# stemangiola/ppcseq

Hardware: AMD Instinct MI355X
Metric: effective samples/sec (whole node) for NB hierarchical fit (higher is better)
Workload: dtype f64; 1 GPU; BASELINE cfg3: synthetic 20000 genes x 200 samples (seed 20253), C=2, K=1000; NUTS (Stan defaults) warm-up 150 + 250 kept draws/chain, 8 chains per GPU (cfg3 names 8 chains; chains are the sharded unit, so N GPUs run 8N chains); mode=chains, chains_total=8, lanes_per_gene=4, loglik_workgroups=939, ess_estimator=rank-normalised split-chain bulk-ESS, min over 6 hyper-parameters and lp__, grad_evals=1471121, divergent_after_warmup=0, round_structure=pipelined: merged log-likelihood / state-machine launch + gene kernel, stream_groups=library default (3 from eight chains on, 2 from four), rounds_last_step_all_groups=115040

## Files before the change

### include/ppcx.h

```cpp
#ifndef PPCX_H
#define PPCX_H
#include <stdint.h>
#ifdef __cplusplus
extern "C" {
#endif

#if defined(__GNUC__)
#define PPCX_API __attribute__((visibility("default")))
#else
#define PPCX_API
#endif

#define PPCX_OK 0
#define PPCX_ERR_ARG (-1)
#define PPCX_ERR_HIP (-2)
#define PPCX_ERR_INIT (-3)
#define PPCX_ERR_STEPSIZE (-4)
#define PPCX_ERR_STALL (-5)
#define PPCX_ERR_LIMIT (-6)
#define PPCX_ERR_CANCELLED (-7)

typedef struct ppcx_model ppcx_model;
typedef struct ppcx_fit ppcx_fit;

#define PPCX_VERSION 400
PPCX_API int ppcx_version(void);
PPCX_API int ppcx_device_count(void);
PPCX_API int ppcx_device_memory(int device, unsigned long long* free_bytes, unsigned long long* total_bytes);
PPCX_API const char* ppcx_last_error(void);

PPCX_API int ppcx_model_create(int device, int G, int S, int C, int K, const int32_t* counts, const double* X,
                      const double* exposure_rate, double lambda_mu_mu, int n_excl, const int32_t* excl,
                      ppcx_model** out);
PPCX_API int ppcx_model_set_exclusions(ppcx_model* m, int n_excl, const int32_t* excl);
PPCX_API int ppcx_model_set_launch(ppcx_model* m, int lanes_per_gene, int workgroups);
PPCX_API int ppcx_model_get_launch(const ppcx_model* m, int* lanes_per_gene, int* nblocks);
PPCX_API int ppcx_model_set_rounds(ppcx_model* m, int pipelined, int stream_groups);
typedef int (*ppcx_progress_fn)(void* user, int first_chain, int chains, int chains_done, long long rounds, double seconds);
PPCX_API int ppcx_model_set_progress(ppcx_model* m, ppcx_progress_fn fn, void* user, double every_seconds);
PPCX_API int ppcx_model_get_rounds(const ppcx_model* m, int nchains, int* pipelined, int* stream_groups);
PPCX_API int ppcx_model_get_plan(ppcx_model* m, int nchains, int* lanes_per_gene, int* workgroups_per_chain, int* bounds, int cap);
PPCX_API int ppcx_model_dim(const ppcx_model* m);
PPCX_API void ppcx_model_destroy(ppcx_model* m);

PPCX_API int ppcx_log_prob_grad(ppcx_model* m, int n_points, const double* u, double* lp, double* grad);

typedef struct {
  int chains, iter, warmup;
  unsigned long long seed;
  double adapt_delta;
  int max_treedepth;
  double init_radius;
  double stepsize0;
  int init_buffer, term_buffer, window;
  int chain_id_offset;
} ppcx_nuts_config;
PPCX_API void ppcx_nuts_config_default(ppcx_nuts_config* cfg);

PPCX_API int ppcx_fit_nuts(ppcx_model* m, const ppcx_nuts_config* cfg, ppcx_fit** out);
PPCX_API int ppcx_fit_info(const ppcx_fit* f, int* chains, int* n_keep, int* D, int* iter);
PPCX_API int ppcx_fit_from_draws(ppcx_model* m, int chains, int n_keep, const double* draws, ppcx_fit** out);
PPCX_API int ppcx_fit_get_draws(ppcx_fit* f, double* out);
PPCX_API int ppcx_fit_get_columns(ppcx_fit* f, int n_cols, const int32_t* cols, double* out);
#define PPCX_SUMMARY_FIELDS 8
PPCX_API int ppcx_fit_summary(ppcx_fit* f, int n_cols, const int32_t* cols, double* out);
PPCX_API int ppcx_fit_get_approximation(ppcx_fit* f, double* mu, double* omega);
PPCX_API int ppcx_fit_get_log_ratios(ppcx_fit* f, double* log_p, double* log_g);
PPCX_API int ppcx_fit_psis(ppcx_fit* f, int n_cols, const int32_t* cols, double* khat);
#define PPCX_LOO_FIELDS 4
PPCX_API int ppcx_fit_get_log_lik(ppcx_fit* f, int n_genes, const int32_t* genes, double* out);
PPCX_API int ppcx_fit_loo(ppcx_fit* f, int n_genes, const int32_t* genes, const double* r_eff, double* out);
#define PPCX_LOO_MCSE_FIELDS 6
PPCX_API int ppcx_fit_loo_mcse(ppcx_fit* f, int n_genes, const int32_t* genes, const double* r_eff, double* out);
PPCX_API int ppcx_fit_relative_eff(ppcx_fit* f, int n_genes, const int32_t* genes, double* out);
#define PPCX_LOO_PREDICT_FIELDS 6
PPCX_API int ppcx_fit_loo_predict(ppcx_fit* f, int n_genes, const int32_t* genes, const double* r_eff, double truncation_compensation,
                                  double p_lo, double p_hi, unsigned long long seed, double* out);
PPCX_API int ppcx_fit_loo_approx(ppcx_fit* f, int n_genes, const int32_t* genes, double* out);
PPCX_API int ppcx_fit_loo_predict_approx(ppcx_fit* f, int n_genes, const int32_t* genes, double truncation_compensation, double p_lo,
                                         double p_hi, unsigned long long seed, double* out);
#define PPCX_PPC_EXACT_FIELDS 9
PPCX_API int ppcx_fit_ppc_exact(ppcx_fit* f, int n_genes, const int32_t* genes, double truncation_compensation, double p_lo,
                                double p_hi, double* out);
PPCX_API int ppcx_fit_get_diagnostics(ppcx_fit* f, double* lp, double* stepsize, int32_t* treedepth,
                             int32_t* n_leapfrog, int32_t* divergent, double* accept);
PPCX_API int ppcx_fit_get_inv_metric(ppcx_fit* f, double* inv_metric);
PPCX_API int ppcx_fit_get_timing(ppcx_fit* f, double* seconds, long long* grad_evals, double* gene_kernel_ms_mean,
                        long long* gene_kernel_samples, double* gene_kernel_chain_launches_mean);

PPCX_API int ppcx_fit_get_kernel_times(ppcx_fit* f, double* loglik_ms, double* close_ms, double* update_ms,
                              long long* launch_triples);

PPCX_API int ppcx_fit_ppc(ppcx_fit* f, double truncation_compensation, double p_lo, double p_hi,
                 unsigned long long seed, int n_gen, int resample, double* ci, int32_t* counts_rng);
PPCX_API int ppcx_fit_get_ppc_timing(ppcx_fit* f, double* kernel_ms, long long* nb_draws);
PPCX_API void ppcx_fit_free(ppcx_fit* f);

PPCX_API void ppcx_do_inference_C(const int* dims, const int* counts, const double* X, const double* exposure_rate,
                         const int* excl, const double* reals, double* ci, double* slope, int* counts_rng,
                         int* status, char** errbuf, const int* errlen);

typedef struct {
  int output_samples, iter; double tol_rel_obj; int grad_samples, elbo_samples, eval_elbo, adapt_iter;
  unsigned long long seed; double init_radius;
} ppcx_advi_config;
PPCX_API void ppcx_advi_config_default(ppcx_advi_config* cfg);
PPCX_API int ppcx_fit_advi(ppcx_model* m, const ppcx_advi_config* cfg, ppcx_fit** out);
PPCX_API int ppcx_fit_advi_iterative(ppcx_model* m, const ppcx_advi_config* cfg, int max_attempts, ppcx_fit** out);
PPCX_API int ppcx_fit_advi_info(const ppcx_fit* f, int* iterations, int* converged, double* elbo, double* eta);

typedef struct ppcx_comm ppcx_comm;
PPCX_API int ppcx_model_create_shard(int device, int G_total, int S, int C, int K_total, int g0, int g1,
                            const int32_t* counts_shard, const double* X, const double* exposure_rate,
                            double lambda_mu_mu, int n_excl, const int32_t* excl_local, ppcx_model** out);
PPCX_API int ppcx_model_create_shard_strided(int device, int G_total, int S, int C, int K_total, int g0, int gene_stride, int n_genes,
                            const int32_t* counts_shard, const double* X, const double* exposure_rate,
                            double lambda_mu_mu, int n_excl, const int32_t* excl_local, ppcx_model** out);
PPCX_API int ppcx_fit_nuts_shards(ppcx_model** shards, int n_shards, const ppcx_nuts_config* cfg, ppcx_fit** fits);
PPCX_API int ppcx_comm_unique_id(char* out128);
PPCX_API int ppcx_comm_create(int device, int nranks, int rank, const char* id128, ppcx_comm** out);
PPCX_API void ppcx_comm_destroy(ppcx_comm* c);
PPCX_API int ppcx_fit_nuts_comm(ppcx_model* shard, const ppcx_nuts_config* cfg, ppcx_comm* comm, ppcx_fit** out);

typedef struct ppcx_xchg ppcx_xchg;
PPCX_API int ppcx_xchg_create(int device, int nranks, int rank, int max_chains, ppcx_xchg** out);
PPCX_API int ppcx_xchg_handle(ppcx_xchg* x, char* out64);
PPCX_API int ppcx_xchg_connect(ppcx_xchg* x, const char* handles );
PPCX_API int ppcx_xchg_connect_local(ppcx_xchg** group, int n);
PPCX_API int ppcx_xchg_set_timeout(ppcx_xchg* x, double seconds);
PPCX_API void ppcx_xchg_destroy(ppcx_xchg* x);
PPCX_API int ppcx_fit_nuts_xchg(ppcx_model* shard, const ppcx_nuts_config* cfg, ppcx_xchg* x, ppcx_fit** out);
PPCX_API int ppcx_fit_get_xchg_timing(ppcx_fit* f, double* wait_us_per_exchange, long long* exchanges);

PPCX_API int ppcx_guard_decision(const double* reduced5, int local_status);

#ifdef __cplusplus
}
#endif
#endif
```

### ppcseq_amd/_lib.py

```python
from __future__ import annotations

import ctypes as C
import os
from dataclasses import dataclass

import numpy as np

_HERE = os.path.dirname(os.path.abspath(__file__))
LIB_PATH = os.environ.get("PPCX_LIB", os.path.join(_HERE, "libppcx.so"))

EXPORTS = [
    "ppcx_version", "ppcx_device_count", "ppcx_last_error", "ppcx_model_create", "ppcx_model_set_exclusions",
    "ppcx_model_set_launch", "ppcx_model_get_launch", "ppcx_model_get_plan", "ppcx_model_dim", "ppcx_model_destroy", "ppcx_log_prob_grad",
    "ppcx_nuts_config_default", "ppcx_fit_nuts", "ppcx_fit_info", "ppcx_fit_from_draws", "ppcx_fit_get_draws", "ppcx_fit_get_columns",
    "ppcx_fit_get_diagnostics", "ppcx_fit_get_timing", "ppcx_fit_get_kernel_times", "ppcx_fit_ppc", "ppcx_fit_free", "ppcx_do_inference_C", "ppcx_model_set_rounds", "ppcx_model_get_rounds", "ppcx_model_set_progress",
    "ppcx_model_create_shard", "ppcx_model_create_shard_strided", "ppcx_fit_nuts_shards", "ppcx_comm_unique_id", "ppcx_comm_create", "ppcx_comm_destroy",
    "ppcx_fit_nuts_comm", "ppcx_advi_config_default", "ppcx_fit_advi", "ppcx_fit_advi_info", "ppcx_fit_advi_iterative",
    "ppcx_guard_decision", "ppcx_device_memory", "ppcx_fit_get_ppc_timing",
    "ppcx_xchg_create", "ppcx_xchg_handle", "ppcx_xchg_connect", "ppcx_xchg_connect_local", "ppcx_xchg_set_timeout", "ppcx_xchg_destroy",
    "ppcx_fit_nuts_xchg", "ppcx_fit_get_xchg_timing", "ppcx_fit_get_inv_metric", "ppcx_fit_summary",
    "ppcx_fit_get_approximation", "ppcx_fit_get_log_ratios", "ppcx_fit_psis", "ppcx_fit_get_log_lik", "ppcx_fit_loo",
    "ppcx_fit_loo_predict", "ppcx_fit_relative_eff", "ppcx_fit_loo_mcse", "ppcx_fit_loo_approx", "ppcx_fit_loo_predict_approx",
    "ppcx_fit_ppc_exact",
]
ABI_VERSION = 400
SUMMARY_FIELDS = ("mean", "sd", "q05", "q50", "q95", "rhat", "ess_bulk", "ess_tail")
LOO_FIELDS = ("elpd_loo", "p_loo", "looic", "khat")
LOO_MCSE_FIELDS = LOO_FIELDS + ("mcse_elpd_loo", "n_eff")
LOO_PREDICT_FIELDS = ("mean", "lower", "upper", "pit_lt", "pit_le", "khat")
PPC_EXACT_FIELDS = ("mean", "sd", "p_le", "p_ge", "lower", "upper", "y", "excluded", "outside")


class PpcxError(RuntimeError):
    pass


class NutsConfig(C.Structure):
    _fields_ = [("chains", C.c_int), ("iter", C.c_int), ("warmup", C.c_int), ("seed", C.c_ulonglong),
                ("adapt_delta", C.c_double), ("max_treedepth", C.c_int), ("init_radius", C.c_double),
                ("stepsize0", C.c_double), ("init_buffer", C.c_int), ("term_buffer", C.c_int), ("window", C.c_int),
                ("chain_id_offset", C.c_int)]


class AdviConfig(C.Structure):
    _fields_ = [("output_samples", C.c_int), ("iter", C.c_int), ("tol_rel_obj", C.c_double), ("grad_samples", C.c_int),
                ("elbo_samples", C.c_int), ("eval_elbo", C.c_int), ("adapt_iter", C.c_int), ("seed", C.c_ulonglong),
                ("init_radius", C.c_double)]


PROGRESS_FN = C.CFUNCTYPE(C.c_int, C.c_void_p, C.c_int, C.c_int, C.c_int, C.c_longlong, C.c_double)
_lib = None


def use_library(path=None):
    global _lib, LIB_PATH
    _lib = None
    LIB_PATH = path if path else os.environ.get("PPCX_LIB", os.path.join(_HERE, "libppcx.so"))


def load() -> C.CDLL:
    global _lib
    if _lib is not None:
        return _lib
    if not os.path.exists(LIB_PATH):
        raise PpcxError(f"{LIB_PATH} not found: run `python -m ppcseq_amd.build` (hipcc, gfx950) first; "
                        "there is no CPU fallback")
    lib = C.CDLL(LIB_PATH)
    lib.ppcx_version.restype = C.c_int
    if lib.ppcx_version() != ABI_VERSION:
        raise PpcxError(f"{LIB_PATH} has ABI version {lib.ppcx_version()}, this binding needs {ABI_VERSION}: rebuild it "
                        "(`python -m ppcseq_amd.build --force`)")
    dp, ip = C.POINTER(C.c_double), C.POINTER(C.c_int32)
    lib.ppcx_guard_decision.argtypes = [dp, C.c_int]
    lib.ppcx_device_memory.argtypes = [C.c_int, C.POINTER(C.c_ulonglong), C.POINTER(C.c_ulonglong)]
    lib.ppcx_fit_get_ppc_timing.argtypes = [C.c_void_p, dp, C.POINTER(C.c_longlong)]
    lib.ppcx_last_error.restype = C.c_char_p
    lib.ppcx_model_create.argtypes = [C.c_int] * 5 + [ip, dp, dp, C.c_double, C.c_int, ip, C.POINTER(C.c_void_p)]
    lib.ppcx_model_set_exclusions.argtypes = [C.c_void_p, C.c_int, ip]
    lib.ppcx_model_set_launch.argtypes = [C.c_void_p, C.c_int, C.c_int]
    lib.ppcx_model_get_launch.argtypes = [C.c_void_p, C.POINTER(C.c_int), C.POINTER(C.c_int)]
    lib.ppcx_model_get_plan.argtypes = [C.c_void_p, C.c_int, C.POINTER(C.c_int), C.POINTER(C.c_int), C.POINTER(C.c_int32), C.c_int]
    lib.ppcx_model_dim.argtypes = [C.c_void_p]
    lib.ppcx_model_destroy.argtypes = [C.c_void_p]
    lib.ppcx_model_destroy.restype = None
    lib.ppcx_log_prob_grad.argtypes = [C.c_void_p, C.c_int, dp, dp, dp]
    lib.ppcx_nuts_config_default.argtypes = [C.POINTER(NutsConfig)]
    lib.ppcx_nuts_config_default.restype = None
    lib.ppcx_fit_nuts.argtypes = [C.c_void_p, C.POINTER(NutsConfig), C.POINTER(C.c_void_p)]
    lib.ppcx_fit_info.argtypes = [C.c_void_p] + [C.POINTER(C.c_int)] * 4
    lib.ppcx_fit_from_draws.argtypes = [C.c_void_p, C.c_int, C.c_int, dp, C.POINTER(C.c_void_p)]
    lib.ppcx_fit_get_draws.argtypes = [C.c_void_p, dp]
    lib.ppcx_fit_get_columns.argtypes = [C.c_void_p, C.c_int, ip, dp]
    lib.ppcx_fit_summary.argtypes = [C.c_void_p, C.c_int, ip, dp]
    lib.ppcx_fit_get_approximation.argtypes = [C.c_void_p, dp, dp]
    lib.ppcx_fit_get_log_ratios.argtypes = [C.c_void_p, dp, dp]
    lib.ppcx_fit_psis.argtypes = [C.c_void_p, C.c_int, ip, dp]
    lib.ppcx_fit_get_log_lik.argtypes = [C.c_void_p, C.c_int, ip, dp]
    lib.ppcx_fit_loo.argtypes = [C.c_void_p, C.c_int, ip, dp, dp]
    lib.ppcx_fit_loo_mcse.argtypes = [C.c_void_p, C.c_int, ip, dp, dp]
    lib.ppcx_fit_loo_predict.argtypes = [C.c_void_p, C.c_int, ip, dp, C.c_double, C.c_double, C.c_double, C.c_ulonglong, dp]
    lib.ppcx_fit_relative_eff.argtypes = [C.c_void_p, C.c_int, ip, dp]
    lib.ppcx_fit_loo_approx.argtypes = [C.c_void_p, C.c_int, ip, dp]
    lib.ppcx_fit_loo_predict_approx.argtypes = [C.c_void_p, C.c_int, ip, C.c_double, C.c_double, C.c_double, C.c_ulonglong, dp]
    lib.ppcx_fit_ppc_exact.argtypes = [C.c_void_p, C.c_int, ip, C.c_double, C.c_double, C.c_double, dp]
    lib.ppcx_fit_get_diagnostics.argtypes = [C.c_void_p, dp, dp, ip, ip, ip, dp]
    lib.ppcx_fit_get_timing.argtypes = [C.c_void_p, dp, C.POINTER(C.c_longlong), dp, C.POINTER(C.c_longlong), dp]
    lib.ppcx_fit_get_kernel_times.argtypes = [C.c_void_p, dp, dp, dp, C.POINTER(C.c_longlong)]
    lib.ppcx_fit_get_inv_metric.argtypes = [C.c_void_p, dp]
    lib.ppcx_fit_ppc.argtypes = [C.c_void_p, C.c_double, C.c_double, C.c_double, C.c_ulonglong, C.c_int, C.c_int, dp, ip]
    lib.ppcx_fit_free.argtypes = [C.c_void_p]
    lib.ppcx_model_set_rounds.argtypes = [C.c_void_p, C.c_int, C.c_int]
    lib.ppcx_xchg_create.argtypes = [C.c_int, C.c_int, C.c_int, C.c_int, C.POINTER(C.c_void_p)]
    lib.ppcx_xchg_handle.argtypes = [C.c_void_p, C.c_char_p]
    lib.ppcx_xchg_connect.argtypes = [C.c_void_p, C.c_char_p]
    lib.ppcx_xchg_connect_local.argtypes = [C.POINTER(C.c_void_p), C.c_int]
    lib.ppcx_xchg_set_timeout.argtypes = [C.c_void_p, C.c_double]
    lib.ppcx_xchg_destroy.argtypes = [C.c_void_p]
    lib.ppcx_xchg_destroy.restype = None
    lib.ppcx_fit_nuts_xchg.argtypes = [C.c_void_p, C.POINTER(NutsConfig), C.c_void_p, C.POINTER(C.c_void_p)]
    lib.ppcx_fit_get_xchg_timing.argtypes = [C.c_void_p, dp, C.POINTER(C.c_longlong)]
    lib.ppcx_model_get_rounds.argtypes = [C.c_void_p, C.c_int, C.POINTER(C.c_int), C.POINTER(C.c_int)]
    lib.ppcx_model_set_progress.argtypes = [C.c_void_p, PROGRESS_FN, C.c_void_p, C.c_double]
    if hasattr(lib, "ppcx_testing_set"):
        lib.ppcx_testing_set.argtypes = [C.c_char_p, C.c_longlong]
        lib.ppcx_testing_set_nccl_provider.argtypes = [C.c_char_p]
        lib.ppcx_testing_bench_kernel.argtypes = [C.c_void_p, C.c_int, C.c_int, C.c_int, C.c_int, C.c_int, dp, C.POINTER(C.c_int)]
    if hasattr(lib, "ppcx_testing_eval_math"):
        lib.ppcx_testing_eval_math.argtypes = [C.c_int, C.c_int, dp, dp, ip, dp, dp]
    if hasattr(lib, "ppcx_testing_get_disp_table"):
        lib.ppcx_testing_get_disp_table.argtypes = [C.c_void_p, dp]
    if hasattr(lib, "ppcx_testing_psis"):
        lib.ppcx_testing_psis.argtypes = [C.c_int, C.c_int, dp, dp, dp]
    if hasattr(lib, "ppcx_testing_loo"):
        lib.ppcx_testing_loo.argtypes = [C.c_int, C.c_int, dp, ip, dp, dp]
    if hasattr(lib, "ppcx_testing_loo_mcse"):
        lib.ppcx_testing_loo_mcse.argtypes = [C.c_int, C.c_int, dp, ip, dp, dp]
    if hasattr(lib, "ppcx_testing_loo_predict"):
        lib.ppcx_testing_loo_predict.argtypes = [dp, ip, C.c_int, C.c_int, ip, ip, dp, C.c_double, C.c_double, dp]
    if hasattr(lib, "ppcx_testing_loo_approx"):
        lib.ppcx_testing_loo_approx.argtypes = [C.c_int, C.c_int, dp, dp, ip, dp]
        lib.ppcx_testing_loo_predict_approx.argtypes = [dp, dp, ip, C.c_int, C.c_int, ip, ip, C.c_double, C.c_double, dp]
    if hasattr(lib, "ppcx_testing_relative_eff"):
        lib.ppcx_testing_relative_eff.argtypes = [C.c_int, C.c_int, C.c_int, dp, dp]
    if hasattr(lib, "ppcx_testing_ppc_exact"):
        lib.ppcx_testing_ppc_exact.argtypes = [C.c_int, C.c_int, dp, dp, ip, ip, C.c_double, C.c_double, C.c_double, dp]
    lib.ppcx_fit_free.restype = None
    lib.ppcx_advi_config_default.argtypes = [C.POINTER(AdviConfig)]
    lib.ppcx_advi_config_default.restype = None
    lib.ppcx_fit_advi.argtypes = [C.c_void_p, C.POINTER(AdviConfig), C.POINTER(C.c_void_p)]
    lib.ppcx_fit_advi_iterative.argtypes = [C.c_void_p, C.POINTER(AdviConfig), C.c_int, C.POINTER(C.c_void_p)]
    lib.ppcx_fit_advi_info.argtypes = [C.c_void_p, C.POINTER(C.c_int), C.POINTER(C.c_int), C.POINTER(C.c_double), C.POINTER(C.c_double)]
    lib.ppcx_model_create_shard.argtypes = [C.c_int] * 7 + [ip, dp, dp, C.c_double, C.c_int, ip, C.POINTER(C.c_void_p)]
    lib.ppcx_model_create_shard_strided.argtypes = [C.c_int] * 8 + [ip, dp, dp, C.c_double, C.c_int, ip, C.POINTER(C.c_void_p)]
    lib.ppcx_fit_nuts_shards.argtypes = [C.POINTER(C.c_void_p), C.c_int, C.POINTER(NutsConfig), C.POINTER(C.c_void_p)]
    lib.ppcx_comm_unique_id.argtypes = [C.c_char_p]
    lib.ppcx_comm_create.argtypes = [C.c_int, C.c_int, C.c_int, C.c_char_p, C.POINTER(C.c_void_p)]
    lib.ppcx_comm_destroy.argtypes = [C.c_void_p]
    lib.ppcx_comm_destroy.restype = None
    lib.ppcx_fit_nuts_comm.argtypes = [C.c_void_p, C.POINTER(NutsConfig), C.c_void_p, C.POINTER(C.c_void_p)]
    _lib = lib
    return lib


def _check(rc: int):
    if rc != 0:
        raise PpcxError(f"ppcx error {rc}: {load().ppcx_last_error().decode()}")


def _p(a, t):
    return a.ctypes.data_as(C.POINTER(t)) if a is not None else None


def testing_set(key: str, value: int):
    lib = load()
    if not hasattr(lib, "ppcx_testing_set"):
        raise PpcxError(f"{LIB_PATH} is not the testing build")
    _check(lib.ppcx_testing_set(key.encode(), int(value)))


def testing_set_nccl_provider(path: str):
    lib = load()
    if not hasattr(lib, "ppcx_testing_set_nccl_provider"):
        raise PpcxError(f"{LIB_PATH} is not the testing build")
    _check(lib.ppcx_testing_set_nccl_provider(path.encode() if path else None))


TESTING_MATH = ("fast_rcp", "fast_log", "fast_exp", "table_log", "window_log", "stirling_tails", "stirling_excess",
                "log_erfc_ratio", "cell", "cell_win", "cell_y", "cell_win_y", "sincos_2pi", "lgamma_int1", "rng_exp", "rng_div")
TESTING_MATH_MORE = ("nb2_tails",)


def testing_eval_math(fn: str, a, b=None, y=None):
    lib = load()
    if not hasattr(lib, "ppcx_testing_eval_math"):
        raise PpcxError(f"{LIB_PATH} is not the testing build, or one built before ppcx_testing_math.hip existed: rebuild it "
                        "(`python -m ppcseq_amd.build --testing --force`)")
    a = np.ascontiguousarray(a, dtype=np.float64).ravel()
    n = a.size
    b = np.ascontiguousarray(np.zeros(n) if b is None else np.broadcast_to(b, (n,)), dtype=np.float64)
    y = np.ascontiguousarray(np.zeros(n) if y is None else np.broadcast_to(y, (n,)), dtype=np.int32)
    o0, o1 = np.zeros(n), np.zeros(n)
    rc = lib.ppcx_testing_eval_math((TESTING_MATH + TESTING_MATH_MORE).index(fn), n, _p(a, C.c_double), _p(b, C.c_double), _p(y, C.c_int32),
                                    _p(o0, C.c_double), _p(o1, C.c_double))
    if rc != 0:
        raise PpcxError(f"ppcx_testing_eval_math({fn}) failed with code {rc}")
    return o0, o1


def testing_psis(lr, cols=None):
    lib = load()
    if not hasattr(lib, "ppcx_testing_psis"):
        raise PpcxError(f"{LIB_PATH} is not the testing build, or one built before ppcx_testing_psis existed: rebuild it "
                        "(`python -m ppcseq_amd.build --testing --force`)")
    lr = np.ascontiguousarray(lr, dtype=np.float64).ravel()
    n = lr.size
    cols = np.zeros((n, 0)) if cols is None else np.ascontiguousarray(cols, dtype=np.float64).reshape(n, -1)
    out = np.zeros(cols.shape[1] + 1)
    _check(lib.ppcx_testing_psis(n, int(cols.shape[1]), _p(lr, C.c_double), _p(cols, C.c_double) if cols.size else None,
                                 _p(out, C.c_double)))
    return out


def testing_loo(ll, excluded=None, r_eff=None):
    return _testing_loo("ppcx_testing_loo", LOO_FIELDS, ll, excluded, r_eff)


def testing_loo_mcse(ll, excluded=None, r_eff=None):
    return _testing_loo("ppcx_testing_loo_mcse", LOO_MCSE_FIELDS, ll, excluded, r_eff)


def _testing_loo(entry, fields, ll, excluded, r_eff):
    lib = load()
    if not hasattr(lib, entry):
        raise PpcxError(f"{LIB_PATH} is not the testing build, or one built before {entry} existed: rebuild it "
                        "(`python -m ppcseq_amd.build --testing --force`)")
    ll = np.asarray(ll, dtype=np.float64)
    ll = ll.reshape(ll.shape[0], -1)
    n, nc = ll.shape
    cols = np.ascontiguousarray(ll.T)
    ex = None if excluded is None else np.ascontiguousarray(excluded, dtype=np.int32).ravel()
    re = None if r_eff is None else np.ascontiguousarray(r_eff, dtype=np.float64).ravel()
    out = np.zeros((nc, len(fields)))
    _check(getattr(lib, entry)(n, nc, _p(cols, C.c_double), _p(ex, C.c_int32) if ex is not None else None,
                               _p(re, C.c_double) if re is not None else None, _p(out, C.c_double)))
    return out


def testing_loo_predict(ll, x, y, excluded=None, r_eff=None, p_lo=0.025, p_hi=0.975):
    lib = load()
    if not hasattr(lib, "ppcx_testing_loo_predict"):
        raise PpcxError(f"{LIB_PATH} is not the testing build, or one built before ppcx_testing_loo_predict existed: rebuild it "
                        "(`python -m ppcseq_amd.build --testing --force`)")
    ll = np.asarray(ll, dtype=np.float64)
    ll = ll.reshape(ll.shape[0], -1)
    n, nc = ll.shape
    cols = np.ascontiguousarray(ll.T)
    xs = np.ascontiguousarray(np.asarray(x).reshape(n, nc).T, dtype=np.int32)
    ys = np.ascontiguousarray(np.broadcast_to(np.asarray(y), (nc,)), dtype=np.int32)
    ex = None if excluded is None else np.ascontiguousarray(excluded, dtype=np.int32).ravel()
    re = None if r_eff is None else np.ascontiguousarray(r_eff, dtype=np.float64).ravel()
    out = np.zeros((nc, len(LOO_PREDICT_FIELDS)))
    _check(lib.ppcx_testing_loo_predict(_p(cols, C.c_double), _p(xs, C.c_int32), n, nc, _p(ys, C.c_int32),
                                        _p(ex, C.c_int32) if ex is not None else None,
                                        _p(re, C.c_double) if re is not None else None, float(p_lo), float(p_hi),
                                        _p(out, C.c_double)))
    return out


def _testing_approx_columns(entry, ll, log_ratio, excluded):
    lib = load()
    if not hasattr(lib, entry):
        raise PpcxError(f"{LIB_PATH} is not the testing build, or one built before {entry} existed: rebuild it "
                        "(`python -m ppcseq_amd.build --testing --force`)")
    ll = np.asarray(ll, dtype=np.float64)
    ll = ll.reshape(ll.shape[0], -1)
    lr = np.ascontiguousarray(log_ratio, dtype=np.float64).ravel()
    if lr.size != ll.shape[0]:
        raise ValueError("log_ratio must hold one value per draw")
    ex = None if excluded is None else np.ascontiguousarray(excluded, dtype=np.int32).ravel()
    return lib, np.ascontiguousarray(ll.T), lr, ex


def testing_loo_approx(ll, log_ratio, excluded=None):
# ... 11 lines not shown
    xs = np.ascontiguousarray(np.asarray(x).reshape(n, nc).T, dtype=np.int32)
    ys = np.ascontiguousarray(np.broadcast_to(np.asarray(y), (nc,)), dtype=np.int32)
    out = np.zeros((nc, len(LOO_PREDICT_FIELDS)))
    _check(lib.ppcx_testing_loo_predict_approx(_p(cols, C.c_double), _p(lr, C.c_double), _p(xs, C.c_int32), n, nc, _p(ys, C.c_int32),
                                               _p(ex, C.c_int32) if ex is not None else None, float(p_lo), float(p_hi),
                                               _p(out, C.c_double)))
    return out


def testing_relative_eff(ll, chains):
    lib = load()
    if not hasattr(lib, "ppcx_testing_relative_eff"):
        raise PpcxError(f"{LIB_PATH} is not the testing build, or one built before ppcx_testing_relative_eff existed: rebuild it "
                        "(`python -m ppcseq_amd.build --testing --force`)")
    ll = np.asarray(ll, dtype=np.float64)
    ll = ll.reshape(ll.shape[0], -1)
    rows, nc = ll.shape
    chains = int(chains)
    if chains < 1 or rows % chains:
        raise ValueError("ll must hold chains * n rows")
    cols = np.ascontiguousarray(ll.T)
    out = np.zeros(nc)
    _check(lib.ppcx_testing_relative_eff(chains, rows // chains, nc, _p(cols, C.c_double), _p(out, C.c_double)))
    return out


def _ppc_exact_dict(out):
    res = {k: out[..., i].copy() for i, k in enumerate(PPC_EXACT_FIELDS)}
    nan = np.isnan(res["lower"]) | np.isnan(res["upper"])
    for k in ("lower", "upper"):
        res[k] = np.where(nan, -1, res[k]).astype(np.int64)
    res["y"] = res["y"].astype(np.int64)
    res["excluded"] = res["excluded"] != 0
    res["outside"] = np.where(nan, 0, res["outside"]) != 0
    return res


def testing_ppc_exact(eta, sigma_raw, y, excluded=None, truncation_compensation=1.0, p_lo=0.025, p_hi=0.975, raw=False):
    lib = load()
    if not hasattr(lib, "ppcx_testing_ppc_exact"):
        raise PpcxError(f"{LIB_PATH} is not the testing build, or one built before ppcx_testing_ppc_exact existed: rebuild it "
                        "(`python -m ppcseq_amd.build --testing --force`)")
    eta = np.asarray(eta, dtype=np.float64)
    eta = eta.reshape(eta.shape[0], -1)
    n, nc = eta.shape
    ec = np.ascontiguousarray(eta.T)
    sc = np.ascontiguousarray(np.asarray(sigma_raw, dtype=np.float64).reshape(n, nc).T)
    ys = np.ascontiguousarray(np.broadcast_to(np.asarray(y), (nc,)), dtype=np.int32)
    ex = None if excluded is None else np.ascontiguousarray(excluded, dtype=np.int32).ravel()
    out = np.zeros((nc, len(PPC_EXACT_FIELDS)))
    _check(lib.ppcx_testing_ppc_exact(n, nc, _p(ec, C.c_double), _p(sc, C.c_double), _p(ys, C.c_int32),
                                      _p(ex, C.c_int32) if ex is not None else None, float(truncation_compensation), float(p_lo),
                                      float(p_hi), _p(out, C.c_double)))
    return out if raw else _ppc_exact_dict(out)


def loo_estimates(pointwise, excluded):
    keep = ~np.asarray(excluded, bool)
    out = {}
    for name in LOO_FIELDS[:3]:
        v = np.asarray(pointwise[name], dtype=np.float64)[keep]
        se = float(np.sqrt(v.size * np.var(v, ddof=1))) if v.size > 1 else float("nan")
        out[name] = (float(np.sum(v)), se)
    return out


def device_count() -> int:
    return int(load().ppcx_device_count())


def device_memory(device=0):
    f, t = C.c_ulonglong(), C.c_ulonglong()
    _check(load().ppcx_device_memory(int(device), C.byref(f), C.byref(t)))
    return int(f.value), int(t.value)


def shard_genes(G_total, g0, stride):
    return list(range(int(g0), int(G_total), int(stride)))


class Model:

    def __init__(self, counts, X, exposure_rate, K, lambda_mu_mu=5.612671, excl=None, device=0, shard=None):
        lib = load()
        counts = np.ascontiguousarray(counts, dtype=np.int32)
        if counts.ndim != 2:
            raise ValueError("counts must be G x S")
        self.G, self.S = counts.shape
        X = np.asfortranarray(np.asarray(X, dtype=np.float64).reshape(self.S, -1))
        self.C = X.shape[1]
        self.K = int(K)
        exposure_rate = np.ascontiguousarray(exposure_rate, dtype=np.float64)
        if exposure_rate.shape != (self.S,):
            raise ValueError("exposure_rate must have length S")
        excl = np.ascontiguousarray(excl if excl is not None else np.zeros(0), dtype=np.int32)
        self.X, self.exposure_rate = X, exposure_rate
        self.excl = excl.copy()
        self.counts = counts
        h = C.c_void_p()
        self.shard = shard
        if shard is None:
            _check(lib.ppcx_model_create(int(device), self.G, self.S, self.C, self.K, _p(counts, C.c_int32),
                                         _p(X, C.c_double), _p(exposure_rate, C.c_double), float(lambda_mu_mu),
                                         int(excl.size), _p(excl, C.c_int32), C.byref(h)))
        else:
            if len(shard) == 5:
                Gt, Kt, g0, stride = int(shard[0]), int(shard[1]), int(shard[2]), int(shard[4])
                if len(shard_genes(Gt, g0, stride)) != self.G:
                    raise ValueError("counts must hold exactly the genes of the shard")
                self.K = len([g for g in shard_genes(Gt, g0, stride) if g < Kt])
                _check(lib.ppcx_model_create_shard_strided(int(device), Gt, self.S, self.C, Kt, g0, stride, self.G, _p(counts, C.c_int32),
                                                           _p(X, C.c_double), _p(exposure_rate, C.c_double), float(lambda_mu_mu),
                                                           int(excl.size), _p(excl, C.c_int32), C.byref(h)))
            else:
                Gt, Kt, g0, g1 = (int(v) for v in shard)
                if g1 - g0 != self.G:
                    raise ValueError("counts must hold exactly the genes of the shard")
                self.K = max(0, min(g1, Kt) - min(g0, Kt))
                _check(lib.ppcx_model_create_shard(int(device), Gt, self.S, self.C, Kt, g0, g1, _p(counts, C.c_int32),
                                                   _p(X, C.c_double), _p(exposure_rate, C.c_double), float(lambda_mu_mu),
                                                   int(excl.size), _p(excl, C.c_int32), C.byref(h)))
        self._h = h
        self.D = int(lib.ppcx_model_dim(h))

    def set_exclusions(self, excl):
        excl = np.ascontiguousarray(excl if excl is not None else np.zeros(0), dtype=np.int32)
        _check(load().ppcx_model_set_exclusions(self._h, int(excl.size), _p(excl, C.c_int32)))
        self.excl = excl.copy()

    def set_launch(self, lanes_per_gene=0, workgroups=0):
        _check(load().ppcx_model_set_launch(self._h, int(lanes_per_gene), int(workgroups)))

    def get_plan(self, nchains):
        lanes, nb = C.c_int(), C.c_int()
        _check(load().ppcx_model_get_plan(self._h, int(nchains), C.byref(lanes), C.byref(nb), None, 0))
        b = np.zeros(4 * nb.value + 1, np.int32)
        _check(load().ppcx_model_get_plan(self._h, int(nchains), C.byref(lanes), C.byref(nb), _p(b, C.c_int32), int(b.size)))
        return lanes.value, nb.value, b

    def get_launch(self):
        a, b = C.c_int(), C.c_int()
        _check(load().ppcx_model_get_launch(self._h, C.byref(a), C.byref(b)))
        return a.value, b.value

    def testing_disp_table(self):
        lib = load()
        if not hasattr(lib, "ppcx_testing_get_disp_table"):
            raise PpcxError(f"{LIB_PATH} is not the testing build, or one built before ppcx_testing_get_disp_table existed: "
                            "rebuild it (`python -m ppcseq_amd.build --testing --force`)")
        out = np.zeros((self.G, 32, 2, 12))
        _check(lib.ppcx_testing_get_disp_table(self._h, _p(out, C.c_double)))
        return out

    def log_prob_grad(self, u):
        u = np.ascontiguousarray(u, dtype=np.float64)
        one = u.ndim == 1
        u2 = u.reshape(-1, self.D)
        lp = np.zeros(u2.shape[0])
        g = np.zeros_like(u2)
        _check(load().ppcx_log_prob_grad(self._h, u2.shape[0], _p(u2, C.c_double), _p(lp, C.c_double), _p(g, C.c_double)))
        return (float(lp[0]), g[0]) if one else (lp, g)

    def fit_nuts(self, chains=3, iter=300, warmup=150, seed=1, adapt_delta=0.8, max_treedepth=10, init_radius=2.0,
                 stepsize0=1.0, init_buffer=75, term_buffer=50, window=25, chain_id_offset=0) -> "Fit":
        cfg = NutsConfig(chains, iter, warmup, seed, adapt_delta, max_treedepth, init_radius, stepsize0,
                         init_buffer, term_buffer, window, chain_id_offset)
        h = C.c_void_p()
        _check(load().ppcx_fit_nuts(self._h, C.byref(cfg), C.byref(h)))
        return Fit(self, h)

    def fit_advi(self, output_samples=1000, iter=50000, tol_rel_obj=0.005, elbo_samples=100, eval_elbo=100, adapt_iter=50,
                 seed=1, init_radius=2.0, max_attempts=1) -> "Fit":
        cfg = AdviConfig(output_samples, iter, tol_rel_obj, 1, elbo_samples, eval_elbo, adapt_iter, seed, init_radius)
        h = C.c_void_p()
        if max_attempts > 1:
            _check(load().ppcx_fit_advi_iterative(self._h, C.byref(cfg), int(max_attempts), C.byref(h)))
        else:
            _check(load().ppcx_fit_advi(self._h, C.byref(cfg), C.byref(h)))
        return Fit(self, h)

    def fit_from_draws(self, draws) -> "Fit":
        draws = np.ascontiguousarray(draws, dtype=np.float64)
        if draws.ndim != 3 or draws.shape[2] != self.D:
            raise ValueError("draws must be [chains, n_keep, D]")
        h = C.c_void_p()
        _check(load().ppcx_fit_from_draws(self._h, draws.shape[0], draws.shape[1], _p(draws, C.c_double), C.byref(h)))
        return Fit(self, h)

    def fit_nuts_comm(self, comm: "Comm", **kw) -> "Fit":
        cfg = _make_cfg(**kw)
        h = C.c_void_p()
        _check(load().ppcx_fit_nuts_comm(self._h, C.byref(cfg), comm._h, C.byref(h)))
        return Fit(self, h)

    def fit_nuts_xchg(self, xchg: "Xchg", **kw) -> "Fit":
        cfg = _make_cfg(**kw)
        h = C.c_void_p()
        _check(load().ppcx_fit_nuts_xchg(self._h, C.byref(cfg), xchg._h, C.byref(h)))
        return Fit(self, h)

    def set_rounds(self, pipelined=-2, stream_groups=-1):
        _check(load().ppcx_model_set_rounds(self._h, int(pipelined), int(stream_groups)))

    def set_progress(self, fn=None, every_seconds=1.0):
        self._progress_cb = PROGRESS_FN((lambda user, c0, n, done, rounds, sec: 1 if fn(c0, n, done, rounds, sec) else 0) if fn else 0)
        _check(load().ppcx_model_set_progress(self._h, self._progress_cb, None, float(every_seconds)))

    def get_rounds(self, nchains=1):
        a, b = C.c_int(), C.c_int()
        _check(load().ppcx_model_get_rounds(self._h, int(nchains), C.byref(a), C.byref(b)))
        return bool(a.value), b.value

    def bench_kernel(self, which=0, nchains=1, warm_rounds=40, reps=50, n_merge=1):
        lib = load()
        if not hasattr(lib, "ppcx_testing_bench_kernel"):
            raise PpcxError(f"{LIB_PATH} is not the testing build")
        ms, t = C.c_double(), C.c_int()
        _check(lib.ppcx_testing_bench_kernel(self._h, int(which), nchains, warm_rounds, reps, n_merge, C.byref(ms), C.byref(t)))
        return ms.value, t.value

    def close(self):
        if getattr(self, "_h", None):
            load().ppcx_model_destroy(self._h)
            self._h = None

    def __del__(self):
        try:
            self.close()
        except Exception:
            pass


def _make_cfg(chains=3, iter=300, warmup=150, seed=1, adapt_delta=0.8, max_treedepth=10, init_radius=2.0,
              stepsize0=1.0, init_buffer=75, term_buffer=50, window=25, chain_id_offset=0):
    return NutsConfig(chains, iter, warmup, seed, adapt_delta, max_treedepth, init_radius, stepsize0,
                      init_buffer, term_buffer, window, chain_id_offset)


def fit_nuts_shards(models, **kw):
    cfg = _make_cfg(**kw)
    n = len(models)
    hm = (C.c_void_p * n)(*[m._h for m in models])
    hf = (C.c_void_p * n)()
    _check(load().ppcx_fit_nuts_shards(hm, n, C.byref(cfg), hf))
    return [Fit(m, C.c_void_p(h)) for m, h in zip(models, hf)]


class Comm:

    @staticmethod
    def unique_id() -> bytes:
        buf = C.create_string_buffer(128)
        _check(load().ppcx_comm_unique_id(buf))
        return buf.raw

    def __init__(self, nranks, rank, unique_id: bytes, device=0):
        h = C.c_void_p()
        _check(load().ppcx_comm_create(int(device), int(nranks), int(rank), unique_id, C.byref(h)))
        self._h = h

    def close(self):
        if getattr(self, "_h", None):
            load().ppcx_comm_destroy(self._h)
            self._h = None


class Xchg:

    def __init__(self, nranks, rank, max_chains, device=0):
        h = C.c_void_p()
        _check(load().ppcx_xchg_create(int(device), int(nranks), int(rank), int(max_chains), C.byref(h)))
        self._h, self.nranks, self.rank = h, int(nranks), int(rank)

    def handle(self) -> bytes:
        buf = C.create_string_buffer(64)
        _check(load().ppcx_xchg_handle(self._h, buf))
        return buf.raw

    def connect(self, handles):
        blob = b"".join(handles)
        if len(blob) != 64 * self.nranks:
            raise ValueError("need one 64-byte handle per rank")
        _check(load().ppcx_xchg_connect(self._h, blob))

    @staticmethod
    def local_group(n, max_chains, devices=None):
        xs = [Xchg(n, k, max_chains, device=(devices[k] if devices else 0)) for k in range(n)]
        arr = (C.c_void_p * n)(*[x._h for x in xs])
        _check(load().ppcx_xchg_connect_local(arr, n))
        return xs

    def set_timeout(self, seconds):
        _check(load().ppcx_xchg_set_timeout(self._h, float(seconds)))

    def close(self):
        if getattr(self, "_h", None):
            load().ppcx_xchg_destroy(self._h)
            self._h = None


@dataclass
class Timing:
    seconds: float
    grad_evals: int
    gene_kernel_ms_mean: float
    gene_kernel_samples: int
# ... 212 lines not shown
```

### ppcseq_amd/build.py

```python
from __future__ import annotations

import os
import subprocess
import sys
import threading

HERE = os.path.dirname(os.path.abspath(__file__))
CSRC = os.path.join(HERE, "csrc")
LIB = os.path.join(HERE, "libppcx.so")
TESTING_LIB = os.path.join(os.path.dirname(HERE), "tests", "libppcx_testing.so")
SOURCES = ["ppcx_kernels.hip", "ppcx_summary.hip", "ppcx_psis.hip", "ppcx_loo.hip", "ppcx_loo_predict.hip", "ppcx_reff.hip", "ppcx_ppc_exact.hip", "ppcx_ppc.hip",
           "ppcx_capi.hip", "ppcx_run.hip", "ppcx_fit_nuts.hip", "ppcx_fit_advi.hip", "ppcx_fit_api.hip"]
TESTING_SOURCES = ["ppcx_testing_math.hip"]
HEADERS = ["ppcx_math.h", "ppcx_disp.h", "ppcx_model.h", "ppcx_nuts.h", "ppcx_gene.h", "ppcx_kernels.h", "ppcx_summary.h", "ppcx_summary_dev.h", "ppcx_psis.h", "ppcx_psis_dev.h", "ppcx_loo.h", "ppcx_loo_ap.h", "ppcx_loo_dev.h", "ppcx_loo_predict.h", "ppcx_reff.h", "ppcx_nbcdf.h", "ppcx_ppc_exact.h", "ppcx_ppc.h", "ppcx_table.h", "ppcx_block.h", "ppcx_columns.h", "ppcx_host.h", "ppcx_testing.h",
           os.path.join("..", "..", "include", "ppcx.h")]


CODEGEN_FLAGS = ["-fno-slp-vectorize"]


def _sources(extra):
    return SOURCES + (TESTING_SOURCES if "-DPPCX_TESTING" in extra else [])


def _stale(lib: str, extra=()) -> bool:
    if not os.path.exists(lib):
        return True
    t = os.path.getmtime(lib)
    return any(os.path.getmtime(os.path.join(CSRC, f)) > t for f in _sources(extra) + HEADERS)


_COMPILERS = threading.BoundedSemaphore(16)


def _start_compiler(cmd):
    _COMPILERS.acquire()
    p = subprocess.Popen(cmd)
    threading.Thread(target=lambda: (p.wait(), _COMPILERS.release()), daemon=True).start()
    return p


def _compile(lib: str, extra, verbose: bool) -> None:
    hipcc = os.environ.get("HIPCC", "/opt/rocm/bin/hipcc")
    objs = []
    procs = []
    for s in _sources(extra):
        o = lib + "." + s + ".o"
        objs.append(o)
        cmd = [hipcc, "-O3", "-std=c++17", "--offload-arch=gfx950", "-fPIC", "-fvisibility=hidden", "-Wno-unused-result"] + CODEGEN_FLAGS + extra + \
              ["-c", "-o", o, os.path.join(CSRC, s)]
        if verbose:
            print(" ".join(cmd), file=sys.stderr)
        procs.append(_start_compiler(cmd))
    for p in procs:
        if p.wait() != 0:
            raise subprocess.CalledProcessError(p.returncode, p.args)
    subprocess.check_call([hipcc, "--offload-arch=gfx950", "-shared", "-fPIC", "-o", lib] + objs)
    for o in objs:
        os.remove(o)


def build(force: bool = False, verbose: bool = False) -> str:
    if force or _stale(LIB):
        _compile(LIB, [], verbose)
    return LIB


def build_testing(force: bool = False, verbose: bool = False) -> str:
    if force or _stale(TESTING_LIB, ["-DPPCX_TESTING"]):
        _compile(TESTING_LIB, ["-DPPCX_TESTING"], verbose)
    return TESTING_LIB


def build_all(force: bool = False, verbose: bool = False):
    jobs = []
    if force or _stale(LIB):
        jobs.append((LIB, []))
    if force or _stale(TESTING_LIB, ["-DPPCX_TESTING"]):
        jobs.append((TESTING_LIB, ["-DPPCX_TESTING"]))
    errs = []

    def run(lib, extra):
        try:
            _compile(lib, extra, verbose)
        except Exception as e:
            errs.append(e)
    th = [threading.Thread(target=run, args=j) for j in jobs]
    for t in th:
        t.start()
    for t in th:
        t.join()
    if errs:
        raise errs[0]
    return LIB, TESTING_LIB


if __name__ == "__main__":
    if "--testing" in sys.argv:
        print(*build_all(force="--force" in sys.argv, verbose=True))
    else:
        print(build(force="--force" in sys.argv, verbose=True))
```

### ppcseq_amd/csrc/ppcx_capi.hip

```cpp
#include <math.h>
#include <stdlib.h>
#include <algorithm>
#include <memory>
#include "ppcx_host.h"

thread_local std::string g_err;
int fail(int code, const std::string& msg) { g_err = msg; return code; }
int hip_fail(hipError_t e, const char* what) { return fail(PPCX_ERR_HIP, std::string(what) + ": " + hipGetErrorString(e)); }
int hip_done(const char* who, hipError_t e) {
  return e == hipSuccess ? PPCX_OK : who ? hip_fail(e, who) : fail(PPCX_ERR_HIP, hipGetErrorString(e));
}
#ifdef PPCX_TESTING
TestHooks g_test;
#endif

extern "C" int ppcx_version(void) { return PPCX_VERSION; }
extern "C" int ppcx_device_count(void) { int n = 0; if (hipGetDeviceCount(&n) != hipSuccess) return 0; return n; }
extern "C" const char* ppcx_last_error(void) { return g_err.c_str(); }
extern "C" int ppcx_device_memory(int device, unsigned long long* free_bytes, unsigned long long* total_bytes) {
  int ndev = 0;
  HIPCHK(hipGetDeviceCount(&ndev));
  if (device < 0 || device >= ndev) return fail(PPCX_ERR_ARG, "no such HIP device");
  HIPCHK(hipSetDevice(device));
  size_t f = 0, t = 0;
  HIPCHK(hipMemGetInfo(&f, &t));
  if (free_bytes) *free_bytes = (unsigned long long)f;
  if (total_bytes) *total_bytes = (unsigned long long)t;
  return PPCX_OK;
}

static double pass_cost(const ppcx_model* m, int L, int p, int n) {
  const int S = m->d.S;
  bool slope = false;
  for (int i = p; i < p + n; ++i) slope = slope || m->pos_slope[i];
  double slope_w = m->d.C > 2 ? 1.0 : 1.15;
#ifdef PPCX_TESTING
  if (g_test.slope_cost_permille > 0) slope_w = 1e-3 * g_test.slope_cost_permille;
#endif
  double lin_w = 2.5;
#ifdef PPCX_TESTING
  if (g_test.slope_cost_permille > 0) lin_w = 1e-3 * g_test.slope_cost_permille;
#endif
  const double sweep = (double)((S + L - 1) / L) * (!m->d.x0_is_one ? 2.5 : (slope && !m->d.x1_binary ? lin_w : (slope ? slope_w : 1.0)));
  return 5.8 + sweep;
}
static int resident_workgroups(const ppcx_model* m, int reserve) {
  int n = m->wgs_override > 0 ? m->wgs_override : m->n_cu * (reserve > 0 ? m->ls_wgs_per_cu : m->wgs_per_cu);
  n -= reserve;
  return n < 1 ? 1 : n;
}
constexpr double kTrimSlack = 0.0;
static int workgroups_per_chain(const ppcx_model* m, int L, int nch, int n_res, bool whole_runs = true, bool trim = false) {
  int nbpc = n_res / (nch < 1 ? 1 : nch);
  if (nbpc >= 8 && whole_runs) nbpc = nbpc / 8 * 8;
  if (nbpc < 1) nbpc = 1;
  const int gpw = 64 / L, npass = (m->d.G + gpw - 1) / gpw;
  if (nbpc > (npass + 3) / 4) nbpc = (npass + 3) / 4;
  if (trim) {
    double slack = kTrimSlack;
#ifdef PPCX_TESTING
    if (g_test.trim_slack_permille >= 0) slack = 1e-3 * g_test.trim_slack_permille;
#endif
    int maxp = (npass + 4 * nbpc - 1) / (4 * nbpc);
#ifdef PPCX_TESTING
    maxp += g_test.trim_extra_passes;
#endif
    int nb2 = (int)ceil((double)npass * (1.0 + slack) / (4.0 * maxp));
    if (nb2 >= 8 && whole_runs) nb2 = (nb2 + 7) / 8 * 8;
    if (nb2 < nbpc) nbpc = nb2;
  }
  return nbpc;
}
static int default_stream_groups(int nch) { return nch >= 8 ? 3 : (nch >= 4 ? 2 : 1); }
int fit_stream_groups(const ppcx_model* m, int nch) {
  if (m->opt_stream_groups >= 1) return m->opt_stream_groups < nch ? m->opt_stream_groups : nch;
  return default_stream_groups(nch);
}
int fit_launch_chains(const ppcx_model* m, int nch) {
  const int g = fit_stream_groups(m, nch);
  return (nch + g - 1) / g;
}
static void drop_plans(ppcx_model* m) {
  std::lock_guard<std::mutex> lk(m->plan_mutex);
  m->plans.clear();
}
void choose_launch(ppcx_model* m, int nchains) {
  const int G = m->d.G, S = m->d.S;
  int bestL = 64; double best = 1e300;
  for (int L = 64; L >= 1; L >>= 1) {
    const int gpw = 64 / L;
    const double npass = ceil((double)G / gpw), c_pass = (8.0 + (double)((S + L - 1) / L)) * (L <= 2 ? 1.2 : 1.0);
    const int wpc = 4 * workgroups_per_chain(m, L, nchains, resident_workgroups(m, 0));
    const double t = ceil(npass / wpc) * c_pass;
    if (t < best) { best = t; bestL = L; }
  }
  const int L = m->L_override > 0 ? m->L_override : bestL;
  if (L != m->L) {
    drop_plans(m);
    m->L = L;
  }
  m->nblocks_chosen = workgroups_per_chain(m, m->L, nchains, resident_workgroups(m, 0)) * nchains;
}
int plan_launch(ppcx_model* m, int nch, int reserve, bool trim, int* nbpc_out, const int** d_bounds_out) {
  std::lock_guard<std::mutex> lk(m->plan_mutex);
  const int n_res = resident_workgroups(m, reserve);
  const auto key = std::make_pair(nch, trim ? -n_res : n_res);
  auto it = m->plans.find(key);
  if (it != m->plans.end()) { *nbpc_out = it->second.nbpc; *d_bounds_out = it->second.d_bounds.p; return PPCX_OK; }
  const int G = m->d.G, L = m->L, gpw = 64 / L;
  const int nbpc = workgroups_per_chain(m, L, nch, n_res, reserve == 0, trim), wpc = 4 * nbpc, npass = (G + gpw - 1) / gpw;
  std::vector<double> cost(npass);
  double total = 0;
  for (int k = 0; k < npass; ++k) {
    const int p = k * gpw;
    cost[k] = pass_cost(m, L, p, G - p < gpw ? G - p : gpw);
    total += cost[k];
  }
  std::vector<int> bounds(wpc + 1, G);
  bounds[0] = 0;
  {
    int k = 0; double cum = 0.0;
    for (int j = 1; j < wpc; ++j) {
      const double target = total * (double)j / (double)wpc;
      while (k < npass && cum + 0.5 * cost[k] < target) cum += cost[k++];
      bounds[j] = k * gpw < G ? k * gpw : G;
    }
  }
  {
    const long pmax = ((long)(npass + wpc - 1) / wpc) * gpw;
    for (int j = 0; j < wpc; ++j) if (bounds[j + 1] - bounds[j] > pmax) bounds[j + 1] = (int)(bounds[j] + pmax);
    bounds[wpc] = G;
    for (int j = wpc - 1; j >= 0; --j) if (bounds[j + 1] - bounds[j] > pmax) bounds[j] = (int)(bounds[j + 1] - pmax);
  }
  DeviceBuffer<int> d_bounds;
  HIPCHK(d_bounds.alloc((size_t)(wpc + 1)));
  HIPCHK(hipMemcpy(d_bounds.p, bounds.data(), sizeof(int) * (size_t)(wpc + 1), hipMemcpyHostToDevice));
  ppcx_model::Plan& pl = m->plans[key];
  pl.nbpc = nbpc; std::swap(pl.d_bounds.p, d_bounds.p);
  *nbpc_out = pl.nbpc; *d_bounds_out = pl.d_bounds.p;
  return PPCX_OK;
}

static int upload_counts(ppcx_model* m, int n_excl, const int32_t* excl) {
  const int G = m->d.G, S = m->d.S, C = m->d.C;
  std::vector<int32_t> cnt(m->counts_host);
  for (int e = 0; e < n_excl; ++e) {
    if (excl[e] < 0 || excl[e] >= G * S) return fail(PPCX_ERR_ARG, "excluded cell id out of range");
    cnt[excl[e]] = -1;
  }
  std::vector<double> Sy(G, 0.0), SyE(G, 0.0), SyX((size_t)C * G, 0.0), SX((size_t)C * G, 0.0), ncell(G, 0.0), Lg1(G, 0.0);
  std::vector<unsigned char> gflags(G, 0);
  for (int g = 0; g < G; ++g) {
    double sy = 0, sye = 0, nc = 0, lg1 = 0;
    for (int s = 0; s < S; ++s) {
      const int y = cnt[(size_t)g * S + s];
      if (y < 0) { gflags[g] |= 1; continue; }
      sy += y; sye += (double)y * m->expo_host[s]; nc += 1.0; lg1 += lgamma((double)y + 1.0);
      for (int c = 0; c < C; ++c) { SyX[(size_t)c * G + g] += (double)y * m->X_host[(size_t)c * S + s]; SX[(size_t)c * G + g] += m->X_host[(size_t)c * S + s]; }
    }
    Sy[g] = sy; SyE[g] = sye; ncell[g] = nc; Lg1[g] = lg1;
  }
  HIPCHK(hipMemcpy(m->d_gflags.p, gflags.data(), (size_t)G, hipMemcpyHostToDevice));
  {
    std::vector<int> ord(G);
    for (int g = 0; g < G; ++g) ord[g] = g;
    const int K = m->d.K;
    std::stable_sort(ord.begin(), ord.end(), [&](int a, int b) {
      const bool sa = a < K && C >= 2, sb = b < K && C >= 2;
      if (sa != sb) return sa;
      return gflags[a] > gflags[b];
    });
    {
      int ns = 0;
      while (ns < G && ord[ns] < K && C >= 2) ++ns;
      constexpr int kOrderBlock = 16;
      const int nbs = (ns + kOrderBlock - 1) / kOrderBlock, nb = (G + kOrderBlock - 1) / kOrderBlock;
      const bool dear_slopes = m->d.x0_is_one && !m->d.x1_binary;
      if (ns > 0 && ns < G && nbs < nb && dear_slopes) {
        std::vector<int> mixed; mixed.reserve(G);
        int is = 0, ip = ns, sb = 0;
        for (int b = 0; b < nb; ++b) {
          const bool slope_block = sb < nbs && b == (int)((long long)sb * nb / nbs);
          if (slope_block && is < ns) { for (int k = 0; k < kOrderBlock && is < ns; ++k) mixed.push_back(ord[is++]); ++sb; }
          else { for (int k = 0; k < kOrderBlock && ip < G; ++k) mixed.push_back(ord[ip++]); }
        }
        while (is < ns) mixed.push_back(ord[is++]);
        while (ip < G) mixed.push_back(ord[ip++]);
        ord.swap(mixed);
      }
    }
    HIPCHK(hipMemcpy(m->d_order.p, ord.data(), sizeof(int) * (size_t)G, hipMemcpyHostToDevice));
    m->pos_slope.resize(G);
    for (int p = 0; p < G; ++p) m->pos_slope[p] = ord[p] < K && C >= 2;
    drop_plans(m);
  }
  HIPCHK(hipMemcpy(m->d_counts.p, cnt.data(), sizeof(int32_t) * cnt.size(), hipMemcpyHostToDevice));
  m->excluded_host.assign(cnt.size(), 0);
  for (size_t i = 0; i < cnt.size(); ++i) m->excluded_host[i] = cnt[i] < 0;
  {
    const hipError_t e = launch_disp_build_kernel(m->d_counts.p, G, S, nullptr, G, m->fit, m->d_disp.p, m->stream.s);
    if (e != hipSuccess) return fail(PPCX_ERR_HIP, std::string("dispersion-table kernel: ") + hipGetErrorString(e));
  }
  HIPCHK(hipMemcpy(m->d_Sy.p, Sy.data(), sizeof(double) * G, hipMemcpyHostToDevice));
  HIPCHK(hipMemcpy(m->d_SyE.p, SyE.data(), sizeof(double) * G, hipMemcpyHostToDevice));
  HIPCHK(hipMemcpy(m->d_SyX.p, SyX.data(), sizeof(double) * SyX.size(), hipMemcpyHostToDevice));
  HIPCHK(hipMemcpy(m->d_SX.p, SX.data(), sizeof(double) * SX.size(), hipMemcpyHostToDevice));
  HIPCHK(hipMemcpy(m->d_ncell.p, ncell.data(), sizeof(double) * G, hipMemcpyHostToDevice));
  HIPCHK(hipMemcpy(m->d_Lg1.p, Lg1.data(), sizeof(double) * G, hipMemcpyHostToDevice));
  HIPCHK(hipStreamSynchronize(m->stream.s));
  return PPCX_OK;
}

extern "C" int ppcx_model_create(int device, int G, int S, int C, int K, const int32_t* counts, const double* X,
                                 const double* exposure, double lambda_mu_mu, int n_excl, const int32_t* excl,
                                 ppcx_model** out) {
  if (!out) return fail(PPCX_ERR_ARG, "out is NULL");
  *out = nullptr;
  if (G < 1 || S < 1 || C < 1 || K < 0 || K > G) return fail(PPCX_ERR_ARG, "need G>=1, S>=1, C>=1, 0<=K<=G");
  if (C > kMaxC) return fail(PPCX_ERR_LIMIT, "C exceeds the 16 design columns this build supports");
  if ((long long)G * S > 2000000000LL) return fail(PPCX_ERR_LIMIT, "G*S exceeds int32 cell ids");
  if (!counts || !X || !exposure || (n_excl > 0 && !excl)) return fail(PPCX_ERR_ARG, "NULL input buffer");
  for (long long i = 0; i < (long long)G * S; ++i) if (counts[i] < 0) return fail(PPCX_ERR_ARG, "negative count");
  int ndev = 0;
  HIPCHK(hipGetDeviceCount(&ndev));
  if (device < 0 || device >= ndev) return fail(PPCX_ERR_ARG, "no such HIP device");
  HIPCHK(hipSetDevice(device));
  std::unique_ptr<ppcx_model> owner(new ppcx_model());
  ppcx_model* m = owner.get();
  m->device = device;
  m->d = make_dims(G, S, C, K, lambda_mu_mu);
  m->CM = C <= 2 ? 2 : (C <= 4 ? 4 : (C <= 8 ? 8 : 16));
  {
    hipDeviceProp_t prop;
    HIPCHK(hipGetDeviceProperties(&prop, device));
    m->n_cu = prop.multiProcessorCount > 0 ? prop.multiProcessorCount : 256;
  }
  m->counts_host.assign(counts, counts + (size_t)G * S);
  m->X_host.assign(X, X + (size_t)S * C);
  m->expo_host.assign(exposure, exposure + S);
  int x0 = 1;
  for (int s = 0; s < S; ++s) if (X[s] != 1.0) x0 = 0;
  m->d.x0_is_one = x0;
  int x1b = (C >= 2);
  for (size_t i = (size_t)S; i < (size_t)S * C && x1b; ++i) if (X[i] != 0.0 && X[i] != 1.0) x1b = 0;
#ifdef PPCX_TESTING
  if (g_test.force_generic) x1b = 0;
#endif
  m->d.x1_binary = x1b;
  m->d.raw_consts = (!x0 || (C >= 2 && K > 0 && !x1b)) ? 1 : 0;
  if (C > 8 && (!x0 || (K > 0 && !x1b)))
    return fail(PPCX_ERR_LIMIT, "more than 8 design columns are supported for designs of a column of ones and 0 / 1 indicator columns only");
  if (const char* e = getenv("PPCX_PIPELINE")) if (atoi(e) == 0) m->opt_pipelined = 0;
  if (const char* e = getenv("PPCX_STREAM_GROUPS")) { const int v = atoi(e); if (v >= 1) m->opt_stream_groups = v; }
  if (loglik_lds_bytes(m->d) > 160u * 1024u)
    return fail(PPCX_ERR_LIMIT, "the per-sample constants (S * C doubles; S * (2 + C) for a design without a column of ones) do not fit the 160 KB of LDS of a compute unit beside the 20 KB of tables");
  m->wgs_per_cu = loglik_resident_workgroups_per_cu(m->CM, m->d);
  if (m->wgs_per_cu < 1) return fail(PPCX_ERR_LIMIT, "the log-likelihood kernel cannot be resident with S * (2 + C) doubles of per-sample constants in LDS");
  m->ls_wgs_per_cu = ls_resident_workgroups_per_cu(m->CM, m->d);
  std::vector<double> E(S);
  for (int s = 0; s < S; ++s) E[s] = exp(exposure[s]);
  HIPCHK(m->stream.create());
  HIPCHK(m->d_counts.alloc(((size_t)G * S + 512)));
  HIPCHK(hipMemset(m->d_counts.p, 0, sizeof(int32_t) * ((size_t)G * S + 512)));
  HIPCHK(m->d_E.alloc(S));
  HIPCHK(m->d_expo.alloc(S));
  HIPCHK(m->d_X.alloc((size_t)S * C));
  HIPCHK(m->d_Sy.alloc(G));
  HIPCHK(m->d_SyE.alloc(G));
  HIPCHK(m->d_SyX.alloc((size_t)C * G));
  HIPCHK(m->d_SX.alloc((size_t)C * G));
  HIPCHK(m->d_ncell.alloc(G));
  HIPCHK(m->d_disp.alloc((size_t)G * kDispGeneDoubles));
  HIPCHK(m->d_gflags.alloc((size_t)G));
  disp_fit_init(m->fit);
  HIPCHK(m->d_Lg1.alloc(G));
  HIPCHK(m->d_logtab.alloc(2 * kLogTabSize));
  { double tab[2 * kLogTabSize]; fill_log_table(tab); HIPCHK(hipMemcpy(m->d_logtab.p, tab, sizeof(tab), hipMemcpyHostToDevice)); }
  HIPCHK(m->d_wintab.alloc(2 * kWinTabSize));
  { std::vector<double> wt(2 * kWinTabSize); fill_window_log_table(wt.data()); HIPCHK(hipMemcpy(m->d_wintab.p, wt.data(), sizeof(double) * wt.size(), hipMemcpyHostToDevice)); }
  m->e_min = m->e_max = E[0];
  for (int s = 1; s < S; ++s) { if (E[s] < m->e_min) m->e_min = E[s]; if (E[s] > m->e_max) m->e_max = E[s]; }
  HIPCHK(m->d_order.alloc((size_t)G));
  HIPCHK(hipMemcpy(m->d_E.p, E.data(), sizeof(double) * S, hipMemcpyHostToDevice));
  HIPCHK(hipMemcpy(m->d_expo.p, exposure, sizeof(double) * S, hipMemcpyHostToDevice));
  HIPCHK(hipMemcpy(m->d_X.p, X, sizeof(double) * (size_t)S * C, hipMemcpyHostToDevice));
  const int rc = upload_counts(m, n_excl, excl);
  if (rc != PPCX_OK) return rc;
  choose_launch(m, 1);
  *out = owner.release();
  return PPCX_OK;
}
extern "C" int ppcx_model_create_shard_strided(int device, int G_total, int S, int C, int K_total, int g0, int gene_stride, int n_genes,
                                               const int32_t* counts_shard, const double* X, const double* exposure,
                                               double lambda_mu_mu, int n_excl, const int32_t* excl_local, ppcx_model** out) {
  if (g0 < 0 || gene_stride < 1 || n_genes < 1 || K_total < 0 || K_total > G_total ||
      (long long)g0 + (long long)gene_stride * (n_genes - 1) >= G_total) return fail(PPCX_ERR_ARG, "bad gene shard");
  int kl = 0;
  if (g0 < K_total) kl = (K_total - g0 + gene_stride - 1) / gene_stride;
  if (kl > n_genes) kl = n_genes;
  int rc = ppcx_model_create(device, n_genes, S, C, kl, counts_shard, X, exposure, lambda_mu_mu, n_excl, excl_local, out);
  if (rc != PPCX_OK) return rc;
  (*out)->d.Gt = G_total; (*out)->d.Kt = K_total; (*out)->d.g0 = g0; (*out)->d.k0 = g0 < K_total ? g0 : K_total; (*out)->d.gstride = gene_stride;
  return PPCX_OK;
}
extern "C" int ppcx_model_create_shard(int device, int G_total, int S, int C, int K_total, int g0, int g1,
                                       const int32_t* counts_shard, const double* X, const double* exposure,
                                       double lambda_mu_mu, int n_excl, const int32_t* excl_local, ppcx_model** out) {
  if (g0 < 0 || g1 <= g0 || g1 > G_total) return fail(PPCX_ERR_ARG, "bad gene range");
  return ppcx_model_create_shard_strided(device, G_total, S, C, K_total, g0, 1, g1 - g0, counts_shard, X, exposure, lambda_mu_mu, n_excl, excl_local, out);
}

extern "C" int ppcx_model_set_exclusions(ppcx_model* m, int n_excl, const int32_t* excl) {
  if (!m || (n_excl > 0 && !excl) || n_excl < 0) return fail(PPCX_ERR_ARG, "bad arguments");
  HIPCHK(hipSetDevice(m->device));
  return upload_counts(m, n_excl, excl);
}
extern "C" int ppcx_model_set_launch(ppcx_model* m, int lanes_per_gene, int workgroups) {
  if (!m) return fail(PPCX_ERR_ARG, "model is NULL");
  if (lanes_per_gene != 0 && (lanes_per_gene < 1 || lanes_per_gene > 64 || (lanes_per_gene & (lanes_per_gene - 1))))
    return fail(PPCX_ERR_ARG, "lanes_per_gene must be 0 or a power of two <= 64");
  if (workgroups < 0 || workgroups > (1 << 20)) return fail(PPCX_ERR_ARG, "workgroups must be 0 (automatic) or a positive count");
  HIPCHK(hipSetDevice(m->device));
  m->L_override = lanes_per_gene; m->wgs_override = workgroups;
  drop_plans(m);
  choose_launch(m, 1);
  return PPCX_OK;
}
extern "C" int ppcx_model_set_rounds(ppcx_model* m, int pipelined, int stream_groups) {
  if (!m) return fail(PPCX_ERR_ARG, "model is NULL");
  if (pipelined < -2 || pipelined > 1 || stream_groups < -1 || stream_groups > 64) return fail(PPCX_ERR_ARG, "pipelined must be -2 .. 1 and stream_groups -1 .. 64");
  if (pipelined != -2) m->opt_pipelined = pipelined;
  if (stream_groups != -1) m->opt_stream_groups = stream_groups;
  return PPCX_OK;
}
bool model_pipelines(const ppcx_model* m) {
  return m->opt_pipelined != 0 && m->ls_wgs_per_cu >= 1;
}
extern "C" int ppcx_model_set_progress(ppcx_model* m, ppcx_progress_fn fn, void* user, double every_seconds) {
  if (!m || !(every_seconds >= 0)) return fail(PPCX_ERR_ARG, "bad arguments");
  m->progress = fn; m->progress_user = user; m->progress_every = every_seconds;
  return PPCX_OK;
}
extern "C" int ppcx_model_get_rounds(const ppcx_model* m, int nchains, int* pipelined, int* stream_groups) {
  if (!m || nchains < 1) return fail(PPCX_ERR_ARG, "bad arguments");
  if (pipelined) *pipelined = model_pipelines(m) ? 1 : 0;
  if (stream_groups) *stream_groups = fit_stream_groups(m, nchains);
  return PPCX_OK;
}
extern "C" int ppcx_model_get_launch(const ppcx_model* m, int* lanes_per_gene, int* nblocks) {
  if (!m) return fail(PPCX_ERR_ARG, "model is NULL");
  if (lanes_per_gene) *lanes_per_gene = m->L;
  if (nblocks) *nblocks = m->nblocks_chosen;
  return PPCX_OK;
}
extern "C" int ppcx_model_get_plan(ppcx_model* m, int nchains, int* lanes_per_gene, int* workgroups_per_chain, int* bounds, int cap) {
  if (!m || nchains == 0) return fail(PPCX_ERR_ARG, "bad arguments");
  HIPCHK(hipSetDevice(m->device));
  const bool trim = nchains < 0;
  if (trim) nchains = -nchains; else choose_launch(m, nchains);
  int nbpc = 0; const int* d_bounds = nullptr;
  const int rc = plan_launch(m, nchains, 0, trim, &nbpc, &d_bounds);
  if (rc != PPCX_OK) return rc;
  if (lanes_per_gene) *lanes_per_gene = m->L;
  if (workgroups_per_chain) *workgroups_per_chain = nbpc;
  if (bounds) {
    const int n = 4 * nbpc + 1;
    if (cap < n) return fail(PPCX_ERR_ARG, "bounds buffer too small");
    HIPCHK(hipMemcpy(bounds, d_bounds, sizeof(int) * (size_t)n, hipMemcpyDeviceToHost));
  }
  return PPCX_OK;
}
extern "C" int ppcx_model_dim(const ppcx_model* m) { return m ? m->d.D : PPCX_ERR_ARG; }
extern "C" void ppcx_model_destroy(ppcx_model* m) {
  if (!m) return;
  if (m->live_fits > 0) { m->destroy_requested = true; return; }
  (void)hipSetDevice(m->device);
  delete m;
}

#ifdef PPCX_TESTING
extern "C" int ppcx_testing_set(const char* key, long long value) {
  if (!key) return fail(PPCX_ERR_ARG, "key is NULL");
  const std::string k(key);
  if (k == "fail_at_round") g_test.fail_at_round = value;
  else if (k == "fail_rank") g_test.fail_rank = (int)value;
  else if (k == "force_generic") g_test.force_generic = (int)value;
  else if (k == "slope_cost_permille") g_test.slope_cost_permille = (int)value;
  else if (k == "trim_slack_permille") g_test.trim_slack_permille = (int)value;
  else if (k == "trim_extra_passes") g_test.trim_extra_passes = (int)value;
  else if (k == "psis_slots") g_test.psis_slots = (int)value;
  else if (k == "psis_scratch_bytes") g_test.psis_scratch_bytes = value;
  else if (k == "loo_scratch_bytes") g_test.loo_scratch_bytes = value;
  else return fail(PPCX_ERR_ARG, "unknown test hook " + k);
  return PPCX_OK;
}
extern "C" int ppcx_testing_get_disp_table(ppcx_model* m, double* out) {
  if (!m || !out) return fail(PPCX_ERR_ARG, "bad arguments");
  HIPCHK(hipSetDevice(m->device));
  HIPCHK(hipStreamSynchronize(m->stream.s));
  HIPCHK(hipMemcpy(out, m->d_disp.p, sizeof(double) * (size_t)m->d.G * kDispGeneDoubles, hipMemcpyDeviceToHost));
  return PPCX_OK;
}
#endif
```

### ppcseq_amd/csrc/ppcx_gene.h

```cpp
#pragma once
#include "ppcx_nuts.h"


namespace ppcx {

template <int CM>
struct GeneCtx {
  static constexpr int NCM = CM + 1;
  int gg, ncoord;
  bool active, has_slopes, fast, two;
  int idx[NCM];
  double q[NCM];
  GeneParams<CM> gp;
};

PPCX_HD void coord_consts(const Dims& d, const VecRef& v, int i, double q) {
  if (i >= d.off_sigma_raw && i < d.off_tail) {
    v.at(V_C0, i) = fast_exp(-q); v.at(V_C2, i) = q;
  } else if (i >= d.off_intercept && i < d.off_sigma_raw) {
    v.at(V_C0, i) = fast_exp(q);
    if (d.raw_consts) v.at(V_C2, i) = q;
  }
}

template <int CM>
PPCX_HD void gene_index(const Dims& d, int g, GeneCtx<CM>& x) {
  constexpr int NCM = CM + 1;
  x.active = g < d.G;
  x.gg = x.active ? g : 0;
  const int C = d.C;
  const int nslope = x.gg < d.K ? (C - 1 > 1 ? C - 1 : 1) : 0;
  x.ncoord = x.active ? 2 + nslope : 0;
#pragma unroll
  for (int j = 0; j < NCM; ++j)
    x.idx[j] = j == 0 ? d.off_intercept + x.gg : (j == 1 ? d.off_sigma_raw + x.gg : coef_index(d, j - 1, x.gg));
  x.has_slopes = x.active && x.gg < d.K && C >= 2;
  x.two = x.has_slopes && d.x0_is_one && d.x1_binary;
  x.fast = d.x0_is_one && (!x.has_slopes || x.two);
}
template <int CM>
PPCX_HD void gene_params(const Dims& d, const VecRef& v, GeneCtx<CM>& x) {
  x.gp.coef[0] = x.q[0];
#pragma unroll
  for (int cc = 1; cc < CM; ++cc) x.gp.coef[cc] = (x.has_slopes && cc < d.C) ? x.q[cc + 1] : 0.0;
  x.gp.sigma_raw = x.q[1];
  x.gp.phi = x.active ? v.at(V_C0, x.idx[1]) : 1.0;
  x.gp.invphi = 0.0;
}
template <int CM>
PPCX_HD void gene_load(const Dims& d, const Cmd& c, const VecRef& v, int g, GeneCtx<CM>& x) {
  constexpr int NCM = CM + 1;
  gene_index<CM>(d, g, x);
#pragma unroll
  for (int j = 0; j < NCM; ++j) x.q[j] = j < x.ncoord ? v.at(V_Q0 + 3 * c.dir, x.idx[j]) : 0.0;
  gene_params<CM>(d, v, x);
}

struct CellData {
  const int* counts;
  const double* disp;
  const unsigned char* gflags;
  const double* Sy;
  const double* ncell;
  double e_min, e_max;
};

struct GenePre { double phi, sigma, a0, Sy, n; int flags; };
PPCX_HD GenePre gene_pre_load(const Dims& d, const VecRef& v, const CellData& m, int g) {
  GenePre r;
  r.phi = v.at(V_C0, d.off_sigma_raw + g);
  r.sigma = v.at(V_C2, d.off_sigma_raw + g);
  r.a0 = v.at(V_C0, d.off_intercept + g);
  r.Sy = m.Sy[g]; r.n = m.ncell[g]; r.flags = m.gflags[g];
  return r;
}
template <int L> struct DispDeal {
  static constexpr int NL = L >= 8 ? 4 : (L >= 4 ? 2 : 1);
  static constexpr int CH = kDispStride / NL;
};

template <int CM, int L, int MODE, bool MASKED, bool WIN>
PPCX_HD void sweep_cells(int S, const int* row, const double* sE, const double* sX1, int sub, double A, double A1, double one,
                         const GeneParams<CM>& gp, const double* tab, CellAcc<CM>& acc, const double* ec = nullptr, int C = 2) {
  const int nmin = S / L;
  const int nlane = nmin + (sub < S - nmin * L ? 1 : 0);
  const int* p = row + sub;
  const double* q = sE + sub;
  const double* qx = sX1 + sub;
  int y0 = p[0], y1 = p[L], y2 = p[2 * L], y3 = p[3 * L];
  int k = 0;
#define PPCX_SWEEP_CELL(Y, E, XB, OFF, COND)                                                    \
  if ((COND) && (!MASKED || (Y) >= 0)) {                                                        \
    if (MODE == 1) { const double a1_ = (XB) != 0.0 ? A1 : A;                                   \
                     const double rho_ = WIN ? cell_eval_win<CM, true>(Y, E, a1_, one, gp, tab, acc) : cell_eval<CM, true>(Y, E, a1_, gp, tab, acc); \
                     acc.Tx[1] = fma(XB, rho_, acc.Tx[1]); }                                    \
    else if (MODE == 2) {                                                                       \
      double a_ = (XB) != 0.0 ? A1 : A; double xk_[CM];                                         \
      _Pragma("unroll") for (int cc = 2; cc < CM; ++cc) { xk_[cc] = cc < C ? qx[(cc - 1) * S + (OFF)] : 0.0; a_ = xk_[cc] != 0.0 ? a_ * ec[cc] : a_; } \
      const double rho_ = WIN ? cell_eval_win<CM, true>(Y, E, a_, one, gp, tab, acc) : cell_eval<CM, true>(Y, E, a_, gp, tab, acc); \
      acc.Tx[1] = fma(XB, rho_, acc.Tx[1]);                                                     \
      _Pragma("unroll") for (int cc = 2; cc < CM; ++cc) acc.Tx[cc] = fma(xk_[cc], rho_, acc.Tx[cc]); \
    }                                                                                           \
    else if (MODE == 3) {                                                                       \
      double t_ = (XB) * ec[1]; double xk_[CM];                                                 \
      _Pragma("unroll") for (int cc = 2; cc < CM; ++cc) { xk_[cc] = cc < C ? qx[(cc - 1) * S + (OFF)] : 0.0; t_ = fma(xk_[cc], ec[cc], t_); } \
      const double rho_ = cell_eval<CM, true>(Y, E, A * fast_exp(t_), gp, tab, acc);           \
      acc.Tx[1] = fma(XB, rho_, acc.Tx[1]);                                                     \
      _Pragma("unroll") for (int cc = 2; cc < CM; ++cc) acc.Tx[cc] = fma(xk_[cc], rho_, acc.Tx[cc]); \
    }                                                                                           \
    else if (WIN) (void)cell_eval_win<CM, false>(Y, E, A, one, gp, tab, acc);                   \
    else (void)cell_eval<CM, false>(Y, E, A, gp, tab, acc);                                     \
  }
  for (; k + 4 <= nmin; k += 4) {
    const double e0 = q[0], e1 = q[L], e2 = q[2 * L], e3 = q[3 * L];
    double x0 = 0.0, x1 = 0.0, x2 = 0.0, x3 = 0.0;
    if (MODE != 0) { x0 = qx[0]; x1 = qx[L]; x2 = qx[2 * L]; x3 = qx[3 * L]; }
    p += 4 * L; q += 4 * L; qx += 4 * L;
    const int n0 = p[0], n1 = p[L], n2 = p[2 * L], n3 = p[3 * L];
    if (MODE == 0 && !MASKED && WIN) {
      CellMidWin c0, c1, c2, c3;
      (void)cell_front_win<CM, false>(y0, e0, A, one, gp, tab, acc, c0);
      (void)cell_front_win<CM, false>(y1, e1, A, one, gp, tab, acc, c1);
      (void)cell_front_win<CM, false>(y2, e2, A, one, gp, tab, acc, c2);
      (void)cell_front_win<CM, false>(y3, e3, A, one, gp, tab, acc, c3);
#if defined(__HIP_DEVICE_COMPILE__)
      __builtin_amdgcn_sched_barrier(0);
#endif
      cell_back_win<CM>(c0, acc); cell_back_win<CM>(c1, acc); cell_back_win<CM>(c2, acc); cell_back_win<CM>(c3, acc);
    } else if (MODE == 0 && !MASKED) {
      CellMid c0, c1, c2, c3;
      (void)cell_front<CM, false>(y0, e0, A, gp, tab, acc, c0);
      (void)cell_front<CM, false>(y1, e1, A, gp, tab, acc, c1);
      (void)cell_front<CM, false>(y2, e2, A, gp, tab, acc, c2);
      (void)cell_front<CM, false>(y3, e3, A, gp, tab, acc, c3);
#if defined(__HIP_DEVICE_COMPILE__)
      __builtin_amdgcn_sched_barrier(0);
#endif
      cell_back<CM>(c0, acc); cell_back<CM>(c1, acc); cell_back<CM>(c2, acc); cell_back<CM>(c3, acc);
    } else {
      PPCX_SWEEP_CELL(y0, e0, x0, -4 * L, true)
      PPCX_SWEEP_CELL(y1, e1, x1, -3 * L, true)
      PPCX_SWEEP_CELL(y2, e2, x2, -2 * L, true)
      PPCX_SWEEP_CELL(y3, e3, x3, -L, true)
    }
    y0 = n0; y1 = n1; y2 = n2; y3 = n3;
  }
  if (k < nlane) {
    const double e0 = q[0], e1 = q[L], e2 = q[2 * L], e3 = q[3 * L];
    double x0 = 0.0, x1 = 0.0, x2 = 0.0, x3 = 0.0;
    if (MODE != 0) { x0 = qx[0]; x1 = qx[L]; x2 = qx[2 * L]; x3 = qx[3 * L]; }
    PPCX_SWEEP_CELL(y0, e0, x0, 0, true)
    PPCX_SWEEP_CELL(y1, e1, x1, L, k + 1 < nlane)
    PPCX_SWEEP_CELL(y2, e2, x2, 2 * L, k + 2 < nlane)
    PPCX_SWEEP_CELL(y3, e3, x3, 3 * L, k + 3 < nlane)
  }
#undef PPCX_SWEEP_CELL
}

template <int CM, int L>
PPCX_HD void generic_cells(const Dims& d, const Cmd& c, const VecRef& v, int g, bool has_slopes, const int* row,
                           const double* sExpo, const double* sX, int sub, GeneParams<CM>& gp, const double* tab,
                           CellAcc<CM>& acc) {
  const int S = d.S, C = d.C;
  gp.coef[0] = v.at(V_C2, d.off_intercept + g);
#pragma unroll
  for (int cc = 1; cc < CM; ++cc) gp.coef[cc] = (has_slopes && cc < C) ? v.at(V_C2, coef_index(d, cc, g)) : 0.0;
  (void)c;
  for (int s = sub; s < S; s += L) {
    const int y = row[s];
    if (y >= 0) {
      double t = sExpo[s] + gp.sigma_raw;
#pragma unroll
      for (int cc = 0; cc < CM; ++cc) if (cc < C) t += sX[cc * S + s] * gp.coef[cc];
      const double u = fast_exp(t);
      const double rho = cell_eval<CM, true>(y, u, 1.0, gp, tab, acc);
#pragma unroll
      for (int cc = 0; cc < CM; ++cc) if (cc < C) acc.Tx[cc] = fma(sX[cc * S + s], rho, acc.Tx[cc]);
    }
  }
}

template <int CM, int L, int GEN = 3>
PPCX_HD void lane_gene_sums(const Dims& d, const Cmd& c, const VecRef& v, const CellData& m, int g, const GenePre& pre, int sub,
                            const double* sE, const double* sExpo, const double* sX, const double* tab, const double* wtab,
                            GeneSumsV<CM>& o
#ifdef PPCX_TRACE
                            , unsigned long long* trace_stamps = nullptr
#endif
                            ) {
#if defined(PPCX_TRACE) && defined(__HIP_DEVICE_COMPILE__)
#define PPCX_GSTAMP(k) do { if (trace_stamps) trace_stamps[k] = __builtin_readcyclecounter(); } while (0)
#else
#define PPCX_GSTAMP(k) ((void)0)
#endif
  const int S = d.S;
  const bool has_slopes = g < d.K && d.C >= 2;
  const bool two = has_slopes && d.x0_is_one && d.x1_binary;
  const bool lin = (GEN & 1) && d.x0_is_one && has_slopes && !two;
  const bool generic = (GEN & 2) && !d.x0_is_one;
  GeneParams<CM> gp;
  gp.phi = pre.phi;
  const double sigma = pre.sigma;
  gp.sigma_raw = sigma;
  gp.invphi = fast_rcp(gp.phi);
  const double A = pre.a0 * gp.invphi;
  const bool masked = (pre.flags & 1) != 0;
  const int* row = m.counts + (long)g * S;
  constexpr int NL = DispDeal<L>::NL, CH = DispDeal<L>::CH;
  const DispRef dr = disp_ref(sigma);
  const int fn = L == 1 ? 0 : sub / NL, jch = L == 1 ? 0 : sub - fn * NL;
  const bool tab_lane = dr.in && (L == 1 || fn < 2);
  const double* pc = m.disp + (((long)g * kDispPanels + dr.panel) * 2 + (fn & 1)) * kDispStride + jch * CH;
  double cf[CH], cf2[L == 1 ? CH : 1];
#pragma unroll
  for (int k = 0; k < CH; ++k) cf[k] = 0.0;
  cf2[0] = 0.0;
  if (tab_lane) {
#pragma unroll
    for (int k = 0; k < CH; ++k) cf[k] = pc[k];
    if (L == 1) {
#pragma unroll
      for (int k = 0; k < CH; ++k) cf2[k] = pc[kDispStride + k];
    }
  }
  CellAcc<CM> acc; acc.zero();
  PPCX_GSTAMP(5);
  if (GEN & 2) {
    if (PPCX_WAVE_ANY(generic)) {
      if (generic) generic_cells<CM, L>(d, c, v, g, has_slopes, row, sExpo, sX, sub, gp, tab, acc);
    }
  }
  GeneWindow gw; gw.k = 0; gw.ok = false; gw.scale = 1.0;
  bool win = false;
  if (!(GEN & 2) || PPCX_WAVE_ANY(!generic)) {
    if (!generic) {
      const bool any_masked = PPCX_WAVE_ANY(masked);
#define PPCX_SWEEP(MODE, A_LO, A_HI, A_, A1_, X1_, ...)                                                                  \
      gw = gene_window(fma(m.e_min, A_LO, 1.0), fma(m.e_max, A_HI, 1.0));                                                 \
      win = !any_masked && PPCX_WAVE_ALL(gw.ok);                                                                          \
      if (any_masked) sweep_cells<CM, L, MODE, true, false>(S, row, sE, X1_, sub, A_, A1_, 1.0, gp, tab, acc, ##__VA_ARGS__);   \
      else if (win) sweep_cells<CM, L, MODE, false, true>(S, row, sE, X1_, sub, (A_) * gw.scale, (A1_) * gw.scale, gw.scale, gp, wtab, acc, ##__VA_ARGS__); \
      else sweep_cells<CM, L, MODE, false, false>(S, row, sE, X1_, sub, A_, A1_, 1.0, gp, tab, acc, ##__VA_ARGS__);
      if ((GEN & 1) && PPCX_WAVE_ANY(lin)) {
        double be[CM];
        be[0] = 0.0;
#pragma unroll
        for (int cc = 1; cc < CM; ++cc) be[cc] = (lin && cc < d.C) ? v.at(V_C2, coef_index(d, cc, g)) : 0.0;
        if (any_masked) sweep_cells<CM, L, 3, true, false>(S, row, sE, sX + S, sub, A, A, 1.0, gp, tab, acc, be, d.C);
        else sweep_cells<CM, L, 3, false, false>(S, row, sE, sX + S, sub, A, A, 1.0, gp, tab, acc, be, d.C);
      } else if (CM > 2 && d.C > 2 && PPCX_WAVE_ANY(two)) {
        double ec[CM];
        ec[0] = 1.0;
        double a_lo = A, a_hi = A;
#pragma unroll
        for (int cc = 1; cc < CM; ++cc) {
          ec[cc] = (two && cc < d.C) ? v.at(V_C0, coef_index(d, cc, g)) : 1.0;
          a_lo = ec[cc] < 1.0 ? a_lo * ec[cc] : a_lo; a_hi = ec[cc] > 1.0 ? a_hi * ec[cc] : a_hi;
        }
        const double A1 = A * ec[1];
        PPCX_SWEEP(2, a_lo, a_hi, A, A1, sX + S, ec, d.C)
      } else if (PPCX_WAVE_ANY(two)) {
        const double A1 = two ? A * v.at(V_C0, coef_index(d, 1, g)) : A;
        PPCX_SWEEP(1, (A1 < A ? A1 : A), (A1 > A ? A1 : A), A, A1, sX + S)
      } else {
        PPCX_SWEEP(0, A, A, A, A, sX)
      }
#undef PPCX_SWEEP
    }
  }
  PPCX_GSTAMP(6);
  if (!win) gw.scale = 1.0;
  cell_acc_close<CM>(gp, acc, gw.scale, &o);
  if ((GEN & 1) && lin) o.Tx[0] = o.Sr;
  if (win && sub == 0 && gw.k != 0) {
    const double kd = (double)gw.k;
    const double klog2 = fma(kd, 6.93147180369123816490e-01, kd * 1.90821492927058770002e-10);
    o.lik -= klog2 * fma(gp.phi, pre.n, pre.Sy);
    o.dph -= klog2 * pre.n;
  }
  if (tab_lane) {
    double hv = cf[CH - 1];
#pragma unroll
    for (int k = CH - 2; k >= 0; --k) hv = fma(hv, dr.x, cf[k]);
    if (NL > 1) {
      const double x3 = dr.x * dr.x * dr.x, xc = CH == 3 ? x3 : x3 * x3;
      double xp = (jch & 1) ? xc : 1.0;
      if (NL > 2) xp = (jch & 2) ? xp * (xc * xc) : xp;
      hv *= xp;
    }
    if (L == 1) {
      double h2 = cf2[CH - 1];
#pragma unroll
      for (int k = CH - 2; k >= 0; --k) h2 = fma(h2, dr.x, cf2[k]);
      o.lik += hv; o.dph += h2;
    } else if (fn == 0) o.lik += hv;
    else o.dph += hv;
  }
  if (PPCX_WAVE_ANY(!dr.in)) {
    PPCX_KEEP_BRANCH();
    if (!dr.in) {
      double F, D;
      disp_row_at(row, S, sub, L, sigma, &F, &D);
      o.lik += F; o.dph += D;
    }
  }
}

struct GeneData { double Sy, SyE, ncell, Lg1, SyX[kMaxC], SX[kMaxC]; };
template <int CM>
PPCX_HD void gene_data_load(const Dims& d, int gg, const double* Sy, const double* SyE, const double* SyXg, const double* SXg,
                            const double* ncell, const double* Lg1, GeneData& o) {
  o.Sy = Sy[gg]; o.SyE = SyE[gg]; o.ncell = ncell[gg]; o.Lg1 = Lg1[gg];
#pragma unroll
  for (int cc = 0; cc < CM; ++cc) {
    if (cc == 0 && d.x0_is_one) { o.SyX[0] = o.Sy; o.SX[0] = o.ncell; continue; }
    o.SyX[cc] = (cc < d.C) ? SyXg[(long)cc * d.G + gg] : 0.0;
    o.SX[cc] = (cc < d.C) ? SXg[(long)cc * d.G + gg] : 0.0;
  }
}
template <int CM>
PPCX_HD void gene_finish_vals(const Dims& d, const Cmd& c, const VecRef& v, const GeneCtx<CM>& x, GeneSumsV<CM>& acc,
                              const GeneData& gd, const double* p_in, const double* minv, double* part, double* pn,
                              double* gn = nullptr) {
  constexpr int NCM = CM + 1;
  if (x.fast) acc.Tx[0] = acc.Sr;
  GeneOut<CM> go;
  gene_close<CM>(d, c.hy, x.gg, x.has_slopes, x.gp, acc, gd.Sy, gd.SyE, gd.SyX, gd.SX, gd.ncell, gd.Lg1, &go);
#pragma unroll
  for (int k = 0; k < 10; ++k) part[k] = 0.0;
  bool bad = false;
#pragma unroll
  for (int j = 0; j < NCM; ++j) {
    const double gnew = j == 0 ? go.g_coef[0] : (j == 1 ? go.g_sigma_raw : go.g_coef[j >= 2 ? j - 1 : 0]);
    pn[j] = 0.0;
    if (gn) gn[j] = gnew;
    if (j < x.ncoord) {
      pn[j] = p_in[j] + 0.5 * c.eps * gnew;
      v.at(V_P0 + 3 * c.dir, x.idx[j]) = pn[j];
      v.at(V_G0 + 3 * c.dir, x.idx[j]) = gnew;
      part[PT_T1] += pn[j] * pn[j] * minv[j];
      bad = bad || !isfinite(gnew);
    }
  }
  if (x.active) {
    part[PT_LP] = go.lp;
#pragma unroll
    for (int k = 0; k < 6; ++k) part[PT_H0 + k] = go.h[k];
    part[PT_NONFINITE] = bad ? 1.0 : 0.0;
  }
}
template <int CM>
PPCX_HD void gene_finish(const Dims& d, const Cmd& c, const VecRef& v, const GeneCtx<CM>& x, GeneSumsV<CM>& acc,
                         const double* Sy, const double* SyE, const double* SyXg, const double* SXg, const double* ncell,
                         const double* Lg1, double* part, double* pn, double* minv, double* gn = nullptr) {
  constexpr int NCM = CM + 1;
  GeneData gd;
  gene_data_load<CM>(d, x.gg, Sy, SyE, SyXg, SXg, ncell, Lg1, gd);
  double p_in[NCM];
#pragma unroll
  for (int j = 0; j < NCM; ++j) {
    minv[j] = 1.0; p_in[j] = 0.0;
    if (j < x.ncoord) { minv[j] = v.at(V_MINV, x.idx[j]); p_in[j] = v.at(V_P0 + 3 * c.dir, x.idx[j]); }
  }
  gene_finish_vals<CM>(d, c, v, x, acc, gd, p_in, minv, part, pn, gn);
}

PPCX_HD void coord_update(const Dims& d, const Cmd& nc, const VecRef& v, int i, double* draws, double* T0,
                          const CoordCache* cc = nullptr) {
  const CoordVals cv = coord_pre(nc, v, i, i, global_flat(d, i), true, draws, d.D, nc.k0, nc.k1, T0, cc);
  if (nc.type == CMD_FLUSH) return;
  double qn = cv.q;
  if (nc.eps != 0.0) {
    double ph;
    kick_drift(cv.q, cv.p, cv.g, nc.eps, cv.minv, &ph, &qn);
    v.at(V_P0 + 3 * nc.dir, i) = ph;
    v.at(V_Q0 + 3 * nc.dir, i) = qn;
  }
  coord_consts(d, v, i, qn);
}

template <int CM>
PPCX_HD int gene_rare_pre(const Dims& d, const Cmd& c, const VecRef& v, const GeneCtx<CM>& x, double* draws, double* T0) {
  if ((c.pre_flags & ~kPreCommon) == 0) return ~0;
  constexpr int NCM = CM + 1;
#pragma unroll
  for (int j = 0; j < NCM; ++j) {
    if (j < x.ncoord) { const int i = x.idx[j]; (void)coord_pre<~0>(c, v, i, i, global_flat(d, i), true, draws, d.D, c.k0, c.k1, T0); }
  }
  return 0;
}
template <int CM, bool CACHED = false>
PPCX_HD void gene_coord_update(const Dims& d, const Cmd& c, const VecRef& v, GeneCtx<CM>& x, double* draws, double* T0,
                               bool consts, const CoordCache* cache = nullptr, double* p_out = nullptr,
                               double* minv_out = nullptr, bool store_p = true, int fmask = -1) {
  constexpr int NCM = CM + 1;
  if (!CACHED && fmask == -1) fmask = gene_rare_pre<CM>(d, c, v, x, draws, T0);
#pragma unroll
  for (int j = 0; j < NCM; ++j) {
    x.q[j] = 0.0;
    if (p_out) { p_out[j] = 0.0; minv_out[j] = 1.0; }
    if (j < x.ncoord) {
      const int i = x.idx[j];
      CoordVals cv;
      if (CACHED) { const CoordCache cj = cache[j]; cv = coord_pre<kPreCommon>(c, v, i, i, global_flat(d, i), true, draws, d.D, c.k0, c.k1, T0, &cj, fmask); }
      else cv = coord_pre<kPreCommon>(c, v, i, i, global_flat(d, i), true, draws, d.D, c.k0, c.k1, T0, nullptr, fmask);
      double qn = cv.q, ph = cv.p;
      if (c.type != CMD_FLUSH) {
        if (c.eps != 0.0) {
          kick_drift(cv.q, cv.p, cv.g, c.eps, cv.minv, &ph, &qn);
          if (store_p) v.at(V_P0 + 3 * c.dir, i) = ph;
          v.at(V_Q0 + 3 * c.dir, i) = qn;
        }
        if (consts) coord_consts(d, v, i, qn);
      }
      x.q[j] = qn;
      if (p_out) { p_out[j] = ph; minv_out[j] = cv.minv; }
    }
  }
}
template <int CM>
PPCX_HD void gene_spec_consts(const Dims& d, const Cmd& c, const VecRef& v, const GeneCtx<CM>& x, const double* pn,
                              const double* gn, const double* minv) {
  constexpr int NCM = CM + 1;
  const bool turn = c.next_dir != c.dir;
  const int o = 1 - c.dir;
#pragma unroll
  for (int j = 0; j < NCM; ++j) {
    if (j < x.ncoord) {
      double ph, qn;
      if (turn) kick_drift(v.at(V_Q0 + 3 * o, x.idx[j]), v.at(V_P0 + 3 * o, x.idx[j]), v.at(V_G0 + 3 * o, x.idx[j]), -c.eps, minv[j], &ph, &qn);
      else kick_drift(x.q[j], pn[j], gn[j], c.eps, minv[j], &ph, &qn);
// ... 109 lines not shown
```

### ppcseq_amd/csrc/ppcx_host.h

```cpp
#pragma once
#include <hip/hip_runtime.h>
#include <atomic>
#include <map>
#include <mutex>
#include <string>
#include <vector>
#include "../../include/ppcx.h"
#include "ppcx_kernels.h"
#include "ppcx_columns.h"

using namespace ppcx;

extern thread_local std::string g_err;
int fail(int code, const std::string& msg);
int hip_fail(hipError_t e, const char* what);
int hip_done(const char* who, hipError_t e);
#define HIPCHK(expr)                                                                       \
  do {                                                                                     \
    hipError_t e_ = (expr);                                                                \
    if (e_ != hipSuccess) return hip_fail(e_, #expr);                                      \
  } while (0)

#ifdef PPCX_TESTING
#include "ppcx_testing.h"
struct TestHooks {
  long long fail_at_round = 0; int fail_rank = -1;
  int force_generic = 0;
  int slope_cost_permille = 0;
  int trim_slack_permille = -1;
  int trim_extra_passes = 0;
  int psis_slots = 0;
  long long psis_scratch_bytes = 0;
  long long loo_scratch_bytes = 0;
  std::string rccl_lib;
};
extern TestHooks g_test;
#endif

struct ppcx_model {
  int device;
  DeviceStream stream;
  Dims d;
  int CM, L = 64;
  int L_override = 0, wgs_override = 0;
  int n_cu = 256, wgs_per_cu = 4;
  int ls_wgs_per_cu = 0;
  int nblocks_chosen = 0;
  int opt_pipelined = -1, opt_stream_groups = 0;
  ppcx_progress_fn progress = nullptr; void* progress_user = nullptr; double progress_every = 1.0;
  std::vector<char> pos_slope;
  struct Plan { int nbpc = 0; DeviceBuffer<int> d_bounds; };
  std::map<std::pair<int, int>, Plan> plans;
  std::mutex plan_mutex;
  std::vector<int32_t> counts_host;
  std::vector<char> excluded_host;
  std::vector<double> X_host, expo_host;
  DeviceBuffer<int> d_counts;
  DeviceBuffer<double> d_E, d_expo, d_X, d_Sy, d_SyE, d_SyX, d_SX, d_ncell, d_Lg1;
  DeviceBuffer<double> d_disp;
  DeviceBuffer<unsigned char> d_gflags;
  DispFit fit;
  DeviceBuffer<double> d_logtab, d_wintab;
  double e_min = 1.0, e_max = 1.0;
  DeviceBuffer<int> d_order;
  int live_fits = 0;
  bool destroy_requested = false;
};

struct ppcx_fit {
  ppcx_model* m;
  NutsConfig cfg;
  int chains, n_keep, iter;
  DeviceBuffer<double> d_draws;
  DeviceBuffer<double> d_lp, d_stepsize, d_accept;
  DeviceBuffer<int> d_treedepth, d_nleap, d_div;
  double seconds = 0; long long grad_evals = 0;
  double kA_ms_mean = 0; long long kA_samples = 0; double kA_chain_launches_mean = 0;
  double kC_ms_mean = 0, kU_ms_mean = 0; long long launch_triples = 0;
  double advi_elbo = 0, advi_eta = 0; int advi_converged = 0;
  double ppc_ms = 0; long long ppc_draws = 0;
  long long xchg_ticks = 0, xchg_count = 0;
  std::vector<double> inv_metric;
  bool advi = false;
  DeviceBuffer<double> d_mu, d_omega;
  DeviceBuffer<double> d_log_p, d_log_g, d_r;
};
inline void fit_attach(ppcx_fit* f, ppcx_model* m) { f->m = m; m->live_fits++; }

struct Work {
  DeviceStream own;
  hipStream_t stream = nullptr;
  DeviceBuffer<double> vecs, hyper_vecs[2], partials, t0[2], sums, red;
  DeviceBuffer<Cmd> cmds[2]; DeviceBuffer<ChainState> states[2]; DeviceBuffer<int> done;
  PinnedBuffer<int> done_host;
  long Dpad = 0; int nb_update = 1, nb_close = 1; long launches = 0;
  bool pipelined = false;
  bool shared_chip = false;
  std::atomic<int>* stop = nullptr;
  DeviceBuffer<int> active; PinnedBuffer<int> active_host; int n_active = 0;
  const XchgArgs* xchg = nullptr; int xchg_chain0 = 0;
};
struct RunIO {
  double* draws = nullptr; long draws_stride = 0; int n_keep = 0, iter = 0;
  double *lp = nullptr, *stepsize = nullptr, *accept = nullptr; int *treedepth = nullptr, *nleap = nullptr, *div = nullptr;
};
inline ChainState* current_states(Work& w) { return w.states[w.launches & 1].p; }
inline double* current_hyper(Work& w) { return w.hyper_vecs[w.launches & 1].p; }

struct PumpStats { double kA_ms_sum = 0, kC_ms_sum = 0, kU_ms_sum = 0; long long kA_samples = 0; double chain_launches = 0; long long pairs = 0; };
struct Shard { ppcx_model* m; Work* w; RunIO io; };

void choose_launch(ppcx_model* m, int nchains);
int fit_stream_groups(const ppcx_model* m, int nch);
int fit_launch_chains(const ppcx_model* m, int nch);
int plan_launch(ppcx_model* m, int nch, int reserve, bool trim, int* nbpc, const int** d_bounds);
bool model_pipelines(const ppcx_model* m);

int work_alloc(Work& w, ppcx_model* m, int nchains);
int launch_step(ppcx_model* m, Work& w, int nchains, const RunIO& io, int phases, bool with_update = false);
int launch_update(ppcx_model* m, Work& w, int nchains, const RunIO& io);
int launch_loglik(ppcx_model* m, Work& w, int nchains);
int launch_close(ppcx_model* m, Work& w, int nchains);
int pump(std::vector<Shard>& sh, int nchains, ppcx_comm* comm, long long max_pairs, bool time_kernels, PumpStats* stats);
int pump(ppcx_model* m, Work& w, int nchains, const RunIO& io, long long max_pairs, bool time_kernels, PumpStats* stats,
         ppcx_comm* comm = nullptr);

int psis_ratios(ppcx_fit* f);
```

### ppcseq_amd/csrc/ppcx_kernels.h

```cpp
#pragma once
#include <hip/hip_runtime.h>
#include "ppcx_gene.h"

namespace ppcx {

constexpr int kLdsPad = 256;
struct LoglikArgs {
  Dims d;
  CellData cd;
  const double* sampleE;
  const double* exposure;
  const double* X;
  double* vecs;
  long Dpad;
  const Cmd* cmds;
  double* sums;
  const double* logtab;
  const double* wintab;
  const int* order;
  int lgL;
  int nchains;
  const int* active;
  int nbpc;
  const int* bounds;
#ifdef PPCX_TRACE
  unsigned long long* trace;
#endif
};
#ifdef PPCX_TRACE
constexpr int kTraceBlocks = 64, kTracePasses = 8, kTraceStamps = 8;
#endif

struct CloseArgs {
  Dims d;
  const double* Sy;
  const double* SyE;
  const double* SyX;
  const double* SX;
  const double* ncell;
  const double* Lg1;
  const double* sums;
  double* vecs; long Dpad;
  const Cmd* cmds;
  double* partials;
};

struct GeneArgs {
  CloseArgs c;
  double* draws; long draws_chain_stride;
  int spec;
};

constexpr int kMaxRanks = 16;
struct XchgArgs {
  int nranks = 1, rank = 0, max_chains = 0;
  int chain0 = 0;
  unsigned epoch = 0;
  long long timeout_ticks = 0;
  double* recv[kMaxRanks];
  unsigned long long* flags[kMaxRanks];
};
PPCX_HD long xchg_recv_index(const XchgArgs& x, int slot, int src, int chain) { return (((long)slot * x.nranks + src) * x.max_chains + x.chain0 + chain) * PT_COUNT; }
PPCX_HD long xchg_flag_index(const XchgArgs& x, int slot, int src, int chain) { return ((long)slot * x.nranks + src) * x.max_chains + x.chain0 + chain; }
PPCX_HD long xchg_abort_index(const XchgArgs& x, int src) { return 2L * x.nranks * x.max_chains + src; }
PPCX_HD size_t xchg_recv_doubles(int nranks, int max_chains) { return (size_t)2 * nranks * max_chains * PT_COUNT; }
PPCX_HD size_t xchg_flag_words(int nranks, int max_chains) { return (size_t)2 * nranks * max_chains + nranks; }

enum StepPhase : int { STEP_REDUCE = 1, STEP_ADVANCE = 2 };
struct StepArgs {
  Dims d;
  int phases;
  const ChainState* states_in; ChainState* states_out;
  const Cmd* cmds_in; Cmd* cmds_out;
  const double* hyper_in; double* hyper_out;
  const double* partials; int nblocks_close;
  int slab_stride;
  const double* t0; int nblocks_update;
  double* red;
  double* draws; long draws_chain_stride;
  int n_keep, iter;
  double* out_lp; double* out_stepsize; int* out_treedepth; int* out_n_leapfrog; int* out_divergent; double* out_accept;
  int* done;
  double* upd_vecs; long upd_Dpad; double* upd_t0_out;
  XchgArgs x;
};

constexpr int kMaxShards = 16;
struct ShardSumArgs { double* bufs[kMaxShards]; int n_shards; int n; };

struct UpdateArgs {
  Dims d;
  const Cmd* cmds;
  double* vecs; long Dpad;
  double* draws; long draws_chain_stride;
  double* t0_out;
};

enum AdviOp : int { ADVI_DRAW = 0, ADVI_RESET = 1, ADVI_STEP = 2 };
struct AdviArgs {
  Dims d;
  double* vecs; long Dpad;
  double* hyper;
  Cmd* cmds;
  const double* red;
  int op, n_slots, first_iter;
  double eta_scaled;
  uint32_t k0, prev_draw, draw_base;
  double* out_draws; int out_row0;
  double* omega_part;
};
struct AdviElboArgs { Dims d; const Cmd* cmds; const double* red; int n_slots; double* acc; const double* omega_part; int n_omega_parts; };

struct PpcArgs {
  Dims d;
  const double* draws;
  long n_draws;
  const double* exposure; const double* X;
  double truncation_compensation, p_lo, p_hi;
  uint32_t k0;
  int n_gen, resample, n_cells;
  double* ci;
  int* counts_rng;
  int* scratch;
};

hipError_t launch_loglik_kernel(int CM, const LoglikArgs& a, hipStream_t st);
int loglik_resident_workgroups_per_cu(int CM, const Dims& d);
size_t loglik_lds_bytes(const Dims& d);
hipError_t launch_close_kernel(int CM, const CloseArgs& a, int nblocks, int nchains, hipStream_t st);
hipError_t launch_ls_kernel(int CM, const LoglikArgs& a, const StepArgs& sa, int n_srun, int n_chains_total, int spec, hipStream_t st,
                            hipEvent_t ev_start = nullptr, hipEvent_t ev_stop = nullptr);
int ls_resident_workgroups_per_cu(int CM, const Dims& d);
hipError_t launch_gene_kernel(int CM, const GeneArgs& a, int nblocks, int nchains, hipStream_t st);
hipError_t launch_step_kernel(const StepArgs& a, int nblocks, int nchains, hipStream_t st);
hipError_t launch_sum_shards_kernel(const ShardSumArgs& a, hipStream_t st);
hipError_t launch_update_kernel(const UpdateArgs& a, int nblocks, int nchains, hipStream_t st);
hipError_t launch_advi_kernel(const AdviArgs& a, int nblocks, hipStream_t st);
hipError_t launch_advi_elbo_kernel(const AdviElboArgs& a, hipStream_t st);
hipError_t launch_disp_build_kernel(const int* counts, int G, int S, const int* genes, int n_genes, const DispFit& fit, double* table, hipStream_t st);
hipError_t launch_gather_kernel(const double* draws, long n_rows, int D, const int* cols, int n_cols, double* out, hipStream_t st);
hipError_t launch_fill_kernel(double* p, long n, double val, hipStream_t st);

constexpr int kSummaryLdsDraws = 8192;
constexpr int kSummaryMaxChains = 128;
struct SummaryArgs {
  const double* x;
  int n_cols, M, n;
  int npad;
  double* out;
  double* scratch; long slice;
};
int summary_npad(int M, int n);
long summary_slice_doubles(int M, int n);
size_t summary_lds_bytes(int M, int n);
hipError_t launch_summary_gather_kernel(const double* draws, const double* lp, long rows, int D, const int* cols, int n_cols, double* out, hipStream_t st);
hipError_t launch_summary_kernel(const SummaryArgs& a, int nblocks, hipStream_t st);
constexpr size_t kSummaryScratchBytes = (size_t)256 << 20;
hipError_t summary_columns(const double* draws, const double* lp, int M, int n, int D, int n_cols, const int* cols, double* out,
                           size_t scratch_bytes, hipStream_t st);

constexpr int kPsisLdsDraws = 4096;
constexpr int kPsisMaxSel = 4096;
constexpr size_t kPsisScratchBytes = (size_t)256 << 20;
struct PsisArgs {
  double* x;
  const double* r;
  const int* cols;
  int n_cols; long n;
  int sel_pad;
  double* out;
};
int psis_sel_pad(long n);
hipError_t launch_psis_approx_kernel(const Dims& d, const double* sq, const double* sg, const double* hyper, double* mu, double* omega,
                                     hipStream_t st);
hipError_t launch_psis_stage_kernel(const Dims& d, const double* draws, long row0, int n_slots, double* vecs, long Dpad, Cmd* cmds,
                                    hipStream_t st);
hipError_t launch_psis_record_kernel(const Dims& d, const Cmd* cmds, const double* red, int n_slots, double* log_p, hipStream_t st);
hipError_t launch_psis_log_g_kernel(const double* draws, long rows, int D, const double* mu, const double* omega, const double* log_p,
                                    double* log_g, double* r, hipStream_t st);
hipError_t launch_psis_kernel(const PsisArgs& a, hipStream_t st);
hipError_t psis_columns(const double* draws, const double* r, long n, int D, int n_cols, const int* cols, double* khat,
                        size_t scratch_bytes, hipStream_t st);
struct LooArgs {
  const double* T = nullptr;
  const int* y = nullptr;
  const double* expo = nullptr;
  const double* X = nullptr;
  int S = 1, C = 1;
  const double* cols = nullptr;
  const int* excl = nullptr;
  const double* r_eff = nullptr;
  const double* lr = nullptr;
  long n = 0;
  int cell0 = 0, n_cells = 0;
  double* scratch = nullptr;
  int sel_pad = 0;
  double* out = nullptr;
};
int loo_sel_pad(long n, double r_eff_min);
hipError_t launch_loo_table_kernel(const double* draws, long n_draws, const Dims& d, const int* genes, int n_genes, double* T,
                                   hipStream_t st);
struct FitCells {
  const double* draws = nullptr;
  long n = 0;
  int chains = 0, n_keep = 0;
  Dims d{};
  const double* expo = nullptr;
  const double* X = nullptr;
  int n_genes = 0;
  const int* genes = nullptr;
  const int* yenc = nullptr;
  const double* r_eff = nullptr;
  double r_eff_min = 1.0;
  const double* log_ratio = nullptr;
};
hipError_t ppc_fit(PpcArgs a, double* ci, int32_t* counts_rng, float* kernel_ms, hipStream_t st);
struct GivenCells {
  const double* cols = nullptr; long n = 0; int n_cols = 0;
  int chains = 0, n_keep = 0;
  const int* excl = nullptr;
  const double* r_eff = nullptr; double r_eff_min = 1.0;
  const double* log_ratio = nullptr;
};
hipError_t loo_fit_cells(const FitCells& fc, int fields, double* out, size_t scratch_bytes, hipStream_t st);
hipError_t loo_columns(const GivenCells& gc, int fields, double* out, size_t scratch_bytes, hipStream_t st);
hipError_t loo_fit_log_lik(const FitCells& fc, double* out, size_t scratch_bytes, hipStream_t st);
hipError_t loo_predict_fit_cells(const FitCells& fc, double tc, double p_lo, double p_hi, uint32_t k0, double* out,
                                 size_t scratch_bytes, hipStream_t st);
hipError_t loo_predict_columns(const GivenCells& gc, const int* x, const int* y, double p_lo, double p_hi, double* out,
                               size_t scratch_bytes, hipStream_t st);
hipError_t ppc_exact_fit_cells(const FitCells& fc, double tc, double p_lo, double p_hi, double* out, size_t scratch_bytes,
                               hipStream_t st);
hipError_t ppc_exact_columns(const GivenCells& gc, const double* sigma_raw, const int* y, double tc, double p_lo, double p_hi,
                             double* out, size_t scratch_bytes, hipStream_t st);
struct ReffArgs { LooArgs l; int chains = 0, n_keep = 0; };
hipError_t reff_fit_cells(const FitCells& fc, double* out, size_t scratch_bytes, hipStream_t st);
hipError_t reff_columns(const GivenCells& gc, double* out, size_t scratch_bytes, hipStream_t st);
hipError_t launch_xchg_abort_kernel(const XchgArgs& x, hipStream_t st);

}
```

### ppcseq_amd/csrc/ppcx_kernels.hip

```cpp
#include <hip/hip_runtime.h>
#include <hip/hip_ext.h>
#include "ppcx_gene.h"
#include "ppcx_kernels.h"

namespace ppcx {

typedef int __attribute__((may_alias)) word_t;
typedef double2 __attribute__((may_alias)) dpair_t;

#ifndef PPCX_LOGLIK_OCC
#define PPCX_LOGLIK_OCC 2
#endif
#ifndef PPCX_LOGLIK_OCC_FAST
#define PPCX_LOGLIK_OCC_FAST 4
#endif
__device__ __forceinline__ double wave_xor_add_rt(double v, int lane_xor_mask) {
  const int src = (int)((threadIdx.x ^ (unsigned)lane_xor_mask) & 63u) << 2;
  const int lo = __builtin_amdgcn_ds_bpermute(src, __double2loint(v));
  const int hi = __builtin_amdgcn_ds_bpermute(src, __double2hiint(v));
  return v + __hiloint2double(hi, lo);
}
template <int CTRL, int ROW_MASK>
__device__ __forceinline__ double dpp_take(double v) {
  const int lo = __builtin_amdgcn_update_dpp(0, __double2loint(v), CTRL, ROW_MASK, 0xf, true);
  const int hi = __builtin_amdgcn_update_dpp(0, __double2hiint(v), CTRL, ROW_MASK, 0xf, true);
  return __hiloint2double(hi, lo);
}
template <int L>
__device__ __forceinline__ double group_sum(double v) {
  if (L >= 2) v += dpp_take<0xB1, 0xf>(v);
  if (L >= 4) v += dpp_take<0x4E, 0xf>(v);
  if (L >= 8) v += dpp_take<0x141, 0xf>(v);
  if (L >= 16) v += dpp_take<0x140, 0xf>(v);
  if (L >= 32) v = wave_xor_add_rt(v, 16);
  if (L >= 64) v = wave_xor_add_rt(v, 32);
  return v;
}
template <int CM, int LG, int GEN>
__device__ __forceinline__ void loglik_passes(const LoglikArgs& a, const Cmd& c, const VecRef& v, double* sums, int p0, int p1,
                                              const double* stab, const double* swin, const double* sE, const double* sExpo, const double* sX,
                                              int lane, bool any_generic) {
  constexpr int L = 1 << LG, GPW = 64 >> LG;
  const Dims& d = a.d;
  const int sub = lane & (L - 1), gl = lane >> LG;
  int g_cur = a.order[p0 + gl < p1 ? p0 + gl : p1 - 1];
  int g_next = a.order[p0 + GPW + gl < p1 ? p0 + GPW + gl : p1 - 1];
  GenePre pre_cur = gene_pre_load(d, v, a.cd, g_cur);
#ifdef PPCX_TRACE
  unsigned long long* tr = nullptr;
  if (a.trace && lane == 0 && (blockIdx.x % 16) == 0 && blockIdx.x / 16 < kTraceBlocks)
    tr = a.trace + (((long)(blockIdx.x / 16) * 4 + (threadIdx.x >> 6)) * kTracePasses) * kTraceStamps;
  int tpass = 0;
#define PPCX_STAMP(k) do { if (tr && tpass < kTracePasses) tr[tpass * kTraceStamps + (k)] = __builtin_readcyclecounter(); } while (0)
#else
#define PPCX_STAMP(k) ((void)0)
#endif
  for (int p = p0; p < p1; p += GPW) {
    PPCX_STAMP(0);
#ifdef PPCX_TRACE
    if (tr && tpass < kTracePasses) tr[tpass * kTraceStamps + 7] = __builtin_amdgcn_s_memrealtime();
#endif
#ifdef PPCX_PRIO_BALANCE
    {
      const int rem = (p1 - p + GPW - 1) / GPW;
      if (rem >= 4) __builtin_amdgcn_s_setprio(3); else if (rem == 3) __builtin_amdgcn_s_setprio(2); else if (rem == 2) __builtin_amdgcn_s_setprio(1); else __builtin_amdgcn_s_setprio(0);
    }
#endif
    const bool act = p + gl < p1;
    const int g = g_cur;
    const GenePre pre = pre_cur;
    if (p + GPW < p1) {
      g_cur = g_next;
      pre_cur = gene_pre_load(d, v, a.cd, g_next);
      const int pn = p + 2 * GPW + gl;
      g_next = a.order[pn < p1 ? pn : p1 - 1];
    }
    if (CM > 2 && d.x0_is_one && !PPCX_WAVE_ANY(g < d.K)) {
      GeneSumsV<2> o2;
      lane_gene_sums<2, L, 0>(d, c, v, a.cd, g, pre, sub, sE, sExpo, sX, stab, swin, o2);
      o2.lik = group_sum<L>(o2.lik); o2.dph = group_sum<L>(o2.dph); o2.Sr = group_sum<L>(o2.Sr);
      if (act && sub == 0) { const long G = d.G; sums[0 * G + g] = o2.lik; sums[1 * G + g] = o2.dph; sums[2 * G + g] = o2.Sr; }
      continue;
    }
    GeneSumsV<CM> o;
    PPCX_STAMP(1);
#ifdef PPCX_TRACE
    lane_gene_sums<CM, L, GEN>(d, c, v, a.cd, g, pre, sub, sE, sExpo, sX, stab, swin, o, (tr && tpass < kTracePasses) ? tr + tpass * kTraceStamps : nullptr);
#else
    lane_gene_sums<CM, L, GEN>(d, c, v, a.cd, g, pre, sub, sE, sExpo, sX, stab, swin, o);
#endif
    PPCX_STAMP(2);
    const bool with_tx = any_generic && (!d.x0_is_one || PPCX_WAVE_ANY(g < d.K));
    o.lik = group_sum<L>(o.lik); o.dph = group_sum<L>(o.dph); o.Sr = group_sum<L>(o.Sr);
    PPCX_STAMP(3);
    if (with_tx) {
#pragma unroll
      for (int cc = 0; cc < CM; ++cc) if (cc < d.C) o.Tx[cc] = group_sum<L>(o.Tx[cc]);
    }
    if (act && sub == 0) {
      const long G = d.G;
      sums[0 * G + g] = o.lik; sums[1 * G + g] = o.dph; sums[2 * G + g] = o.Sr;
      if (with_tx) {
#pragma unroll
        for (int cc = 0; cc < CM; ++cc) if (cc < d.C) sums[(3 + cc) * G + g] = o.Tx[cc];
      }
    }
    PPCX_STAMP(4);
#ifdef PPCX_TRACE
    ++tpass;
#endif
  }
#undef PPCX_STAMP
}

template <int CM, int GEN, bool PIPE>
__device__ __forceinline__ void loglik_role(const LoglikArgs& a, int jb, int col, double* lds) {
  if (jb >= a.nbpc) return;
  constexpr int NS = GeneSums<CM>::N;
  const Dims& d = a.d;
  const int S = d.S, C = d.C;
  const int tid = threadIdx.x;
  const int wave = tid >> 6, lane = tid & 63;
  static_assert(2 * kLogTabSize == 2 * 256, "one 16-byte request per thread fills the table");
  const bool any_generic = !d.x0_is_one || (C >= 2 && d.K > 0);
  const bool evenS = (S & 1) == 0;
  const int p0 = a.bounds[jb * 4 + wave], p1 = a.bounds[jb * 4 + wave + 1];
  const double2 f_tab = reinterpret_cast<const dpair_t*>(a.logtab)[tid];
  static_assert(2 * kWinTabSize == 4 * 2 * 256, "four 16-byte requests per thread fill the window table");
  double2 f_win[4];
#pragma unroll
  for (int k = 0; k < 4; ++k) f_win[k] = reinterpret_cast<const dpair_t*>(a.wintab)[tid + 256 * k];
  double2 f_e = {0.0, 0.0};
  if (evenS) { if (tid < S / 2) f_e = reinterpret_cast<const dpair_t*>(a.sampleE)[tid]; }
  else if (tid < S) f_e.x = a.sampleE[tid];
  double f_x = 0.0;
  if (GEN != 2 && any_generic && tid < S) f_x = a.X[S + tid];
  const int chain = a.active ? a.active[col] : col;
  const Cmd& c = a.cmds[chain];
  if (c.type == CMD_DONE || c.type == CMD_FLUSH) return;
  if (PIPE) {
    if (c.evaluated && c.type != CMD_LEAF) return;
  }
  double* stab = lds;
  double* swin = lds + 2 * kLogTabSize;
  double* sE = swin + 2 * kWinTabSize;
  double* sExpo = GEN == 2 ? sE + S + kLdsPad : nullptr;
  double* sX = GEN == 2 ? sExpo + S : sE + kLdsPad;
  const VecRef v{a.vecs + (long)chain * V_COUNT * a.Dpad, a.Dpad};
  double* sums = a.sums + (long)chain * NS * d.G;
  reinterpret_cast<dpair_t*>(stab)[tid] = f_tab;
#pragma unroll
  for (int k = 0; k < 4; ++k) reinterpret_cast<dpair_t*>(swin)[tid + 256 * k] = f_win[k];
  if (evenS) {
    if (tid < S / 2) reinterpret_cast<dpair_t*>(sE)[tid] = f_e;
    for (int i = tid + 256; i < S / 2; i += 256) reinterpret_cast<dpair_t*>(sE)[i] = reinterpret_cast<const dpair_t*>(a.sampleE)[i];
  } else {
    if (tid < S) sE[tid] = f_e.x;
    for (int i = tid + 256; i < S; i += 256) sE[i] = a.sampleE[i];
  }
  if (any_generic) {
    if (GEN == 2) {
      for (int i = tid; i < S; i += 256) sExpo[i] = a.exposure[i];
      for (int i = tid; i < S * C; i += 256) sX[i] = a.X[i];
    } else {
      if (tid < S) sX[S + tid] = f_x;
      for (int i = tid + 256; i < S; i += 256) sX[S + i] = a.X[S + i];
      for (int i = 2 * S + tid; i < S * C; i += 256) sX[i] = a.X[i];
    }
  }
  __syncthreads();
  if (p0 >= p1) return;
  switch (a.lgL) {
    case 0: loglik_passes<CM, 0, GEN>(a, c, v, sums, p0, p1, stab, swin, sE, sExpo, sX, lane, any_generic); break;
    case 1: loglik_passes<CM, 1, GEN>(a, c, v, sums, p0, p1, stab, swin, sE, sExpo, sX, lane, any_generic); break;
    case 2: loglik_passes<CM, 2, GEN>(a, c, v, sums, p0, p1, stab, swin, sE, sExpo, sX, lane, any_generic); break;
    case 3: loglik_passes<CM, 3, GEN>(a, c, v, sums, p0, p1, stab, swin, sE, sExpo, sX, lane, any_generic); break;
    case 4: loglik_passes<CM, 4, GEN>(a, c, v, sums, p0, p1, stab, swin, sE, sExpo, sX, lane, any_generic); break;
    case 5: loglik_passes<CM, 5, GEN>(a, c, v, sums, p0, p1, stab, swin, sE, sExpo, sX, lane, any_generic); break;
    default: loglik_passes<CM, 6, GEN>(a, c, v, sums, p0, p1, stab, swin, sE, sExpo, sX, lane, any_generic); break;
  }
}

template <int CM, int GEN>
__global__ __launch_bounds__(256, GEN ? PPCX_LOGLIK_OCC : PPCX_LOGLIK_OCC_FAST) void ppcx_loglik_kernel(LoglikArgs a) {
  extern __shared__ double lds[];
  const int nch = a.nchains;
  const int lin = blockIdx.x, run = lin / (8 * nch), r = lin - run * (8 * nch);
  loglik_role<CM, GEN, false>(a, run * 8 + (r & 7), r >> 3, lds);
}

__device__ __forceinline__ double wave_sum_to_lane63(double v) {
  v += dpp_take<0x111, 0xf>(v);
  v += dpp_take<0x112, 0xf>(v);
  v += dpp_take<0x114, 0xf>(v);
  v += dpp_take<0x118, 0xf>(v);
  v += dpp_take<0x142, 0xa>(v);
  v += dpp_take<0x143, 0xc>(v);
  return v;
}
template <int N>
__device__ __forceinline__ void block_accumulate(double* vals, double* wacc, int wave, int lane) {
#pragma unroll
  for (int k = 0; k < N; ++k) vals[k] = wave_sum_to_lane63(vals[k]);
  if (lane == 63) {
#pragma unroll
    for (int k = 0; k < N; ++k) wacc[wave * PT_COUNT + k] = vals[k];
  }
}

constexpr int kRowStride = 65, kPartStride = 16, kRowsPerWave = 16;
template <int N>
__device__ __forceinline__ void wave_sums_lds(const double* vals, double* rows, double* out , int lane) {
  static_assert(N >= 1 && N <= kRowsPerWave, "one batch");
#pragma unroll
  for (int k = 0; k < N; ++k) rows[k * kRowStride + lane + (kPartStride - 16) * (lane >> 4)] = vals[k];
  __builtin_amdgcn_fence(__ATOMIC_RELEASE, "wavefront");
  __builtin_amdgcn_wave_barrier();
  const int k = lane >> 2, part = lane & 3;
  double t = 0.0;
  if (k < N) {
    const double* r = rows + k * kRowStride + kPartStride * part;
    double b[8];
#pragma unroll
// ... 555 lines not shown
  __syncthreads();
  gene_block_finish(c, do_update, do_close, wacc, a.partials + ((long)chain * gridDim.x + blockIdx.x) * PT_COUNT, tid);
}

__global__ void ppcx_sum_shards_kernel(ShardSumArgs a) {
  const int i = blockIdx.x * blockDim.x + threadIdx.x;
  if (i >= a.n) return;
  double s = 0.0;
  for (int k = 0; k < a.n_shards; ++k) s += a.bufs[k][i];
  for (int k = 0; k < a.n_shards; ++k) a.bufs[k][i] = s;
}

__global__ __launch_bounds__(256) void ppcx_update_kernel(UpdateArgs a) {
  __shared__ double sT0[256];
  const int chain = blockIdx.y, tid = threadIdx.x;
  const Cmd& nc = a.cmds[chain];
  const Dims& d = a.d;
  double T0 = 0.0;
  if (nc.type != CMD_DONE) {
    const VecRef v{a.vecs + (long)chain * V_COUNT * a.Dpad, a.Dpad};
    double* draws = a.draws ? a.draws + (long)chain * a.draws_chain_stride : nullptr;
    for (int i = 3 + blockIdx.x * 256 + tid; i < d.off_tail; i += gridDim.x * 256) coord_update(d, nc, v, i, draws, &T0);
  }
  if ((nc.pre_flags & (PRE_NEW_TRANSITION | PRE_EPS_TRY)) == 0) return;
  sT0[tid] = T0;
  __syncthreads();
  for (int stp = 128; stp > 0; stp >>= 1) { if (tid < stp) sT0[tid] += sT0[tid + stp]; __syncthreads(); }
  if (tid == 0) a.t0_out[(long)chain * gridDim.x + blockIdx.x] = sT0[0];
}

__device__ __forceinline__ double advi_eta(uint32_t rid, uint32_t draw, uint32_t k0) {
  return coord_normal(rid, draw, 6u, 0u, k0, 0x41445649u);
}
__device__ __forceinline__ void advi_coord(const AdviArgs& a, double* mu, double* om, double* hm, double* ho,
                                            double mu0, double g, uint32_t rid) {
  if (a.op == ADVI_RESET) { *mu = mu0; *om = 0.0; *hm = 0.0; *ho = 0.0; }
  if (a.op == ADVI_STEP) {
    const double eta = advi_eta(rid, a.prev_draw, a.k0);
    const double gm = g, go = g * eta * exp(*om) + 1.0;
    if (isfinite(gm) && isfinite(go)) {
      *hm = a.first_iter ? gm * gm : 0.1 * gm * gm + 0.9 * *hm;
      *ho = a.first_iter ? go * go : 0.1 * go * go + 0.9 * *ho;
      *mu += a.eta_scaled * gm / (1.0 + sqrt(*hm));
      *om += a.eta_scaled * go / (1.0 + sqrt(*ho));
    }
  }
}
__global__ __launch_bounds__(256) void ppcx_advi_kernel(AdviArgs a) {
  __shared__ double s_g6[6];
  __shared__ double s_om[256];
  const Dims& d = a.d;
  const int tid = threadIdx.x;
  const VecRef v0{a.vecs, a.Dpad};
  if (a.op == ADVI_STEP && tid == 0 && blockIdx.x == 0) {
    const Cmd& c = a.cmds[0];
    const double* r = a.red;
    double g6[6];
    (void)hyper_close(d, c.hy, c.hyp_q, r[PT_LP], r + PT_H0, g6);
    for (int k = 0; k < 6; ++k) s_g6[k] = g6[k];
  }
  __syncthreads();
  double om_sum = 0.0;
  for (int i = 3 + blockIdx.x * 256 + tid; i < d.off_tail; i += gridDim.x * 256) {
    double mu = v0.at(V_SQ, i), om = v0.at(V_SG, i), hm = v0.at(V_WM, i), ho = v0.at(V_WM2, i);
    const uint32_t rid = (uint32_t)global_flat(d, i);
    const double g = a.op == ADVI_STEP ? v0.at(V_G1, i) : 0.0;
    advi_coord(a, &mu, &om, &hm, &ho, v0.at(V_Q0, i), g, rid);
    if (a.op != ADVI_DRAW) { v0.at(V_SQ, i) = mu; v0.at(V_SG, i) = om; v0.at(V_WM, i) = hm; v0.at(V_WM2, i) = ho; }
    om_sum += om;
    const double sd = exp(om);
    for (int c = 0; c < a.n_slots; ++c) {
      const double z = mu + sd * advi_eta(rid, a.draw_base + c, a.k0);
      if (a.out_draws) a.out_draws[(long)(a.out_row0 + c) * d.D + i] = z;
      else {
        a.vecs[((long)c * V_COUNT + V_Q1) * a.Dpad + i] = z;
        coord_consts(d, VecRef{a.vecs + (long)c * V_COUNT * a.Dpad, a.Dpad}, i, z);
      }
    }
  }
  if (blockIdx.x == 0 && tid < 6) {
    const int k = tid, col = hyper_index(d, k);
    double* h = a.hyper;
    double mu = h[V_SQ * 8 + k], om = h[V_SG * 8 + k], hm = h[V_WM * 8 + k], ho = h[V_WM2 * 8 + k];
    const uint32_t rid = (uint32_t)global_flat(d, col);
    advi_coord(a, &mu, &om, &hm, &ho, h[V_Q0 * 8 + k], a.op == ADVI_STEP ? s_g6[k] : 0.0, rid);
    if (a.op != ADVI_DRAW) { h[V_SQ * 8 + k] = mu; h[V_SG * 8 + k] = om; h[V_WM * 8 + k] = hm; h[V_WM2 * 8 + k] = ho; }
    om_sum += om;
    const double sd = exp(om);
    for (int c = 0; c < a.n_slots; ++c) {
      const double z = mu + sd * advi_eta(rid, a.draw_base + c, a.k0);
      if (a.out_draws) a.out_draws[(long)(a.out_row0 + c) * d.D + col] = z;
      else a.cmds[c].hyp_q[k] = z;
    }
  }
  __syncthreads();
  if (blockIdx.x == 0 && tid == 0 && !a.out_draws) {
    for (int c = 0; c < a.n_slots; ++c) {
      Cmd& cm = a.cmds[c];
      cm.type = CMD_EVAL; cm.dir = 1; cm.eps = 0.0; cm.pre_flags = 0; cm.n_merge = 0; cm.subtree_complete = 0; cm.leaf_n = 0;
      cm.hy = make_hyper(cm.hyp_q, d.lambda_mu_mu);
    }
  }
  s_om[tid] = om_sum;
  __syncthreads();
  for (int stp = 128; stp > 0; stp >>= 1) { if (tid < stp) s_om[tid] += s_om[tid + stp]; __syncthreads(); }
  if (tid == 0) a.omega_part[blockIdx.x] = s_om[0];
}

__global__ void ppcx_advi_elbo_kernel(AdviElboArgs a) {
  if (threadIdx.x != 0 || blockIdx.x != 0) return;
  for (int c = 0; c < a.n_slots; ++c) {
    const Cmd& cm = a.cmds[c];
    const double* r = a.red + (long)c * PT_COUNT;
    double g6[6];
    const double lp = hyper_close(a.d, cm.hy, cm.hyp_q, r[PT_LP], r + PT_H0, g6);
    if (isfinite(lp)) { a.acc[0] += lp; a.acc[1] += 1.0; } else a.acc[2] += 1.0;
  }
  double s = 0.0;
  for (int b = 0; b < a.n_omega_parts; ++b) s += a.omega_part[b];
  a.acc[3] = s;
}

constexpr int kDispThreads = 384;
__global__ __launch_bounds__(kDispThreads) void ppcx_disp_build_kernel(const int* counts, int G, int S, const int* genes, int n_genes,
                                                                        DispFit fit, double* table) {
  extern __shared__ int s_row[];
  const int gi = blockIdx.x;
  if (gi >= n_genes) return;
  const int g = genes ? genes[gi] : gi;
  const int tid = threadIdx.x;
  double* s_val = reinterpret_cast<double*>(s_row + ((S + 1) & ~1));
  for (int s = tid; s < S; s += kDispThreads) s_row[s] = counts[(long)g * S + s];
  __syncthreads();
  constexpr int NN = kDispPanels * kDispN;
  for (int t = tid; t < NN; t += kDispThreads) {
    const int p = t / kDispN, k = t - p * kDispN;
    double lo;
    const double sg = disp_node_sigma(fit, p, k, &lo);
    const DispPoint pt = disp_point(sg, lo);
    double F, D;
    disp_row(s_row, S, 0, 1, pt, &F, &D);
    s_val[(p * 2 + 0) * kDispN + k] = F; s_val[(p * 2 + 1) * kDispN + k] = D;
  }
  __syncthreads();
  for (int t = tid; t < 2 * kDispPanels; t += kDispThreads) {
    double out[kDispStride];
    disp_fit_panel(fit, s_val + t * kDispN, out);
    double* dst = table + (long)g * kDispGeneDoubles + (long)t * kDispStride;
#pragma unroll
    for (int m = 0; m < kDispStride; ++m) dst[m] = out[m];
  }
}

__global__ void ppcx_gather_kernel(const double* draws, long n_rows, int D, const int* cols, int n_cols, double* out) {
  const long i = (long)blockIdx.x * blockDim.x + threadIdx.x;
  if (i >= n_rows * n_cols) return;
  const long r = i / n_cols; const int cidx = (int)(i % n_cols);
  out[i] = draws[r * D + cols[cidx]];
}

__global__ void ppcx_xchg_abort_kernel(XchgArgs x) {
  const int k = threadIdx.x;
  if (k < x.nranks) sys_store(x.flags[k] + xchg_abort_index(x, x.rank), (unsigned long long)x.epoch);
  __threadfence_system();
}

__global__ void ppcx_fill_kernel(double* p, long n, double val) {
  const long i = (long)blockIdx.x * blockDim.x + threadIdx.x;
  if (i < n) p[i] = val;
}

static int loglik_generic_possible(const Dims& d) { return !d.x0_is_one ? 2 : ((d.C >= 2 && d.K > 0 && !d.x1_binary) ? 1 : 0); }
size_t loglik_lds_bytes(const Dims& d) {
  const size_t per_sample = loglik_generic_possible(d) == 2 ? (size_t)(2 + d.C) : (size_t)(d.C < 1 ? 1 : d.C);
  return sizeof(double) * (2 * kLogTabSize + 2 * kWinTabSize + (size_t)d.S * per_sample + 2 * kLdsPad);
}
#define PPCX_BY_CM_GEN(KERNEL, CM, GEN, EXPR)                                                                     \
  do {                                                                                                            \
    if ((CM) <= 2) { if ((GEN) == 0) { auto k_ = KERNEL<2, 0>; EXPR; } else if ((GEN) == 1) { auto k_ = KERNEL<2, 1>; EXPR; } else { auto k_ = KERNEL<2, 2>; EXPR; } } \
    else if ((CM) <= 4) { if ((GEN) == 0) { auto k_ = KERNEL<4, 0>; EXPR; } else if ((GEN) == 1) { auto k_ = KERNEL<4, 1>; EXPR; } else { auto k_ = KERNEL<4, 2>; EXPR; } } \
    else if ((CM) <= 8) { if ((GEN) == 0) { auto k_ = KERNEL<8, 0>; EXPR; } else if ((GEN) == 1) { auto k_ = KERNEL<8, 1>; EXPR; } else { auto k_ = KERNEL<8, 2>; EXPR; } } \
    else { auto k_ = KERNEL<16, 0>; EXPR; }    \
  } while (0)
static const void* loglik_kernel_ptr(int CM, int gen) {
  const void* f = nullptr;
  PPCX_BY_CM_GEN(ppcx_loglik_kernel, CM, gen, f = (const void*)k_);
  return f;
}
int loglik_resident_workgroups_per_cu(int CM, const Dims& d) {
  int n = 0;
  const size_t lds_bytes = loglik_lds_bytes(d);
  const int gen = loglik_generic_possible(d);
  const void* f = loglik_kernel_ptr(CM, gen);
  if (lds_bytes > 64u * 1024u) {
    if (hipFuncSetAttribute(f, hipFuncAttributeMaxDynamicSharedMemorySize, (int)lds_bytes) != hipSuccess) { (void)hipGetLastError(); return 0; }
  }
  hipError_t e = hipSuccess;
  PPCX_BY_CM_GEN(ppcx_loglik_kernel, CM, gen, e = hipOccupancyMaxActiveBlocksPerMultiprocessor(&n, k_, 256, lds_bytes));
  if (e != hipSuccess) { (void)hipGetLastError(); return 0; }
  return n;
}
hipError_t launch_loglik_kernel(int CM, const LoglikArgs& a, hipStream_t st) {
  const size_t lds_bytes = loglik_lds_bytes(a.d);
  const dim3 grid((unsigned)((a.nbpc + 7) / 8 * 8) * (unsigned)a.nchains);
  LoglikArgs args = a;
  void* params[] = {&args};
  return hipLaunchKernel(loglik_kernel_ptr(CM, loglik_generic_possible(a.d)), grid, dim3(256), params, lds_bytes, st);
}
hipError_t launch_close_kernel(int CM, const CloseArgs& a, int nblocks, int nchains, hipStream_t st) {
  const dim3 grid(nblocks, nchains);
  if (CM <= 2) hipLaunchKernelGGL((ppcx_close_kernel<2>), grid, dim3(256), 0, st, a);
  else if (CM <= 4) hipLaunchKernelGGL((ppcx_close_kernel<4>), grid, dim3(256), 0, st, a);
  else if (CM <= 8) hipLaunchKernelGGL((ppcx_close_kernel<8>), grid, dim3(256), 0, st, a);
  else hipLaunchKernelGGL((ppcx_close_kernel<16>), grid, dim3(256), 0, st, a);
  return hipGetLastError();
}
static const void* ls_kernel_ptr(int CM, int gen) {
  const void* f = nullptr;
  PPCX_BY_CM_GEN(ppcx_ls_kernel, CM, gen, f = (const void*)k_);
  return f;
}
static size_t ls_lds_bytes(const Dims& d) { const size_t a = loglik_lds_bytes(d); return a > sizeof(StepShared) ? a : sizeof(StepShared); }
int ls_resident_workgroups_per_cu(int CM, const Dims& d) {
  int n = 0;
  const size_t lds_bytes = ls_lds_bytes(d);
  const int gen = loglik_generic_possible(d);
  if (lds_bytes > 64u * 1024u) {
    if (hipFuncSetAttribute(ls_kernel_ptr(CM, gen), hipFuncAttributeMaxDynamicSharedMemorySize, (int)lds_bytes) != hipSuccess) { (void)hipGetLastError(); return 0; }
  }
  hipError_t e = hipSuccess;
  PPCX_BY_CM_GEN(ppcx_ls_kernel, CM, gen, e = hipOccupancyMaxActiveBlocksPerMultiprocessor(&n, k_, 256, lds_bytes));
  if (e != hipSuccess) { (void)hipGetLastError(); return 0; }
  return n;
}
hipError_t launch_ls_kernel(int CM, const LoglikArgs& a, const StepArgs& sa, int n_srun, int n_chains_total, int spec, hipStream_t st,
                            hipEvent_t ev_start, hipEvent_t ev_stop) {
  const size_t lds_bytes = ls_lds_bytes(a.d);
  int runs = n_srun;
  if (a.nbpc > 7 * n_srun) runs += (a.nbpc - 7 * n_srun + 7) / 8;
  const dim3 grid((unsigned)runs * 8u * (unsigned)a.nchains);
  LoglikArgs args = a; StepArgs sargs = sa;
  void* params[] = {&args, &sargs, &n_srun, &n_chains_total, &spec};
  if (ev_start && ev_stop)
    return hipExtLaunchKernel(ls_kernel_ptr(CM, loglik_generic_possible(a.d)), grid, dim3(256), params, lds_bytes, st, ev_start, ev_stop, 0);
  return hipLaunchKernel(ls_kernel_ptr(CM, loglik_generic_possible(a.d)), grid, dim3(256), params, lds_bytes, st);
}
hipError_t launch_gene_kernel(int CM, const GeneArgs& a, int nblocks, int nchains, hipStream_t st) {
  const dim3 grid(nblocks, nchains);
  if (CM <= 2) hipLaunchKernelGGL((ppcx_gene_kernel<2>), grid, dim3(256), 0, st, a);
  else if (CM <= 4) hipLaunchKernelGGL((ppcx_gene_kernel<4>), grid, dim3(256), 0, st, a);
  else if (CM <= 8) hipLaunchKernelGGL((ppcx_gene_kernel<8>), grid, dim3(256), 0, st, a);
  else hipLaunchKernelGGL((ppcx_gene_kernel<16>), grid, dim3(256), 0, st, a);
  return hipGetLastError();
}
hipError_t launch_step_kernel(const StepArgs& a, int nblocks, int nchains, hipStream_t st) {
  hipLaunchKernelGGL(ppcx_step_kernel, dim3(a.upd_vecs ? nblocks : 1, nchains), dim3(256), 0, st, a);
  return hipGetLastError();
}
hipError_t launch_sum_shards_kernel(const ShardSumArgs& a, hipStream_t st) {
  hipLaunchKernelGGL(ppcx_sum_shards_kernel, dim3((a.n + 255) / 256), dim3(256), 0, st, a);
  return hipGetLastError();
}
hipError_t launch_update_kernel(const UpdateArgs& a, int nblocks, int nchains, hipStream_t st) {
  hipLaunchKernelGGL(ppcx_update_kernel, dim3(nblocks, nchains), dim3(256), 0, st, a);
  return hipGetLastError();
}
hipError_t launch_advi_kernel(const AdviArgs& a, int nblocks, hipStream_t st) {
  hipLaunchKernelGGL(ppcx_advi_kernel, dim3(nblocks), dim3(256), 0, st, a);
  return hipGetLastError();
}
hipError_t launch_advi_elbo_kernel(const AdviElboArgs& a, hipStream_t st) {
  hipLaunchKernelGGL(ppcx_advi_elbo_kernel, dim3(1), dim3(64), 0, st, a);
  return hipGetLastError();
}
size_t disp_build_lds_bytes(int S) { return sizeof(int) * (size_t)((S + 1) & ~1) + sizeof(double) * 2 * kDispPanels * kDispN; }
hipError_t launch_disp_build_kernel(const int* counts, int G, int S, const int* genes, int n_genes, const DispFit& fit, double* table, hipStream_t st) {
  const size_t lds = disp_build_lds_bytes(S);
  if (lds > 64u * 1024u) {
    hipError_t e = hipFuncSetAttribute((const void*)ppcx_disp_build_kernel, hipFuncAttributeMaxDynamicSharedMemorySize, (int)lds);
    if (e != hipSuccess) return e;
  }
  hipLaunchKernelGGL(ppcx_disp_build_kernel, dim3((unsigned)n_genes), dim3(kDispThreads), lds, st, counts, G, S, genes, n_genes, fit, table);
  return hipGetLastError();
}
hipError_t launch_gather_kernel(const double* draws, long n_rows, int D, const int* cols, int n_cols, double* out, hipStream_t st) {
  const long n = n_rows * n_cols;
  hipLaunchKernelGGL(ppcx_gather_kernel, dim3((unsigned)((n + 255) / 256)), dim3(256), 0, st, draws, n_rows, D, cols, n_cols, out);
  return hipGetLastError();
}
hipError_t launch_xchg_abort_kernel(const XchgArgs& x, hipStream_t st) {
  hipLaunchKernelGGL(ppcx_xchg_abort_kernel, dim3(1), dim3(64), 0, st, x);
  return hipGetLastError();
}
hipError_t launch_fill_kernel(double* p, long n, double val, hipStream_t st) {
  hipLaunchKernelGGL(ppcx_fill_kernel, dim3((unsigned)((n + 255) / 256)), dim3(256), 0, st, p, n, val);
  return hipGetLastError();
}

}
```

### ppcseq_amd/csrc/ppcx_run.hip

```cpp
#include <stdio.h>
#include <stdlib.h>
#include <string.h>
#include <chrono>
#include <dlfcn.h>
#include "ppcx_host.h"

#ifdef PPCX_TRACE
static unsigned long long* g_trace_dev = nullptr;
#endif
int work_alloc(Work& w, ppcx_model* m, int nchains) {
  const int D = m->d.D;
  if (!w.stream) w.stream = m->stream.s;
  w.Dpad = ((long)D + 31) / 32 * 32;
  w.nb_update = (D + 255) / 256;
  if (w.nb_update > 80) w.nb_update = 80;
  if (w.nb_update < 1) w.nb_update = 1;
  HIPCHK(w.vecs.alloc((size_t)nchains * V_COUNT * w.Dpad));
  w.nb_close = (m->d.G + 255) / 256;
  HIPCHK(w.partials.alloc((size_t)nchains * w.nb_close * PT_COUNT));
  HIPCHK(w.sums.alloc((size_t)nchains * (3 + m->CM) * m->d.G));
  HIPCHK(hipMemsetAsync(w.sums.p, 0, sizeof(double) * (size_t)nchains * (3 + m->CM) * m->d.G, w.stream));
  HIPCHK(w.done.alloc(nchains));
  HIPCHK(w.red.alloc((size_t)nchains * PT_COUNT));
  HIPCHK(hipMemsetAsync(w.red.p, 0, sizeof(double) * (size_t)nchains * PT_COUNT, w.stream));
  HIPCHK(w.done_host.alloc(2 * nchains));
  HIPCHK(w.active_host.alloc(nchains));
  HIPCHK(w.active.alloc(nchains));
  for (int i = 0; i < 2; ++i) {
    HIPCHK(w.hyper_vecs[i].alloc((size_t)nchains * V_COUNT * 8));
    HIPCHK(w.t0[i].alloc((size_t)nchains * w.nb_update));
    HIPCHK(w.cmds[i].alloc(nchains));
    HIPCHK(w.states[i].alloc(nchains));
    HIPCHK(hipMemsetAsync(w.hyper_vecs[i].p, 0, sizeof(double) * (size_t)nchains * V_COUNT * 8, w.stream));
    HIPCHK(hipMemsetAsync(w.t0[i].p, 0, sizeof(double) * (size_t)nchains * w.nb_update, w.stream));
    HIPCHK(hipMemsetAsync(w.cmds[i].p, 0, sizeof(Cmd) * nchains, w.stream));
    HIPCHK(hipMemsetAsync(w.states[i].p, 0, sizeof(ChainState) * nchains, w.stream));
  }
  HIPCHK(hipMemsetAsync(w.vecs.p, 0, sizeof(double) * (size_t)nchains * V_COUNT * w.Dpad, w.stream));
  HIPCHK(hipMemsetAsync(w.partials.p, 0, sizeof(double) * (size_t)nchains * w.nb_close * PT_COUNT, w.stream));
  HIPCHK(hipMemsetAsync(w.done.p, 0, sizeof(int) * nchains, w.stream));
  for (int c = 0; c < nchains; ++c) {
    HIPCHK(launch_fill_kernel(w.vecs.p + ((size_t)c * V_COUNT + V_MINV) * w.Dpad, w.Dpad, 1.0, w.stream));
    HIPCHK(launch_fill_kernel(w.hyper_vecs[0].p + ((size_t)c * V_COUNT + V_MINV) * 8, 8, 1.0, w.stream));
  }
  w.launches = 0;
  HIPCHK(hipStreamSynchronize(w.stream));
  return PPCX_OK;
}

static void step_args(ppcx_model* m, Work& w, const RunIO& io, int phases, bool with_update, StepArgs* o) {
  const int in = (int)(w.launches & 1), out = in ^ 1;
  StepArgs& sa = *o;
  sa.d = m->d; sa.phases = phases;
  sa.states_in = w.states[in].p; sa.states_out = w.states[out].p;
  sa.cmds_in = w.cmds[in].p; sa.cmds_out = w.cmds[out].p;
  sa.hyper_in = w.hyper_vecs[in].p; sa.hyper_out = w.hyper_vecs[out].p;
  sa.partials = w.partials.p; sa.nblocks_close = w.nb_close; sa.slab_stride = w.nb_close; sa.t0 = w.t0[in].p; sa.nblocks_update = w.nb_update; sa.red = w.red.p;
  sa.draws = io.draws; sa.draws_chain_stride = io.draws_stride; sa.n_keep = io.n_keep; sa.iter = io.iter;
  sa.out_lp = io.lp; sa.out_stepsize = io.stepsize; sa.out_treedepth = io.treedepth; sa.out_n_leapfrog = io.nleap;
  sa.out_divergent = io.div; sa.out_accept = io.accept; sa.done = w.done.p;
  sa.upd_vecs = nullptr; sa.upd_Dpad = 0; sa.upd_t0_out = nullptr;
  sa.x = XchgArgs();
  if (w.xchg) {
    sa.x = *w.xchg;
    sa.x.chain0 = w.xchg_chain0;
  }
  if (with_update && (phases & STEP_ADVANCE)) { sa.upd_vecs = w.vecs.p; sa.upd_Dpad = w.Dpad; sa.upd_t0_out = w.t0[out].p; }
}
int launch_step(ppcx_model* m, Work& w, int nchains, const RunIO& io, int phases, bool with_update) {
  StepArgs sa;
  step_args(m, w, io, phases, with_update, &sa);
  hipError_t e = launch_step_kernel(sa, w.nb_update, nchains, w.stream);
  if (e != hipSuccess) return fail(PPCX_ERR_HIP, std::string("step kernel: ") + hipGetErrorString(e));
  if (phases & STEP_ADVANCE) w.launches++;
  return PPCX_OK;
}
int launch_update(ppcx_model* m, Work& w, int nchains, const RunIO& io) {
  UpdateArgs ua;
  ua.d = m->d; ua.cmds = w.cmds[w.launches & 1].p; ua.vecs = w.vecs.p; ua.Dpad = w.Dpad;
  ua.draws = io.draws; ua.draws_chain_stride = io.draws_stride; ua.t0_out = w.t0[w.launches & 1].p;
  hipError_t e = launch_update_kernel(ua, w.nb_update, nchains, w.stream);
  if (e != hipSuccess) return fail(PPCX_ERR_HIP, std::string("update kernel: ") + hipGetErrorString(e));
  return PPCX_OK;
}
static int step_runs(int nchains, int nact) { return (nchains + nact - 1) / nact; }
static int loglik_args(ppcx_model* m, Work& w, int nchains, int reserve, LoglikArgs* out) {
  const int nact = w.n_active > 0 ? w.n_active : nchains;
  LoglikArgs& la = *out;
  int rc = plan_launch(m, nact, reserve, w.shared_chip, &la.nbpc, &la.bounds);
  if (rc != PPCX_OK) return rc;
  la.d = m->d; la.cd.counts = m->d_counts.p; la.cd.disp = m->d_disp.p; la.cd.gflags = m->d_gflags.p; la.cd.Sy = m->d_Sy.p; la.cd.ncell = m->d_ncell.p; la.cd.e_min = m->e_min; la.cd.e_max = m->e_max; la.sampleE = m->d_E.p; la.exposure = m->d_expo.p; la.X = m->d_X.p;
  la.vecs = w.vecs.p; la.Dpad = w.Dpad; la.cmds = w.cmds[w.launches & 1].p; la.sums = w.sums.p; la.logtab = m->d_logtab.p; la.wintab = m->d_wintab.p; la.order = m->d_order.p;
  la.lgL = 0; while ((1 << la.lgL) < m->L) ++la.lgL;
  la.nchains = nact; la.active = w.n_active > 0 ? w.active.p : nullptr;
#ifdef PPCX_TRACE
  la.trace = g_trace_dev;
#endif
  return PPCX_OK;
}
int launch_loglik(ppcx_model* m, Work& w, int nchains) {
  LoglikArgs la;
  int rc = loglik_args(m, w, nchains, 0, &la);
  if (rc != PPCX_OK) return rc;
  hipError_t e = launch_loglik_kernel(m->CM, la, w.stream);
  if (e != hipSuccess) return fail(PPCX_ERR_HIP, std::string("loglik kernel: ") + hipGetErrorString(e));
  return PPCX_OK;
}
static void close_args(ppcx_model* m, Work& w, CloseArgs* o) {
  CloseArgs& ca = *o;
  ca.d = m->d; ca.Sy = m->d_Sy.p; ca.SyE = m->d_SyE.p; ca.SyX = m->d_SyX.p; ca.SX = m->d_SX.p; ca.ncell = m->d_ncell.p; ca.Lg1 = m->d_Lg1.p;
  ca.sums = w.sums.p; ca.vecs = w.vecs.p; ca.Dpad = w.Dpad; ca.cmds = w.cmds[w.launches & 1].p; ca.partials = w.partials.p;
}
static int launch_ls(ppcx_model* m, Work& w, int nchains, const RunIO& io, hipEvent_t ev_start = nullptr, hipEvent_t ev_stop = nullptr) {
  const int nact = w.n_active > 0 ? w.n_active : nchains;
  const int n_srun = step_runs(nchains, nact);
  LoglikArgs la;
  int rc = loglik_args(m, w, nchains, n_srun * nact, &la);
  if (rc != PPCX_OK) return rc;
  StepArgs sa;
  step_args(m, w, io, STEP_REDUCE | STEP_ADVANCE, false, &sa);
  hipError_t e = launch_ls_kernel(m->CM, la, sa, n_srun, nchains, 1, w.stream, ev_start, ev_stop);
  if (e != hipSuccess) return fail(PPCX_ERR_HIP, std::string("merged log-likelihood / step kernel: ") + hipGetErrorString(e));
  w.launches++;
  return PPCX_OK;
}
static int launch_gene_round(ppcx_model* m, Work& w, int nchains, const RunIO& io, int spec = 1) {
  GeneArgs ga;
  close_args(m, w, &ga.c);
  ga.draws = io.draws; ga.draws_chain_stride = io.draws_stride; ga.spec = spec;
  hipError_t e = launch_gene_kernel(m->CM, ga, w.nb_close, nchains, w.stream);
  if (e != hipSuccess) return fail(PPCX_ERR_HIP, std::string("gene kernel: ") + hipGetErrorString(e));
  return PPCX_OK;
}
int launch_close(ppcx_model* m, Work& w, int nchains) {
  CloseArgs ca;
  close_args(m, w, &ca);
  hipError_t e = launch_close_kernel(m->CM, ca, w.nb_close, nchains, w.stream);
  if (e != hipSuccess) return fail(PPCX_ERR_HIP, std::string("close kernel: ") + hipGetErrorString(e));
  return PPCX_OK;
}

typedef struct ncclComm* ncclComm_t;
typedef struct { char internal[128]; } ncclUniqueId_t;
struct RcclApi {
  void* h = nullptr;
  int (*GetUniqueId)(ncclUniqueId_t*) = nullptr;
  int (*CommInitRank)(ncclComm_t*, int, ncclUniqueId_t, int) = nullptr;
  int (*CommDestroy)(ncclComm_t) = nullptr;
  int (*AllReduce)(const void*, void*, size_t, int, int, ncclComm_t, hipStream_t) = nullptr;
  const char* (*GetErrorString)(int) = nullptr;
};
static RcclApi g_rccl;
static int rccl_load() {
  if (g_rccl.h) return PPCX_OK;
#ifdef PPCX_TESTING
  if (!g_test.rccl_lib.empty()) {
    g_rccl.h = dlopen(g_test.rccl_lib.c_str(), RTLD_NOW | RTLD_LOCAL);
    if (!g_rccl.h) return fail(PPCX_ERR_HIP, std::string("cannot load the nccl provider ") + g_test.rccl_lib + ": " + dlerror());
  }
#endif
  if (!g_rccl.h) {
    const char* names[] = {"librccl.so.1", "librccl.so", "/opt/rocm/lib/librccl.so.1"};
    for (const char* n : names) { g_rccl.h = dlopen(n, RTLD_NOW | RTLD_GLOBAL); if (g_rccl.h) break; }
  }
  if (!g_rccl.h) return fail(PPCX_ERR_HIP, "cannot load librccl.so");
  g_rccl.GetUniqueId = (int (*)(ncclUniqueId_t*))dlsym(g_rccl.h, "ncclGetUniqueId");
  g_rccl.CommInitRank = (int (*)(ncclComm_t*, int, ncclUniqueId_t, int))dlsym(g_rccl.h, "ncclCommInitRank");
  g_rccl.CommDestroy = (int (*)(ncclComm_t))dlsym(g_rccl.h, "ncclCommDestroy");
  g_rccl.AllReduce = (int (*)(const void*, void*, size_t, int, int, ncclComm_t, hipStream_t))dlsym(g_rccl.h, "ncclAllReduce");
  g_rccl.GetErrorString = (const char* (*)(int))dlsym(g_rccl.h, "ncclGetErrorString");
  if (!g_rccl.GetUniqueId || !g_rccl.CommInitRank || !g_rccl.CommDestroy || !g_rccl.AllReduce) return fail(PPCX_ERR_HIP, "librccl.so lacks the expected symbols");
  return PPCX_OK;
}
static std::string rccl_error(int e) { return g_rccl.GetErrorString ? g_rccl.GetErrorString(e) : "error"; }
struct ppcx_comm { ncclComm_t comm = nullptr; int nranks = 1, rank = 0, device = 0; DeviceBuffer<double> d_guard; PinnedBuffer<double> h_guard; };
static int guard_decision(const double* g, int local_rc) {
  if (g[4] != 0.0) return local_rc != PPCX_OK ? local_rc : -(int)g[4];
  if (g[0] != -g[1] || g[2] != -g[3]) return PPCX_ERR_STALL;
  return PPCX_OK;
}
extern "C" int ppcx_guard_decision(const double* reduced5, int local_rc) { return reduced5 ? guard_decision(reduced5, local_rc) : PPCX_ERR_ARG; }
static int comm_guard(ppcx_comm* c, hipStream_t st, long long pairs, int n_done, int local_rc, int* all_rc) {
  double* v = c->h_guard.p;
  v[0] = (double)pairs; v[1] = -(double)pairs; v[2] = (double)n_done; v[3] = -(double)n_done; v[4] = local_rc != PPCX_OK ? (double)(-local_rc) : 0.0;
  const std::string local_msg = g_err;
  hipError_t he = hipMemcpyAsync(c->d_guard.p, v, sizeof(double) * 5, hipMemcpyHostToDevice, st);
  const int e = g_rccl.AllReduce(c->d_guard.p, c->d_guard.p, 5,  8,  2, c->comm, st);
  if (e != 0) return fail(PPCX_ERR_HIP, std::string("ncclAllReduce (guard): ") + rccl_error(e));
  if (he == hipSuccess) he = hipMemcpyAsync(c->h_guard.p + 8, c->d_guard.p, sizeof(double) * 5, hipMemcpyDeviceToHost, st);
  if (he == hipSuccess) he = hipStreamSynchronize(st);
  if (he != hipSuccess) return fail(PPCX_ERR_HIP, std::string("guard exchange: ") + hipGetErrorString(he));
  const int d = guard_decision(c->h_guard.p + 8, local_rc);
  *all_rc = d;
  if (d != PPCX_OK) {
    if (local_rc != PPCX_OK) g_err = local_msg;
    else if (d == PPCX_ERR_STALL) g_err = "the ranks of the gene-sharded run disagree on the rounds issued or the chains finished";
    else g_err = "another rank of the gene-sharded run reported an error";
  }
  return PPCX_OK;
}
extern "C" int ppcx_comm_unique_id(char* out128) {
  if (!out128) return fail(PPCX_ERR_ARG, "NULL buffer");
  int rc = rccl_load();
  if (rc != PPCX_OK) return rc;
  ncclUniqueId_t id;
  const int e = g_rccl.GetUniqueId(&id);
  if (e != 0) return fail(PPCX_ERR_HIP, "ncclGetUniqueId failed");
  memcpy(out128, id.internal, 128);
  return PPCX_OK;
}
extern "C" int ppcx_comm_create(int device, int nranks, int rank, const char* id128, ppcx_comm** out) {
  if (!out || !id128 || nranks < 1 || rank < 0 || rank >= nranks) return fail(PPCX_ERR_ARG, "bad communicator arguments");
  *out = nullptr;
  int rc = rccl_load();
  if (rc != PPCX_OK) return rc;
  HIPCHK(hipSetDevice(device));
  ncclUniqueId_t id; memcpy(id.internal, id128, 128);
  ppcx_comm* c = new ppcx_comm();
  c->nranks = nranks; c->rank = rank; c->device = device;
  const int e = g_rccl.CommInitRank(&c->comm, nranks, id, rank);
  if (e != 0) { delete c; return fail(PPCX_ERR_HIP, std::string("ncclCommInitRank: ") + rccl_error(e)); }
  if (c->d_guard.alloc(8) != hipSuccess || c->h_guard.alloc(16) != hipSuccess) {
    ppcx_comm_destroy(c); return fail(PPCX_ERR_HIP, "allocating the communicator's guard buffers failed");
  }
  *out = c;
  return PPCX_OK;
}
extern "C" void ppcx_comm_destroy(ppcx_comm* c) {
  if (!c) return;
  if (c->comm && g_rccl.CommDestroy) (void)g_rccl.CommDestroy(c->comm);
  delete c;
}

int pump(std::vector<Shard>& sh, int nchains, ppcx_comm* comm, long long max_pairs, bool time_kernels, PumpStats* stats) {
  const int ns = (int)sh.size();
  hipStream_t st = sh[0].w->stream;
  int rc = PPCX_OK;
  const bool guarded = comm && comm->comm && comm->nranks > 1;
  const bool piped = ns == 1 && !(comm && comm->comm) && sh[0].w->pipelined;
  int local_rc = PPCX_OK;
#define PUMP_TRY(expr) do { if (local_rc == PPCX_OK) { const int r_ = (expr); if (r_ != PPCX_OK) { if (!guarded) return r_; local_rc = r_; } } } while (0)
#define PUMP_HIP(expr) do { if (local_rc == PPCX_OK) { const hipError_t e_ = (expr); if (e_ != hipSuccess) { const int r_ = fail(PPCX_ERR_HIP, std::string(#expr) + ": " + hipGetErrorString(e_)); if (!guarded) return r_; local_rc = r_; } } } while (0)
  if (!piped) for (int k = 0; k < ns; ++k) {
    PUMP_TRY(launch_step(sh[k].m, *sh[k].w, nchains, sh[k].io, STEP_REDUCE | STEP_ADVANCE));
    PUMP_TRY(launch_update(sh[k].m, *sh[k].w, nchains, sh[k].io));
// ... 274 lines not shown
```

### ppcseq_amd/csrc/ppcx_testing.h

```cpp
#ifndef PPCX_TESTING_H
#define PPCX_TESTING_H
#include "../../include/ppcx.h"
#ifdef __cplusplus
extern "C" {
#endif
PPCX_API int ppcx_testing_set(const char* key, long long value);
PPCX_API int ppcx_testing_set_nccl_provider(const char* path);
enum { PPCX_BENCH_LOGLIK = 0, PPCX_BENCH_CLOSE = 1, PPCX_BENCH_LOGLIK_CLOSE = 2, PPCX_BENCH_STEP = 3, PPCX_BENCH_UPDATE = 4,
       PPCX_BENCH_STEP_REDUCE = 5, PPCX_BENCH_STEP_ADVANCE = 6, PPCX_BENCH_STEP_UPDATE = 7,
       PPCX_BENCH_GENE = 8,
       PPCX_BENCH_GENE_NO_PROP = 9,
       PPCX_BENCH_GENE_NO_SPEC = 10,
       PPCX_BENCH_GENE_UPDATE_ONLY = 11,
       PPCX_BENCH_GENE_NEW_TRANSITION = 12 };
PPCX_API int ppcx_testing_bench_kernel(ppcx_model* m, int which, int nchains, int warm_rounds, int reps, int n_merge,
                                       double* ms_per_launch, int* cmd_type);
PPCX_API int ppcx_testing_sm_trace(double* out6);
enum { PPCX_MATH_FAST_RCP = 0, PPCX_MATH_FAST_LOG = 1, PPCX_MATH_FAST_EXP = 2, PPCX_MATH_TABLE_LOG = 3, PPCX_MATH_WINDOW_LOG = 4,
       PPCX_MATH_STIRLING_TAILS = 5, PPCX_MATH_STIRLING_EXCESS = 6, PPCX_MATH_LOG_ERFC_RATIO = 7, PPCX_MATH_CELL = 8,
       PPCX_MATH_CELL_WIN = 9, PPCX_MATH_CELL_Y = 10, PPCX_MATH_CELL_WIN_Y = 11, PPCX_MATH_SINCOS_2PI = 12, PPCX_MATH_LGAMMA_INT1 = 13,
       PPCX_MATH_RNG_EXP = 14, PPCX_MATH_RNG_DIV = 15, PPCX_MATH_NB2_TAILS = 16, PPCX_MATH_COUNT = 17 };
PPCX_API int ppcx_testing_eval_math(int fn, int n, const double* a, const double* b, const int* y, double* out0, double* out1);
PPCX_API int ppcx_testing_get_disp_table(ppcx_model* m, double* out);
PPCX_API int ppcx_testing_psis(int n, int n_cols, const double* lr, const double* cols, double* khat);
PPCX_API int ppcx_testing_loo(int n, int n_cols, const double* ll, const int32_t* excluded, const double* r_eff, double* out);
PPCX_API int ppcx_testing_loo_mcse(int n, int n_cols, const double* ll, const int32_t* excluded, const double* r_eff, double* out);
PPCX_API int ppcx_testing_loo_predict(const double* ll, const int32_t* x, int n, int n_cols, const int32_t* y, const int32_t* excluded,
                                      const double* r_eff, double p_lo, double p_hi, double* out);
PPCX_API int ppcx_testing_loo_approx(int n, int n_cols, const double* ll, const double* log_ratio, const int32_t* excluded, double* out);
PPCX_API int ppcx_testing_loo_predict_approx(const double* ll, const double* log_ratio, const int32_t* x, int n, int n_cols,
                                             const int32_t* y, const int32_t* excluded, double p_lo, double p_hi, double* out);
PPCX_API int ppcx_testing_relative_eff(int chains, int n, int n_cols, const double* ll, double* out);
PPCX_API int ppcx_testing_ppc_exact(int n, int n_cols, const double* eta, const double* sigma_raw, const int32_t* y,
                                    const int32_t* excluded, double truncation_compensation, double p_lo, double p_hi, double* out);
#ifdef __cplusplus
}
#endif
#endif
```

Before: 437.1 ESS/s.

## Replace per-sample likelihood sweep with per-gene polynomial tables over intercept+sigma

```diff
diff --git a/include/ppcx.h b/include/ppcx.h
--- a/include/ppcx.h
+++ b/include/ppcx.h
@@ -34,6 +34,8 @@
                       ppcx_model** out);
 PPCX_API int ppcx_model_set_exclusions(ppcx_model* m, int n_excl, const int32_t* excl);
 PPCX_API int ppcx_model_set_launch(ppcx_model* m, int lanes_per_gene, int workgroups);
+PPCX_API int ppcx_model_set_sample_tables(ppcx_model* m, int on);
+PPCX_API int ppcx_model_get_sample_tables(const ppcx_model* m, int* on, int* tabulated, int* refused);
 PPCX_API int ppcx_model_get_launch(const ppcx_model* m, int* lanes_per_gene, int* nblocks);
 PPCX_API int ppcx_model_set_rounds(ppcx_model* m, int pipelined, int stream_groups);
 typedef int (*ppcx_progress_fn)(void* user, int first_chain, int chains, int chains_done, long long rounds, double seconds);
diff --git a/ppcseq_amd/_lib.py b/ppcseq_amd/_lib.py
--- a/ppcseq_amd/_lib.py
+++ b/ppcseq_amd/_lib.py
@@ -21,7 +21,7 @@
     "ppcx_fit_nuts_xchg", "ppcx_fit_get_xchg_timing", "ppcx_fit_get_inv_metric", "ppcx_fit_summary",
     "ppcx_fit_get_approximation", "ppcx_fit_get_log_ratios", "ppcx_fit_psis", "ppcx_fit_get_log_lik", "ppcx_fit_loo",
     "ppcx_fit_loo_predict", "ppcx_fit_relative_eff", "ppcx_fit_loo_mcse", "ppcx_fit_loo_approx", "ppcx_fit_loo_predict_approx",
-    "ppcx_fit_ppc_exact",
+    "ppcx_fit_ppc_exact", "ppcx_model_set_sample_tables", "ppcx_model_get_sample_tables",
 ]
 ABI_VERSION = 400
 SUMMARY_FIELDS = ("mean", "sd", "q05", "q50", "q95", "rhat", "ess_bulk", "ess_tail")
@@ -110,6 +110,8 @@
     lib.ppcx_fit_ppc.argtypes = [C.c_void_p, C.c_double, C.c_double, C.c_double, C.c_ulonglong, C.c_int, C.c_int, dp, ip]
     lib.ppcx_fit_free.argtypes = [C.c_void_p]
     lib.ppcx_model_set_rounds.argtypes = [C.c_void_p, C.c_int, C.c_int]
+    lib.ppcx_model_set_sample_tables.argtypes = [C.c_void_p, C.c_int]
+    lib.ppcx_model_get_sample_tables.argtypes = [C.c_void_p, C.POINTER(C.c_int), C.POINTER(C.c_int), C.POINTER(C.c_int)]
     lib.ppcx_xchg_create.argtypes = [C.c_int, C.c_int, C.c_int, C.c_int, C.POINTER(C.c_void_p)]
     lib.ppcx_xchg_handle.argtypes = [C.c_void_p, C.c_char_p]
     lib.ppcx_xchg_connect.argtypes = [C.c_void_p, C.c_char_p]
@@ -129,6 +131,8 @@
         lib.ppcx_testing_eval_math.argtypes = [C.c_int, C.c_int, dp, dp, ip, dp, dp]
     if hasattr(lib, "ppcx_testing_get_disp_table"):
         lib.ppcx_testing_get_disp_table.argtypes = [C.c_void_p, dp]
+    if hasattr(lib, "ppcx_testing_get_samp"):
+        lib.ppcx_testing_get_samp.argtypes = [C.c_void_p, dp, C.POINTER(C.c_ubyte), C.POINTER(C.c_longlong), C.c_int]
     if hasattr(lib, "ppcx_testing_psis"):
         lib.ppcx_testing_psis.argtypes = [C.c_int, C.c_int, dp, dp, dp]
     if hasattr(lib, "ppcx_testing_loo"):
@@ -446,6 +450,27 @@
         _check(lib.ppcx_testing_get_disp_table(self._h, _p(out, C.c_double)))
         return out
 
+    def set_sample_tables(self, on=True):
+        _check(load().ppcx_model_set_sample_tables(self._h, 1 if on else 0))
+
+    def get_sample_tables(self):
+        a, b, c = C.c_int(), C.c_int(), C.c_int()
+        _check(load().ppcx_model_get_sample_tables(self._h, C.byref(a), C.byref(b), C.byref(c)))
+        return bool(a.value), b.value, c.value
+
+    def testing_samp(self, table=False, reset=False):
+        lib = load()
+        if not hasattr(lib, "ppcx_testing_get_samp"):
+            raise PpcxError(f"{LIB_PATH} is not the testing build")
+        flags = np.zeros(self.G, np.uint8)
+        st = np.zeros(5, np.int64)
+        tab = np.zeros((self.G, 64, 4, 12)) if table else None
+        _check(lib.ppcx_testing_get_samp(self._h, _p(tab, C.c_double), _p(flags, C.c_ubyte), _p(st, C.c_longlong), 1 if reset else 0))
+        out = dict(flags=flags, tabulated=int(st[0]), refused=int(st[1]), served=int(st[2]), swept=int(st[3]), allocated=bool(st[4]))
+        if table:
+            out["table"] = tab
+        return out
+
     def log_prob_grad(self, u):
         u = np.ascontiguousarray(u, dtype=np.float64)
         one = u.ndim == 1
diff --git a/ppcseq_amd/build.py b/ppcseq_amd/build.py
--- a/ppcseq_amd/build.py
+++ b/ppcseq_amd/build.py
@@ -12,7 +12,7 @@
 SOURCES = ["ppcx_kernels.hip", "ppcx_summary.hip", "ppcx_psis.hip", "ppcx_loo.hip", "ppcx_loo_predict.hip", "ppcx_reff.hip", "ppcx_ppc_exact.hip", "ppcx_ppc.hip",
            "ppcx_capi.hip", "ppcx_run.hip", "ppcx_fit_nuts.hip", "ppcx_fit_advi.hip", "ppcx_fit_api.hip"]
 TESTING_SOURCES = ["ppcx_testing_math.hip"]
-HEADERS = ["ppcx_math.h", "ppcx_disp.h", "ppcx_model.h", "ppcx_nuts.h", "ppcx_gene.h", "ppcx_kernels.h", "ppcx_summary.h", "ppcx_summary_dev.h", "ppcx_psis.h", "ppcx_psis_dev.h", "ppcx_loo.h", "ppcx_loo_ap.h", "ppcx_loo_dev.h", "ppcx_loo_predict.h", "ppcx_reff.h", "ppcx_nbcdf.h", "ppcx_ppc_exact.h", "ppcx_ppc.h", "ppcx_table.h", "ppcx_block.h", "ppcx_columns.h", "ppcx_host.h", "ppcx_testing.h",
+HEADERS = ["ppcx_math.h", "ppcx_disp.h", "ppcx_samp.h", "ppcx_model.h", "ppcx_nuts.h", "ppcx_gene.h", "ppcx_kernels.h", "ppcx_summary.h", "ppcx_summary_dev.h", "ppcx_psis.h", "ppcx_psis_dev.h", "ppcx_loo.h", "ppcx_loo_ap.h", "ppcx_loo_dev.h", "ppcx_loo_predict.h", "ppcx_reff.h", "ppcx_nbcdf.h", "ppcx_ppc_exact.h", "ppcx_ppc.h", "ppcx_table.h", "ppcx_block.h", "ppcx_columns.h", "ppcx_host.h", "ppcx_testing.h",
            os.path.join("..", "..", "include", "ppcx.h")]
 
 
diff --git a/ppcseq_amd/csrc/ppcx_capi.hip b/ppcseq_amd/csrc/ppcx_capi.hip
--- a/ppcseq_amd/csrc/ppcx_capi.hip
+++ b/ppcseq_amd/csrc/ppcx_capi.hip
@@ -29,6 +29,7 @@
   return PPCX_OK;
 }
 
+constexpr double kTabPassSweep = 3.0;
 static double pass_cost(const ppcx_model* m, int L, int p, int n) {
   const int S = m->d.S;
   bool slope = false;
@@ -42,7 +43,9 @@
   if (g_test.slope_cost_permille > 0) lin_w = 1e-3 * g_test.slope_cost_permille;
 #endif
   const double sweep = (double)((S + L - 1) / L) * (!m->d.x0_is_one ? 2.5 : (slope && !m->d.x1_binary ? lin_w : (slope ? slope_w : 1.0)));
-  return 5.8 + sweep;
+  bool tab = !m->pos_tab.empty();
+  for (int i = p; i < p + n && tab; ++i) tab = m->pos_tab[i];
+  return 5.8 + (tab ? kTabPassSweep : sweep);
 }
 static int resident_workgroups(const ppcx_model* m, int reserve) {
   int n = m->wgs_override > 0 ? m->wgs_override : m->n_cu * (reserve > 0 ? m->ls_wgs_per_cu : m->wgs_per_cu);
@@ -138,6 +141,46 @@
   ppcx_model::Plan& pl = m->plans[key];
   pl.nbpc = nbpc; std::swap(pl.d_bounds.p, d_bounds.p);
   *nbpc_out = pl.nbpc; *d_bounds_out = pl.d_bounds.p;
+  return PPCX_OK;
+}
+
+static bool samp_possible(const ppcx_model* m) {
+  const Dims& d = m->d;
+  return m->opt_samp && d.x0_is_one && !(d.C >= 2 && d.K > 0 && !d.x1_binary) && samp_build_lds_bytes(d.S) <= 160u * 1024u;
+}
+static int samp_rebuild(ppcx_model* m) {
+  const int G = m->d.G, S = m->d.S, K = m->d.K, C = m->d.C;
+  std::vector<unsigned char>& fl = m->gflags_host;
+  int n_elig = 0;
+  for (int g = 0; g < G; ++g) {
+    fl[g] &= 1;
+    if (samp_possible(m) && !(g < K && C >= 2) && !(fl[g] & 1)) { fl[g] |= 2; ++n_elig; }
+  }
+  if (n_elig > 0 && !m->d_samp.p) {
+    if (m->d_samp.alloc((size_t)G * kSampGeneDoubles) != hipSuccess) {
+      (void)hipGetLastError(); m->d_samp.p = nullptr; n_elig = 0;
+      for (int g = 0; g < G; ++g) fl[g] &= 1;
+    }
+  }
+  if (n_elig == 0 && m->d_samp.p) { HIPCHK(hipStreamSynchronize(m->stream.s)); HIPCHK(hipFree(m->d_samp.p)); m->d_samp.p = nullptr; }
+  HIPCHK(hipMemcpy(m->d_gflags.p, fl.data(), (size_t)G, hipMemcpyHostToDevice));
+  m->samp_tabulated = 0; m->samp_refused = 0;
+  if (n_elig > 0) {
+    int pg = -1, pa = -1;
+#ifdef PPCX_TESTING
+    pg = g_test.samp_perturb_gene; pa = g_test.samp_perturb_at;
+#endif
+    const hipError_t e = launch_samp_build_kernel(m->d_counts.p, m->d_E.p, G, S, m->fit, m->d_samp.p, m->d_gflags.p, pg, pa, m->stream.s);
+    if (e != hipSuccess) return fail(PPCX_ERR_HIP, std::string("sample-table kernel: ") + hipGetErrorString(e));
+    HIPCHK(hipStreamSynchronize(m->stream.s));
+    HIPCHK(hipMemcpy(fl.data(), m->d_gflags.p, (size_t)G, hipMemcpyDeviceToHost));
+    for (int g = 0; g < G; ++g) m->samp_tabulated += (fl[g] & 2) ? 1 : 0;
+    m->samp_refused = n_elig - m->samp_tabulated;
+  }
+  m->d.raw_consts = (m->base_raw_consts || m->d_samp.p) ? 1 : 0;
+  m->pos_tab.assign(G, 0);
+  for (int p = 0; p < G; ++p) m->pos_tab[p] = (fl[m->order_host[p]] & 2) ? 1 : 0;
+  drop_plans(m);
   return PPCX_OK;
 }
 
@@ -192,6 +235,7 @@
     HIPCHK(hipMemcpy(m->d_order.p, ord.data(), sizeof(int) * (size_t)G, hipMemcpyHostToDevice));
     m->pos_slope.resize(G);
     for (int p = 0; p < G; ++p) m->pos_slope[p] = ord[p] < K && C >= 2;
+    m->order_host = ord;
     drop_plans(m);
   }
   HIPCHK(hipMemcpy(m->d_counts.p, cnt.data(), sizeof(int32_t) * cnt.size(), hipMemcpyHostToDevice));
@@ -201,6 +245,8 @@
     const hipError_t e = launch_disp_build_kernel(m->d_counts.p, G, S, nullptr, G, m->fit, m->d_disp.p, m->stream.s);
     if (e != hipSuccess) return fail(PPCX_ERR_HIP, std::string("dispersion-table kernel: ") + hipGetErrorString(e));
   }
+  m->gflags_host = gflags;
+  { const int rc = samp_rebuild(m); if (rc != PPCX_OK) return rc; }
   HIPCHK(hipMemcpy(m->d_Sy.p, Sy.data(), sizeof(double) * G, hipMemcpyHostToDevice));
   HIPCHK(hipMemcpy(m->d_SyE.p, SyE.data(), sizeof(double) * G, hipMemcpyHostToDevice));
   HIPCHK(hipMemcpy(m->d_SyX.p, SyX.data(), sizeof(double) * SyX.size(), hipMemcpyHostToDevice));
@@ -247,11 +293,12 @@
   if (g_test.force_generic) x1b = 0;
 #endif
   m->d.x1_binary = x1b;
-  m->d.raw_consts = (!x0 || (C >= 2 && K > 0 && !x1b)) ? 1 : 0;
+  m->d.raw_consts = m->base_raw_consts = (!x0 || (C >= 2 && K > 0 && !x1b)) ? 1 : 0;
   if (C > 8 && (!x0 || (K > 0 && !x1b)))
     return fail(PPCX_ERR_LIMIT, "more than 8 design columns are supported for designs of a column of ones and 0 / 1 indicator columns only");
   if (const char* e = getenv("PPCX_PIPELINE")) if (atoi(e) == 0) m->opt_pipelined = 0;
   if (const char* e = getenv("PPCX_STREAM_GROUPS")) { const int v = atoi(e); if (v >= 1) m->opt_stream_groups = v; }
+  if (const char* e = getenv("PPCX_SAMPLE_TABLES")) if (atoi(e) == 0) m->opt_samp = 0;
   if (loglik_lds_bytes(m->d) > 160u * 1024u)
     return fail(PPCX_ERR_LIMIT, "the per-sample constants (S * C doubles; S * (2 + C) for a design without a column of ones) do not fit the 160 KB of LDS of a compute unit beside the 20 KB of tables");
   m->wgs_per_cu = loglik_resident_workgroups_per_cu(m->CM, m->d);
@@ -281,6 +328,10 @@
   m->e_min = m->e_max = E[0];
   for (int s = 1; s < S; ++s) { if (E[s] < m->e_min) m->e_min = E[s]; if (E[s] > m->e_max) m->e_max = E[s]; }
   HIPCHK(m->d_order.alloc((size_t)G));
+#ifdef PPCX_TESTING
+  HIPCHK(m->d_samp_stat.alloc(2));
+  HIPCHK(hipMemset(m->d_samp_stat.p, 0, 2 * sizeof(unsigned long long)));
+#endif
   HIPCHK(hipMemcpy(m->d_E.p, E.data(), sizeof(double) * S, hipMemcpyHostToDevice));
   HIPCHK(hipMemcpy(m->d_expo.p, exposure, sizeof(double) * S, hipMemcpyHostToDevice));
   HIPCHK(hipMemcpy(m->d_X.p, X, sizeof(double) * (size_t)S * C, hipMemcpyHostToDevice));
@@ -314,6 +365,21 @@
   if (!m || (n_excl > 0 && !excl) || n_excl < 0) return fail(PPCX_ERR_ARG, "bad arguments");
   HIPCHK(hipSetDevice(m->device));
   return upload_counts(m, n_excl, excl);
+}
+extern "C" int ppcx_model_set_sample_tables(ppcx_model* m, int on) {
+  if (!m || on < 0 || on > 1) return fail(PPCX_ERR_ARG, "need a model and on = 0 or 1");
+  HIPCHK(hipSetDevice(m->device));
+  m->opt_samp = on;
+  const int rc = samp_rebuild(m);
+  if (rc == PPCX_OK) choose_launch(m, 1);
+  return rc;
+}
+extern "C" int ppcx_model_get_sample_tables(const ppcx_model* m, int* on, int* tabulated, int* refused) {
+  if (!m) return fail(PPCX_ERR_ARG, "model is NULL");
+  if (on) *on = m->opt_samp;
+  if (tabulated) *tabulated = m->samp_tabulated;
+  if (refused) *refused = m->samp_refused;
+  return PPCX_OK;
 }
 extern "C" int ppcx_model_set_launch(ppcx_model* m, int lanes_per_gene, int workgroups) {
   if (!m) return fail(PPCX_ERR_ARG, "model is NULL");
@@ -391,7 +457,27 @@
   else if (k == "psis_slots") g_test.psis_slots = (int)value;
   else if (k == "psis_scratch_bytes") g_test.psis_scratch_bytes = value;
   else if (k == "loo_scratch_bytes") g_test.loo_scratch_bytes = value;
+  else if (k == "samp_perturb_gene") g_test.samp_perturb_gene = (int)value;
+  else if (k == "samp_perturb_at") g_test.samp_perturb_at = (int)value;
   else return fail(PPCX_ERR_ARG, "unknown test hook " + k);
+  return PPCX_OK;
+}
+extern "C" int ppcx_testing_get_samp(ppcx_model* m, double* table, unsigned char* flags, long long* stats, int reset) {
+  if (!m) return fail(PPCX_ERR_ARG, "model is NULL");
+  HIPCHK(hipSetDevice(m->device));
+  HIPCHK(hipDeviceSynchronize());
+  if (table) {
+    if (!m->d_samp.p) return fail(PPCX_ERR_ARG, "the model holds no sample table");
+    HIPCHK(hipMemcpy(table, m->d_samp.p, sizeof(double) * (size_t)m->d.G * kSampGeneDoubles, hipMemcpyDeviceToHost));
+  }
+  if (flags) HIPCHK(hipMemcpy(flags, m->d_gflags.p, (size_t)m->d.G, hipMemcpyDeviceToHost));
+  if (stats) {
+    unsigned long long st[2];
+    HIPCHK(hipMemcpy(st, m->d_samp_stat.p, sizeof(st), hipMemcpyDeviceToHost));
+    stats[0] = m->samp_tabulated; stats[1] = m->samp_refused; stats[2] = (long long)st[0]; stats[3] = (long long)st[1];
+    stats[4] = m->d_samp.p ? 1 : 0;
+  }
+  if (reset) HIPCHK(hipMemset(m->d_samp_stat.p, 0, 2 * sizeof(unsigned long long)));
   return PPCX_OK;
 }
 extern "C" int ppcx_testing_get_disp_table(ppcx_model* m, double* out) {
diff --git a/ppcseq_amd/csrc/ppcx_gene.h b/ppcseq_amd/csrc/ppcx_gene.h
--- a/ppcseq_amd/csrc/ppcx_gene.h
+++ b/ppcseq_amd/csrc/ppcx_gene.h
@@ -1,5 +1,6 @@
 #pragma once
 #include "ppcx_nuts.h"
+#include "ppcx_samp.h"
 
 
 namespace ppcx {
@@ -63,14 +64,17 @@
   const double* Sy;
   const double* ncell;
   double e_min, e_max;
+  const double* samp = nullptr;
+  unsigned long long* samp_stat = nullptr;
 };
 
-struct GenePre { double phi, sigma, a0, Sy, n; int flags; };
+struct GenePre { double phi, sigma, a0, q0, Sy, n; int flags; };
 PPCX_HD GenePre gene_pre_load(const Dims& d, const VecRef& v, const CellData& m, int g) {
   GenePre r;
   r.phi = v.at(V_C0, d.off_sigma_raw + g);
   r.sigma = v.at(V_C2, d.off_sigma_raw + g);
   r.a0 = v.at(V_C0, d.off_intercept + g);
+  r.q0 = d.raw_consts ? v.at(V_C2, d.off_intercept + g) : 0.0;
   r.Sy = m.Sy[g]; r.n = m.ncell[g]; r.flags = m.gflags[g];
   return r;
 }
@@ -223,6 +227,16 @@
       for (int k = 0; k < CH; ++k) cf2[k] = pc[kDispStride + k];
     }
   }
+  bool stab = false;
+  if (GEN == 0) stab = m.samp != nullptr && (pre.flags & 2) != 0 && samp_in_range(pre.q0, sigma);
+  const bool all_stab = GEN == 0 && PPCX_WAVE_ALL(stab);
+#if defined(PPCX_TESTING) && defined(__HIP_DEVICE_COMPILE__)
+  if (m.samp_stat) {
+    const bool counted = sub == 0 && !(pre.flags & 128);
+    const unsigned long long n1 = __popcll(__ballot(counted && stab)), n0 = __popcll(__ballot(counted && !stab));
+    if ((threadIdx.x & 63) == 0) { if (n1) atomicAdd(m.samp_stat, n1); if (n0) atomicAdd(m.samp_stat + 1, n0); }
+  }
+#endif
   CellAcc<CM> acc; acc.zero();
   PPCX_GSTAMP(5);
   if (GEN & 2) {
@@ -232,7 +246,7 @@
   }
   GeneWindow gw; gw.k = 0; gw.ok = false; gw.scale = 1.0;
   bool win = false;
-  if (!(GEN & 2) || PPCX_WAVE_ANY(!generic)) {
+  if (!all_stab && (!(GEN & 2) || PPCX_WAVE_ANY(!generic))) {
     if (!generic) {
       const bool any_masked = PPCX_WAVE_ANY(masked);
 #define PPCX_SWEEP(MODE, A_LO, A_HI, A_, A1_, X1_, ...)                                                                  \
@@ -277,6 +291,13 @@
     const double klog2 = fma(kd, 6.93147180369123816490e-01, kd * 1.90821492927058770002e-10);
     o.lik -= klog2 * fma(gp.phi, pre.n, pre.Sy);
     o.dph -= klog2 * pre.n;
+  }
+  if (GEN == 0 && PPCX_WAVE_ANY(stab)) {
+    PPCX_KEEP_BRANCH();
+    if (stab) {
+      const SampSums ts = samp_gene_at(m.samp + (long)g * kSampGeneDoubles, pre.q0, sigma, sub, L, gp.phi, gp.invphi);
+      o.lik = ts.lik; o.dph = ts.dph; o.Sr = ts.Sr;
+    }
   }
   if (tab_lane) {
     double hv = cf[CH - 1];
diff --git a/ppcseq_amd/csrc/ppcx_host.h b/ppcseq_amd/csrc/ppcx_host.h
--- a/ppcseq_amd/csrc/ppcx_host.h
+++ b/ppcseq_amd/csrc/ppcx_host.h
@@ -32,6 +32,7 @@
   int psis_slots = 0;
   long long psis_scratch_bytes = 0;
   long long loo_scratch_bytes = 0;
+  int samp_perturb_gene = -1, samp_perturb_at = -1;
   std::string rccl_lib;
 };
 extern TestHooks g_test;
@@ -49,6 +50,7 @@
   int opt_pipelined = -1, opt_stream_groups = 0;
   ppcx_progress_fn progress = nullptr; void* progress_user = nullptr; double progress_every = 1.0;
   std::vector<char> pos_slope;
+  std::vector<char> pos_tab;
   struct Plan { int nbpc = 0; DeviceBuffer<int> d_bounds; };
   std::map<std::pair<int, int>, Plan> plans;
   std::mutex plan_mutex;
@@ -60,6 +62,15 @@
   DeviceBuffer<double> d_disp;
   DeviceBuffer<unsigned char> d_gflags;
   DispFit fit;
+  int opt_samp = 1;
+  DeviceBuffer<double> d_samp;
+  std::vector<unsigned char> gflags_host;
+  std::vector<int> order_host;
+  int base_raw_consts = 0;
+  int samp_tabulated = 0, samp_refused = 0;
+#ifdef PPCX_TESTING
+  DeviceBuffer<unsigned long long> d_samp_stat;
+#endif
   DeviceBuffer<double> d_logtab, d_wintab;
   double e_min = 1.0, e_max = 1.0;
   DeviceBuffer<int> d_order;
diff --git a/ppcseq_amd/csrc/ppcx_kernels.h b/ppcseq_amd/csrc/ppcx_kernels.h
--- a/ppcseq_amd/csrc/ppcx_kernels.h
+++ b/ppcseq_amd/csrc/ppcx_kernels.h
@@ -138,6 +138,9 @@
 hipError_t launch_advi_kernel(const AdviArgs& a, int nblocks, hipStream_t st);
 hipError_t launch_advi_elbo_kernel(const AdviElboArgs& a, hipStream_t st);
 hipError_t launch_disp_build_kernel(const int* counts, int G, int S, const int* genes, int n_genes, const DispFit& fit, double* table, hipStream_t st);
+hipError_t launch_samp_build_kernel(const int* counts, const double* E, int G, int S, const DispFit& fit, double* table, unsigned char* gflags,
+                                    int perturb_gene, int perturb_at, hipStream_t st);
+size_t samp_build_lds_bytes(int S);
 hipError_t launch_gather_kernel(const double* draws, long n_rows, int D, const int* cols, int n_cols, double* out, hipStream_t st);
 hipError_t launch_fill_kernel(double* p, long n, double val, hipStream_t st);
 
diff --git a/ppcseq_amd/csrc/ppcx_kernels.hip b/ppcseq_amd/csrc/ppcx_kernels.hip
--- a/ppcseq_amd/csrc/ppcx_kernels.hip
+++ b/ppcseq_amd/csrc/ppcx_kernels.hip
@@ -68,7 +68,12 @@
 #endif
     const bool act = p + gl < p1;
     const int g = g_cur;
+#ifdef PPCX_TESTING
+    GenePre pre = pre_cur;
+    if (!act) pre.flags |= 128;
+#else
     const GenePre pre = pre_cur;
+#endif
     if (p + GPW < p1) {
       g_cur = g_next;
       pre_cur = gene_pre_load(d, v, a.cd, g_next);
@@ -930,6 +935,50 @@
   }
 }
 
+constexpr int kSampThreads = kSampPanels * kDispN;
+__global__ __launch_bounds__(kSampThreads) void ppcx_samp_build_kernel(const int* counts, const double* E, int G, int S, DispFit fit,
+                                                                        double* table, unsigned char* gflags, int perturb_gene, int perturb_at) {
+  extern __shared__ double s_samp[];
+  const int g = blockIdx.x;
+  if (g >= G || !(gflags[g] & 2)) return;
+  const int tid = threadIdx.x;
+  constexpr int NN = kSampPanels * kDispN;
+  double* s_val = s_samp;
+  double* s_E = s_val + NN * kSampFns;
+  unsigned long long* s_worst = reinterpret_cast<unsigned long long*>(s_E + S);
+  int* s_cnt = reinterpret_cast<int*>(s_worst + 1);
+  for (int s = tid; s < S; s += kSampThreads) { s_cnt[s] = counts[(long)g * S + s]; s_E[s] = E[s]; }
+  if (tid == 0) *s_worst = 0ull;
+  __syncthreads();
+  for (int t = tid; t < NN; t += kSampThreads) {
+    const int p = t / kDispN, k = t - p * kDispN;
+    double v[kSampFns];
+    samp_node(fit, s_cnt, s_E, S, p, k, v);
+#pragma unroll
+    for (int f = 0; f < kSampFns; ++f) s_val[(p * kSampFns + f) * kDispN + k] = v[f];
+  }
+  __syncthreads();
+  double* gtab = table + (long)g * kSampGeneDoubles;
+  for (int t = tid; t < kSampFns * kSampPanels; t += kSampThreads) {
+    double out[kDispStride];
+    disp_fit_panel(fit, s_val + t * kDispN, out);
+#pragma unroll
+    for (int m = 0; m < kDispStride; ++m) {
+      if (g == perturb_gene && t * kDispStride + m == perturb_at) out[m] *= 1.0 + 1e-9;
+      gtab[(long)t * kDispStride + m] = out[m];
+    }
+  }
+  __threadfence_block();
+  __syncthreads();
+  for (int t = tid; t < kSampPanels * kSampChecks; t += kSampThreads) {
+    const int p = t / kSampChecks, j = t - p * kSampChecks;
+    const double dev = samp_check_point(fit, s_cnt, s_E, S, p, j, gtab + (long)p * kSampFns * kDispStride);
+    atomicMax(s_worst, dbl_bits(dev));
+  }
+  __syncthreads();
+  if (tid == 0 && !(bits_dbl(*s_worst) <= kSampBound)) gflags[g] = gflags[g] & (unsigned char)~2u;
+}
+
 __global__ void ppcx_gather_kernel(const double* draws, long n_rows, int D, const int* cols, int n_cols, double* out) {
   const long i = (long)blockIdx.x * blockDim.x + threadIdx.x;
   if (i >= n_rows * n_cols) return;
@@ -1061,6 +1110,17 @@
   hipLaunchKernelGGL(ppcx_disp_build_kernel, dim3((unsigned)n_genes), dim3(kDispThreads), lds, st, counts, G, S, genes, n_genes, fit, table);
   return hipGetLastError();
 }
+size_t samp_build_lds_bytes(int S) { return sizeof(double) * ((size_t)kSampPanels * kDispN * kSampFns + (size_t)S + 1) + sizeof(int) * (size_t)((S + 1) & ~1); }
+hipError_t launch_samp_build_kernel(const int* counts, const double* E, int G, int S, const DispFit& fit, double* table, unsigned char* gflags,
+                                    int perturb_gene, int perturb_at, hipStream_t st) {
+  const size_t lds = samp_build_lds_bytes(S);
+  if (lds > 64u * 1024u) {
+    hipError_t e = hipFuncSetAttribute((const void*)ppcx_samp_build_kernel, hipFuncAttributeMaxDynamicSharedMemorySize, (int)lds);
+    if (e != hipSuccess) return e;
+  }
+  hipLaunchKernelGGL(ppcx_samp_build_kernel, dim3((unsigned)G), dim3(kSampThreads), lds, st, counts, E, G, S, fit, table, gflags, perturb_gene, perturb_at);
+  return hipGetLastError();
+}
 hipError_t launch_gather_kernel(const double* draws, long n_rows, int D, const int* cols, int n_cols, double* out, hipStream_t st) {
   const long n = n_rows * n_cols;
   hipLaunchKernelGGL(ppcx_gather_kernel, dim3((unsigned)((n + 255) / 256)), dim3(256), 0, st, draws, n_rows, D, cols, n_cols, out);
diff --git a/ppcseq_amd/csrc/ppcx_run.hip b/ppcseq_amd/csrc/ppcx_run.hip
--- a/ppcseq_amd/csrc/ppcx_run.hip
+++ b/ppcseq_amd/csrc/ppcx_run.hip
@@ -89,8 +89,11 @@
   LoglikArgs& la = *out;
   int rc = plan_launch(m, nact, reserve, w.shared_chip, &la.nbpc, &la.bounds);
   if (rc != PPCX_OK) return rc;
-  la.d = m->d; la.cd.counts = m->d_counts.p; la.cd.disp = m->d_disp.p; la.cd.gflags = m->d_gflags.p; la.cd.Sy = m->d_Sy.p; la.cd.ncell = m->d_ncell.p; la.cd.e_min = m->e_min; la.cd.e_max = m->e_max; la.sampleE = m->d_E.p; la.exposure = m->d_expo.p; la.X = m->d_X.p;
+  la.d = m->d; la.cd.counts = m->d_counts.p; la.cd.disp = m->d_disp.p; la.cd.gflags = m->d_gflags.p; la.cd.Sy = m->d_Sy.p; la.cd.ncell = m->d_ncell.p; la.cd.e_min = m->e_min; la.cd.e_max = m->e_max; la.cd.samp = m->d_samp.p; la.sampleE = m->d_E.p; la.exposure = m->d_expo.p; la.X = m->d_X.p;
   la.vecs = w.vecs.p; la.Dpad = w.Dpad; la.cmds = w.cmds[w.launches & 1].p; la.sums = w.sums.p; la.logtab = m->d_logtab.p; la.wintab = m->d_wintab.p; la.order = m->d_order.p;
+#ifdef PPCX_TESTING
+  la.cd.samp_stat = m->d_samp_stat.p;
+#endif
   la.lgL = 0; while ((1 << la.lgL) < m->L) ++la.lgL;
   la.nchains = nact; la.active = w.n_active > 0 ? w.active.p : nullptr;
 #ifdef PPCX_TRACE
diff --git a/ppcseq_amd/csrc/ppcx_samp.h b/ppcseq_amd/csrc/ppcx_samp.h
--- /dev/null
+++ b/ppcseq_amd/csrc/ppcx_samp.h
@@ -0,0 +1,126 @@
+#pragma once
+#include "ppcx_disp.h"
+
+namespace ppcx {
+
+constexpr int kSampFns = 4;
+constexpr int kSampPanels = 64;
+constexpr double kSampLo = kDispLo;
+constexpr long kSampGeneDoubles = (long)kSampPanels * kSampFns * kDispStride;
+constexpr double kSampBound = 2.0 * 4.0 * 2.220446049250313e-16;
+constexpr int kSampChecks = 5;
+
+PPCX_HD double samp_exp(double t, double t_lo) { const double e = fast_exp(t); return fma(t_lo, e, e); }
+PPCX_HD void samp_cell(double E, double et, double* l, double* q) {
+  const double z = E * et, z_lo = fma(E, et, -z);
+  const double w = 1.0 + z, bb = w - 1.0;
+  const double err = (1.0 - (w - bb)) + (z - bb);
+  const double qw = 1.0 / w;
+  *l = fma(z_lo, qw, log1p_acc(z));
+  *q = fma(-qw * qw, err + z_lo, qw);
+}
+PPCX_HD void samp_row(const int* row, const double* E, int S, double et, double* out ) {
+  DispSum sl, sa, sq, syq;
+  for (int s = 0; s < S; ++s) {
+    const int y = row[s];
+    if (y < 0) continue;
+    double l, q;
+    samp_cell(E[s], et, &l, &q);
+    const double yd = (double)y;
+    sl.add(l); sa.add(yd * l); sq.add(q); syq.add(yd * q);
+  }
+  out[0] = sl.value(); out[1] = sa.value(); out[2] = sq.value(); out[3] = syq.value();
+}
+PPCX_HD double samp_panel_t(int panel, double x, double* lo) {
+  const double a = fma((double)panel, kDispWidth, kSampLo) + 0.5 * kDispWidth;
+  const double b = 0.5 * kDispWidth * x;
+  const double s = a + b, bb = s - a;
+  *lo = (a - (s - bb)) + (b - bb);
+  return s;
+}
+PPCX_HD double samp_check_x(const DispFit& f, int j) {
+  if (j == 0) return -1.0;
+  if (j == 1) return 1.0;
+  const int k = j == 2 ? 1 : (j == 3 ? 4 : 8);
+  return 0.5 * (f.xnode[k] + f.xnode[k + 1]);
+}
+PPCX_HD double samp_check_point(const DispFit& f, const int* row, const double* E, int S, int panel, int j, const double* coef) {
+  const double x = samp_check_x(f, j);
+  double lo, v[kSampFns], worst = 0.0;
+  const double t = samp_panel_t(panel, x, &lo);
+  samp_row(row, E, S, samp_exp(t, lo), v);
+  for (int fn = 0; fn < kSampFns; ++fn) {
+    const double p = disp_horner(coef + fn * kDispStride, x);
+    double dev = v[fn] != 0.0 ? fabs(p - v[fn]) / fabs(v[fn]) : fabs(p);
+    if (!(dev == dev)) dev = 1.0;
+    worst = dev > worst ? dev : worst;
+  }
+  return worst;
+}
+PPCX_HD void samp_node(const DispFit& f, const int* row, const double* E, int S, int panel, int k, double* out ) {
+  double lo;
+  const double t = disp_node_sigma(f, panel, k, &lo);
+  samp_row(row, E, S, samp_exp(t, lo), out);
+}
+inline bool samp_build_gene_host(const DispFit& f, const int* row, const double* E, int S, double* out ,
+                                 long perturb_at = -1, double* worst_out = nullptr) {
+  for (int p = 0; p < kSampPanels; ++p) {
+    double fv[kSampFns][kDispN];
+    for (int k = 0; k < kDispN; ++k) {
+      double v[kSampFns];
+      samp_node(f, row, E, S, p, k, v);
+      for (int fn = 0; fn < kSampFns; ++fn) fv[fn][k] = v[fn];
+    }
+    for (int fn = 0; fn < kSampFns; ++fn) disp_fit_panel(f, fv[fn], out + ((long)p * kSampFns + fn) * kDispStride);
+  }
+  if (perturb_at >= 0 && perturb_at < kSampGeneDoubles) out[perturb_at] *= 1.0 + 1e-9;
+  double worst = 0.0;
+  for (int p = 0; p < kSampPanels; ++p)
+    for (int j = 0; j < kSampChecks; ++j) {
+      const double dev = samp_check_point(f, row, E, S, p, j, out + (long)p * kSampFns * kDispStride);
+      worst = dev > worst ? dev : worst;
+    }
+  if (worst_out) *worst_out = worst;
+  return worst <= kSampBound;
+}
+
+struct SampRef { int panel; bool in; double x; };
+PPCX_HD SampRef samp_ref(double intercept, double sigma) {
+  SampRef r;
+  const double t = intercept + sigma, bb = t - intercept;
+  const double lo = (intercept - (t - bb)) + (sigma - bb);
+  const double u = (t - kSampLo) * kDispInvWidth;
+  r.in = u >= 0.0 && u < (double)kSampPanels;
+  const int pi = r.in ? (int)u : 0;
+  r.panel = pi;
+  r.x = fma(lo, 2.0 * kDispInvWidth, fma(t - fma((double)pi, kDispWidth, kSampLo), 2.0 * kDispInvWidth, -1.0));
+  if (!r.in) r.x = 0.0;
+  return r;
+}
+PPCX_HD bool samp_in_range(double intercept, double sigma) {
+  const double u = ((intercept + sigma) - kSampLo) * kDispInvWidth;
+  return u >= 0.0 && u < (double)kSampPanels;
+}
+struct SampSums { double lik, dph, Sr; };
+#if defined(__HIPCC__)
+__host__ __device__ __attribute__((noinline))
+#endif
+inline SampSums samp_gene_at(const double* gene_tab, double intercept, double sigma, int sub, int L, double phi, double invphi) {
+  const SampRef r = samp_ref(intercept, sigma);
+  const double* pg = gene_tab + (long)r.panel * (kSampFns * kDispStride);
+  SampSums o; o.lik = 0.0; o.dph = 0.0; o.Sr = 0.0;
+  for (int f = sub; f < kSampFns; f += L) {
+    const double h = disp_horner(pg + f * kDispStride, r.x);
+    if (f == 0) { o.lik = fma(-phi, h, o.lik); o.dph -= h; }
+    else if (f == 1) o.lik -= h;
+    else if (f == 2) o.Sr += h;
+    else o.Sr = fma(invphi, h, o.Sr);
+  }
+  return o;
+}
+PPCX_HD void samp_lookup(const double* gene_tab, const SampRef& r, double* out ) {
+  const double* c = gene_tab + (long)r.panel * kSampFns * kDispStride;
+  for (int fn = 0; fn < kSampFns; ++fn) out[fn] = disp_horner(c + fn * kDispStride, r.x);
+}
+
+}
diff --git a/ppcseq_amd/csrc/ppcx_testing.h b/ppcseq_amd/csrc/ppcx_testing.h
--- a/ppcseq_amd/csrc/ppcx_testing.h
+++ b/ppcseq_amd/csrc/ppcx_testing.h
@@ -22,6 +22,7 @@
        PPCX_MATH_RNG_EXP = 14, PPCX_MATH_RNG_DIV = 15, PPCX_MATH_NB2_TAILS = 16, PPCX_MATH_COUNT = 17 };
 PPCX_API int ppcx_testing_eval_math(int fn, int n, const double* a, const double* b, const int* y, double* out0, double* out1);
 PPCX_API int ppcx_testing_get_disp_table(ppcx_model* m, double* out);
+PPCX_API int ppcx_testing_get_samp(ppcx_model* m, double* table, unsigned char* flags, long long* stats, int reset);
 PPCX_API int ppcx_testing_psis(int n, int n_cols, const double* lr, const double* cols, double* khat);
 PPCX_API int ppcx_testing_loo(int n, int n_cols, const double* ll, const int32_t* excluded, const double* r_eff, double* out);
 PPCX_API int ppcx_testing_loo_mcse(int n, int n_cols, const double* ll, const int32_t* excluded, const double* r_eff, double* out);
```

Result: slower. 254.6 ESS/s (-41.7%).
